# roysubhankar/dwt-domain-adaptation

Measured on NVIDIA H100. Metric: ResNet-50-DWT images/sec fwd+bwd, higher is better.
Workload: dtype f32

## Files before the change

dwt-domain-adaptation_b200/dwt_b200/_native.py:

```python
from __future__ import annotations

import ctypes
import os
import threading

import torch

_HERE = os.path.dirname(os.path.abspath(__file__))
LIB_PATH = os.environ.get("DWT_B200_LIB") or os.path.join(_HERE, "lib", "libdwt_b200.so")

ABI_VERSION = 10
MAX_DOMAINS = 4
MAX_GROUP_SIZE = 64
TC_MAX_GROUP_SIZE = 128
MODE_TRAIN, MODE_EVAL = 0, 1
EPI_NONE, EPI_AFFINE, EPI_RELU, EPI_RESIDUAL = 0, 1, 2, 4
LAYOUT_NHWC = 0x100
DTYPE_BF16 = 0x200
STATUS_NOT_PD, STATUS_BAD_LABEL = 1, 2
ZCA_MAX_ITERATIONS = 16
EIGH = "eigh"
KIND_WHITEN, KIND_BN = 0, 1

_c_float_p = ctypes.c_void_p
_PtrArray = ctypes.c_void_p * MAX_DOMAINS


class TailSite(ctypes.Structure):
    _fields_ = [("x", ctypes.c_void_p), ("eps", ctypes.c_float), ("momentum", ctypes.c_float),
                ("update_running", ctypes.c_int), ("running_mean", ctypes.POINTER(ctypes.c_void_p)),
                ("running_cov", ctypes.POINTER(ctypes.c_void_p)), ("gamma", ctypes.c_void_p), ("beta", ctypes.c_void_p),
                ("save_mean", ctypes.c_void_p), ("save_w", ctypes.c_void_p), ("dx", ctypes.c_void_p),
                ("dgamma", ctypes.c_void_p), ("dbeta", ctypes.c_void_p)]

_SIGNATURES = {
    "dwt_abi_version": (ctypes.c_int, []),
    "dwt_last_error": (ctypes.c_char_p, []),
    "dwt_workspace_bytes": (ctypes.c_size_t, [ctypes.c_int64, ctypes.c_int64, ctypes.c_int64, ctypes.c_int, ctypes.c_int]),
    "dwt_whiten_fwd": (ctypes.c_int, [_c_float_p, _c_float_p, ctypes.c_int64, ctypes.c_int64, ctypes.c_int64,
                                      ctypes.c_int, ctypes.c_int, ctypes.c_int, ctypes.c_float, ctypes.c_float,
                                      ctypes.c_int, ctypes.POINTER(ctypes.c_void_p), ctypes.POINTER(ctypes.c_void_p),
                                      _c_float_p, _c_float_p, _c_float_p, ctypes.c_void_p, ctypes.c_int, _c_float_p,
                                      _c_float_p, ctypes.c_void_p, ctypes.c_size_t, ctypes.c_void_p]),
    "dwt_whiten_bwd": (ctypes.c_int, [_c_float_p, _c_float_p, _c_float_p, _c_float_p, ctypes.c_int64, ctypes.c_int64,
                                      ctypes.c_int64, ctypes.c_int, ctypes.c_int, ctypes.c_int, ctypes.c_float,
                                      _c_float_p, _c_float_p, _c_float_p, _c_float_p, ctypes.c_void_p, _c_float_p,
                                      ctypes.c_int, _c_float_p, _c_float_p, ctypes.c_void_p, ctypes.c_size_t,
                                      ctypes.c_void_p]),
    "dwt_whiten_zca_fwd": (ctypes.c_int, [_c_float_p, _c_float_p, ctypes.c_int64, ctypes.c_int64, ctypes.c_int64,
                                          ctypes.c_int, ctypes.c_int, ctypes.c_int, ctypes.c_float, ctypes.c_float,
                                          ctypes.c_int, ctypes.POINTER(ctypes.c_void_p), ctypes.POINTER(ctypes.c_void_p),
                                          ctypes.c_int, _c_float_p, _c_float_p, _c_float_p, ctypes.c_void_p,
                                          ctypes.c_size_t, ctypes.c_void_p]),
    "dwt_whiten_zca_bwd": (ctypes.c_int, [_c_float_p, _c_float_p, _c_float_p, ctypes.c_int64, ctypes.c_int64,
                                          ctypes.c_int64, ctypes.c_int, ctypes.c_int, ctypes.c_int, ctypes.c_float,
                                          ctypes.c_int, _c_float_p, _c_float_p, _c_float_p, ctypes.c_void_p,
                                          ctypes.c_size_t, ctypes.c_void_p]),
    "dwt_whiten_eigh_fwd": (ctypes.c_int, [_c_float_p, _c_float_p, ctypes.c_int64, ctypes.c_int64, ctypes.c_int64,
                                           ctypes.c_int, ctypes.c_int, ctypes.c_int, ctypes.c_float, ctypes.c_float,
                                           ctypes.c_int, ctypes.POINTER(ctypes.c_void_p), ctypes.POINTER(ctypes.c_void_p),
                                           _c_float_p, _c_float_p, _c_float_p, ctypes.c_void_p, ctypes.c_size_t,
                                           ctypes.c_void_p]),
    "dwt_whiten_eigh_bwd": (ctypes.c_int, [_c_float_p, _c_float_p, _c_float_p, ctypes.c_int64, ctypes.c_int64,
                                           ctypes.c_int64, ctypes.c_int, ctypes.c_int, ctypes.c_int, ctypes.c_float,
                                           _c_float_p, _c_float_p, _c_float_p, ctypes.c_void_p, ctypes.c_size_t,
                                           ctypes.c_void_p]),
    "dwt_whiten_color_fwd": (ctypes.c_int, [_c_float_p, _c_float_p, ctypes.c_int64, ctypes.c_int64, ctypes.c_int64,
                                            ctypes.c_int, ctypes.c_int, ctypes.c_int, ctypes.c_float, ctypes.c_float,
                                            ctypes.c_int, ctypes.POINTER(ctypes.c_void_p), ctypes.POINTER(ctypes.c_void_p),
                                            _c_float_p, _c_float_p, _c_float_p, _c_float_p, ctypes.c_void_p, ctypes.c_size_t,
                                            ctypes.c_void_p]),
    "dwt_whiten_color_bwd": (ctypes.c_int, [_c_float_p, _c_float_p, _c_float_p, ctypes.c_int64, ctypes.c_int64,
                                            ctypes.c_int64, ctypes.c_int, ctypes.c_int, ctypes.c_int, ctypes.c_float,
                                            _c_float_p, _c_float_p, _c_float_p, _c_float_p, _c_float_p, ctypes.c_void_p,
                                            ctypes.c_size_t, ctypes.c_void_p]),
    "dwt_instance_workspace_bytes": (ctypes.c_size_t, [ctypes.c_int64, ctypes.c_int64, ctypes.c_int64, ctypes.c_int]),
    "dwt_whiten_instance_fwd": (ctypes.c_int, [_c_float_p, _c_float_p, ctypes.c_int64, ctypes.c_int64, ctypes.c_int64,
                                               ctypes.c_int, ctypes.c_int, ctypes.c_float, _c_float_p, _c_float_p,
                                               ctypes.c_void_p, ctypes.c_size_t, ctypes.c_void_p]),
    "dwt_whiten_instance_bwd": (ctypes.c_int, [_c_float_p, _c_float_p, _c_float_p, ctypes.c_int64, ctypes.c_int64,
                                               ctypes.c_int64, ctypes.c_int, ctypes.c_int, ctypes.c_float, _c_float_p,
                                               _c_float_p, ctypes.c_void_p, ctypes.c_size_t, ctypes.c_void_p]),
    "dwt_switch_workspace_bytes": (ctypes.c_size_t, [ctypes.c_int64, ctypes.c_int64, ctypes.c_int64, ctypes.c_int]),
    "dwt_whiten_switch_fwd": (ctypes.c_int, [_c_float_p, _c_float_p, ctypes.c_int64, ctypes.c_int64, ctypes.c_int64,
                                             ctypes.c_int, ctypes.c_int, ctypes.c_float, ctypes.c_float, ctypes.c_int,
                                             _c_float_p, _c_float_p, _c_float_p, _c_float_p, _c_float_p, _c_float_p,
                                             ctypes.c_void_p, ctypes.c_size_t, ctypes.c_void_p]),
    "dwt_whiten_switch_bwd": (ctypes.c_int, [_c_float_p, _c_float_p, _c_float_p, ctypes.c_int64, ctypes.c_int64,
                                             ctypes.c_int64, ctypes.c_int, ctypes.c_int, ctypes.c_float, _c_float_p,
                                             _c_float_p, _c_float_p, _c_float_p, _c_float_p, ctypes.c_void_p,
                                             ctypes.c_size_t, ctypes.c_void_p]),
    "dwt_bn_fwd": (ctypes.c_int, [_c_float_p, _c_float_p, ctypes.c_int64, ctypes.c_int64, ctypes.c_int64,
                                  ctypes.c_int, ctypes.c_int, ctypes.c_float, ctypes.c_float, ctypes.c_int,
                                  ctypes.POINTER(ctypes.c_void_p), ctypes.POINTER(ctypes.c_void_p), _c_float_p,
                                  _c_float_p, _c_float_p, ctypes.c_void_p, ctypes.c_int, _c_float_p, _c_float_p,
                                  ctypes.c_void_p, ctypes.c_size_t, ctypes.c_void_p]),
    "dwt_bn_bwd": (ctypes.c_int, [_c_float_p, _c_float_p, _c_float_p, _c_float_p, ctypes.c_int64, ctypes.c_int64, ctypes.c_int64,
                                  ctypes.c_int, ctypes.c_int, _c_float_p, _c_float_p, _c_float_p, _c_float_p,
                                  ctypes.c_void_p, _c_float_p, ctypes.c_int, _c_float_p, _c_float_p, ctypes.c_void_p,
                                  ctypes.c_size_t, ctypes.c_void_p]),
    "dwt_tail2_fwd": (ctypes.c_int, [ctypes.c_int, ctypes.POINTER(TailSite), _c_float_p, ctypes.c_void_p, ctypes.c_int64,
                                     ctypes.c_int64, ctypes.c_int64, ctypes.c_int, ctypes.c_int, ctypes.c_void_p,
                                     ctypes.c_size_t, ctypes.c_void_p]),
    "dwt_tail2_bwd": (ctypes.c_int, [ctypes.c_int, ctypes.POINTER(TailSite), _c_float_p, _c_float_p, ctypes.c_void_p,
                                     _c_float_p, ctypes.c_int64, ctypes.c_int64, ctypes.c_int64, ctypes.c_int, ctypes.c_int,
                                     ctypes.c_void_p, ctypes.c_size_t, ctypes.c_void_p]),
    "dwt_mec_fwd_bwd": (ctypes.c_int, [_c_float_p, _c_float_p, ctypes.c_int64, ctypes.c_int64, _c_float_p,
                                       _c_float_p, _c_float_p, ctypes.c_void_p]),
    "dwt_head_loss_fwd_bwd": (ctypes.c_int, [_c_float_p, ctypes.c_void_p, ctypes.c_int64, ctypes.c_int64, ctypes.c_float,
                                             _c_float_p, _c_float_p, ctypes.c_void_p, ctypes.c_void_p]),
    "dwt_augment_pair": (ctypes.c_int, [ctypes.c_void_p, ctypes.c_int64, ctypes.c_int, ctypes.c_int, ctypes.c_int,
                                        ctypes.c_void_p, ctypes.c_void_p, ctypes.c_void_p, _c_float_p,
                                        ctypes.POINTER(ctypes.c_float), ctypes.POINTER(ctypes.c_float), _c_float_p,
                                        _c_float_p, ctypes.c_int, ctypes.c_void_p]),
    "dwt_maxpool_fwd": (ctypes.c_int, [_c_float_p, _c_float_p, ctypes.c_void_p, ctypes.c_int64, ctypes.c_int64, ctypes.c_int64,
                                       ctypes.c_int64, ctypes.c_int, ctypes.c_int, ctypes.c_int, ctypes.c_int, ctypes.c_void_p]),
    "dwt_maxpool_bwd": (ctypes.c_int, [_c_float_p, ctypes.c_void_p, _c_float_p, ctypes.c_int64, ctypes.c_int64, ctypes.c_int64,
                                       ctypes.c_int64, ctypes.c_int, ctypes.c_int, ctypes.c_int, ctypes.c_int, ctypes.c_void_p]),
    "dwt_launch_count": (ctypes.c_int64, []),
    "dwt_profile_begin": (None, []),
    "dwt_profile_end": (ctypes.c_int, [ctypes.c_void_p, ctypes.c_int]),
}


class ProfileEntry(ctypes.Structure):
    _fields_ = [("name", ctypes.c_char * 48), ("launches", ctypes.c_int64), ("ms", ctypes.c_double),
                ("bytes", ctypes.c_double)]


def profile_begin():
    lib().dwt_profile_begin()


def profile_end():
    cap = 1024
    buf = (ProfileEntry * cap)()
    k = lib().dwt_profile_end(ctypes.cast(buf, ctypes.c_void_p), cap)
    return {buf[i].name.decode(): dict(launches=buf[i].launches, ms=buf[i].ms, bytes=buf[i].bytes) for i in range(k)}


def by_family(prof):
    out = {}
    for name, v in prof.items():
        f = out.setdefault(name.split("|")[0], dict(launches=0, ms=0.0, bytes=0.0))
        for k in f:
            f[k] += v[k]
    return out


def launch_count() -> int:
    return int(lib().dwt_launch_count())
EXPORTS = tuple(_SIGNATURES)

_lib = None
_lock = threading.Lock()


class NativeError(RuntimeError):
    pass


def lib() -> ctypes.CDLL:
    global _lib
    if _lib is None:
        with _lock:
            if _lib is None:
                if not os.path.exists(LIB_PATH):
                    raise NativeError(
                        f"{LIB_PATH} is missing: build it with `python {os.path.join(_HERE, 'build.py')}` "
                        "(dwt_b200 has no CPU or PyTorch fallback)")
                handle = ctypes.CDLL(LIB_PATH)
                for name, (res, args) in _SIGNATURES.items():
                    fn = getattr(handle, name)
                    fn.restype, fn.argtypes = res, args
                if handle.dwt_abi_version() != ABI_VERSION:
                    raise NativeError("libdwt_b200.so ABI version mismatch; rebuild it")
                _lib = handle
    return _lib


def channels_last_supported(channels: int, group_size: int) -> bool:
    if group_size not in (1, 2, 4) or channels % 4:
        return False
    return 0 < channels // 4 <= 16384


def small_bf16_supported(hw: int, group_size: int) -> bool:
    return group_size in (1, 2, 4) and hw % 4 == 0


def tensor_core_bf16_supported(n: int, channels: int, hw: int, group_size: int) -> bool:
    return (group_size in (8, 16, 32, 64) and channels % group_size == 0 and hw >= 32 and hw % 8 == 0
            and n * hw >= 4096)


def tensor_core_nhwc_supported(n: int, channels: int, hw: int, group_size: int) -> bool:
    return (group_size in (8, 16, 32, 64, TC_MAX_GROUP_SIZE) and channels % group_size == 0 and hw >= 32 and hw % 4 == 0
            and n * hw >= 4096)


def check(rc: int) -> None:
    if rc != 0:
        raise NativeError(f"libdwt_b200 error {rc}: {lib().dwt_last_error().decode()}")


def ptr(t):
    return None if t is None else ctypes.c_void_p(t.data_ptr())


def ptr_array(tensors):
    arr = _PtrArray()
    for i, t in enumerate(tensors):
        arr[i] = None if t is None else t.data_ptr()
    return ctypes.cast(arr, ctypes.POINTER(ctypes.c_void_p))


def require_cuda(*tensors, any_dtype=False, bf16=False) -> torch.device:
    dev = None
    for t in tensors:
        if t is None:
            continue
        if not t.is_cuda:
            raise NativeError("dwt_b200 runs on CUDA tensors only (no CPU fallback); got a tensor on " + str(t.device))
        if t.dtype != torch.float32 and not any_dtype and not (bf16 and t.dtype == torch.bfloat16):
            raise NativeError("dwt_b200 computes in float32 (activations may also be bfloat16); got " + str(t.dtype))
        if dev is None:
            dev = t.device
        elif t.device != dev:
            raise NativeError(f"tensors on different devices: {dev} vs {t.device}")
    return dev


def stream_ptr(device) -> ctypes.c_void_p:
    return ctypes.c_void_p(torch.cuda.current_stream(device).cuda_stream)


_workspaces: dict = {}


def workspace(device, n, c, hw, gs, nd):
    if gs == TC_MAX_GROUP_SIZE and c % gs == 0:
        c, gs = 2 * c, MAX_GROUP_SIZE
    need = lib().dwt_workspace_bytes(n, c, hw, gs, nd)
    if need == 0:
        raise NativeError(f"invalid geometry for workspace: C={c} group_size={gs} domains={nd}")
    key = (device.index, torch.cuda.current_stream(device).cuda_stream)
    buf = _workspaces.get(key)
    if buf is None or buf.numel() < need:
        buf = torch.zeros(max(need, 8 << 20), dtype=torch.uint8, device=device)
        _workspaces[key] = buf
    return buf


def instance_workspace(device, n, c, hw, gs):
    need = lib().dwt_instance_workspace_bytes(n, c, hw, gs)
    buf = workspace(device, 1, 4, 1, 1, 1)
    if buf.numel() < need:
        buf = torch.zeros(need, dtype=torch.uint8, device=device)
        _workspaces[(device.index, torch.cuda.current_stream(device).cuda_stream)] = buf
    return buf


def switch_workspace(device, n, c, hw, gs):
    need = lib().dwt_switch_workspace_bytes(n, c, hw, gs)
    buf = workspace(device, 1, 4, 1, 1, 1)
    if buf.numel() < need:
        buf = torch.zeros(need, dtype=torch.uint8, device=device)
        _workspaces[(device.index, torch.cuda.current_stream(device).cuda_stream)] = buf
    return buf


def status(device=None) -> int:
    device = torch.device("cuda", torch.cuda.current_device()) if device is None else device
    buf = _workspaces.get((device.index, torch.cuda.current_stream(device).cuda_stream))
    return 0 if buf is None else int(buf[:4].view(torch.int32).item())


def status_all(device=None) -> int:
    device = torch.device("cuda", torch.cuda.current_device()) if device is None else device
    torch.cuda.synchronize(device)
    st = 0
    for (idx, _), buf in _workspaces.items():
        if idx == device.index:
            st |= int(buf[:4].view(torch.int32).item())
    return st


def status_ptr(device):
    return ctypes.c_void_p(workspace(device, 1, 4, 1, 1, 1).data_ptr())


def clear_status(device=None) -> None:
    device = torch.device("cuda", torch.cuda.current_device()) if device is None else device
    buf = _workspaces.get((device.index, torch.cuda.current_stream(device).cuda_stream))
    if buf is not None:
        buf[:4].zero_()


class NotPositiveDefiniteError(torch.linalg.LinAlgError):
    """What the reference's torch.cholesky raises at utils/whitening.py:53, raised late: the kernels never sync the
    host, so the failure is seen at the next poll (raise_on_status) or explicit check_status() call."""


_poll = {"every": 0, "count": 0}


def raise_on_status(every: int = 1) -> None:
    _poll["every"], _poll["count"] = max(0, int(every)), 0


def check_status(device=None) -> None:
    st = status(device)
    if st == 0:
        return
    clear_status(device)
    if st & STATUS_NOT_PD:
        raise NotPositiveDefiniteError(
            "cholesky: a whitening covariance was not positive definite (status word bit 0; the reference raises "
            "from torch.cholesky, utils/whitening.py:53); the affected group's output is NaN and its running-"
            "statistics update was skipped")
    if st & STATUS_BAD_LABEL:
        raise IndexError("head loss: a label was outside [0, num_classes) and is not ignore_index=-100 "
                         "(F.nll_loss asserts here); the row was dropped")
    raise NativeError(f"unknown status bits {st:#x}")


def poll_status(device) -> None:
    if _poll["every"]:
        _poll["count"] += 1
        if _poll["count"] >= _poll["every"]:
            _poll["count"] = 0
            check_status(device)
```

dwt-domain-adaptation_b200/dwt_b200/build.py:

```python
from __future__ import annotations

import os
import shlex
import subprocess
import sys

HERE = os.path.dirname(os.path.abspath(__file__))
CSRC = os.path.join(HERE, "csrc")
LIB = os.path.join(HERE, "lib", "libdwt_b200.so")
SOURCES = ["api.cu", "norm_small.cu", "norm_tiled.cu", "norm_tc.cu", "norm_tc_apply.cu", "norm_dense.cu", "norm_cl.cu", "mec.cu", "augment.cu", "pool.cu"]
NVCC_FLAGS = ["-O3", "-std=c++17", "-gencode", "arch=compute_90a,code=sm_90a", "-lineinfo",
              "-Xcompiler", "-fPIC,-fvisibility=hidden", "--expt-relaxed-constexpr"]
NVCC_FLAGS += shlex.split(os.environ.get("DWT_NVCC_EXTRA", ""))


def _nvcc() -> str:
    for cand in (os.environ.get("NVCC"), "/usr/local/cuda/bin/nvcc", "nvcc"):
        if cand and (os.path.isabs(cand) and os.path.exists(cand) or not os.path.isabs(cand)):
            return cand
    raise RuntimeError("nvcc not found")


def _stale() -> bool:
    if not os.path.exists(LIB):
        return True
    t = os.path.getmtime(LIB)
    deps = [os.path.join(CSRC, f) for f in os.listdir(CSRC)]
    deps.append(os.path.join(HERE, "..", "..", "include", "dwt_b200.h"))
    deps.append(os.path.abspath(__file__))
    return any(os.path.getmtime(d) > t for d in deps)


def build(force: bool = False, verbose: bool = False) -> str:
    if not force and not _stale():
        return LIB
    os.makedirs(os.path.dirname(LIB), exist_ok=True)
    objs = []
    procs = []
    for src in SOURCES:
        obj = os.path.join(HERE, "lib", src.replace(".cu", ".o"))
        cmd = [_nvcc(), *NVCC_FLAGS, "-c", os.path.join(CSRC, src), "-o", obj]
        if verbose:
            cmd.insert(1, "-Xptxas=-v")
            print(" ".join(cmd), flush=True)
        procs.append((src, subprocess.Popen(cmd, stdout=subprocess.PIPE, stderr=subprocess.STDOUT, text=True)))
        objs.append(obj)
    for src, p in procs:
        out, _ = p.communicate()
        if verbose or p.returncode:
            sys.stdout.write(out)
        if p.returncode:
            raise RuntimeError(f"nvcc failed on {src}")
    link = [_nvcc(), "-shared", "-gencode", "arch=compute_90a,code=sm_90a", "-Xcompiler", "-fPIC", *objs, "-o", LIB]
    subprocess.check_call(link)
    return LIB


if __name__ == "__main__":
    print(build(force="--force" in sys.argv, verbose="--verbose" in sys.argv))
```

dwt-domain-adaptation_b200/dwt_b200/csrc/api.cu:

```cuda
#include <stdarg.h>
#include <stdio.h>
#include <stdlib.h>

#include <atomic>
#include <mutex>
#include <string>
#include <vector>
#include <string.h>

#include "norm_launch.h"

namespace {

thread_local char g_err[512] = "";

int fail(int code, const char* fmt, ...) {
  va_list ap;
  va_start(ap, fmt);
  vsnprintf(g_err, sizeof(g_err), fmt, ap);
  va_end(ap);
  return code;
}

int check_launch(const char* what) {
// ... 587 lines not shown
        case SMALL: dwt::small_bwd_reduce(x, dout, bf16, p.gm, p.vec, fin, beta, w.partial, w.counters, st); break;
        case TILED: dwt::tiled_bwd_reduce(x, dout, p.gm, p.vec, fin, w.partial, w.counters, st); break;
        case TC:
          if (int cr = dwt::tc_bwd_reduce(x, dout, bf16, nhwc, p.gm, rchunks, save_mean, w.partial, st, c.mode == DWT_MODE_TRAIN))
            return fail(DWT_E_LAUNCH, "cuTensorMapEncodeTiled failed (CUresult %d) x=%p dout=%p N=%d C=%d HW=%d D=%d", cr, (const void*)x, (const void*)dout, p.gm.N, p.gm.C, p.gm.HW, p.gm.D);
      }
    }
    if (c.r.fam == CL || c.r.fam == TC) {
      if (int rc = check_launch(c.r.fam == CL ? "channels-last backward reduction kernel" : "tensor-core backward reduction kernel")) return rc;
      Launch l(basis.own() ? basis_family(basis, true, bf16) : c.name(true, FINALIZE), &p.gm, 0.0, st);
      if (c.r.fam == CL) {
        dwt::cl_bwd_finalize(w.partial, cp.nred, p.gm, fin, st);
      } else {
        dwt::dense_partial_reduce(w.partial, rchunks, rproblems, w.gram, st);
        if (basis.own()) basis_bwd(w.gram, p.gm, fin, basis, w.shift, st);
        else dwt::dense_bwd_coef(w.gram, p.gm, fin, w.shift, st);
      }
    }
  } else if (basis.own()) {
    Launch l(basis_family(basis, true, bf16), &p.gm, 0.0, st);
    basis_bwd(nullptr, p.gm, fin, basis, w.shift, st);
  } else {
    Launch l(c.name(true, PREP), &p.gm, 0.0, st);
    if (c.r.fam == TC) dwt::dense_bwd_coef(nullptr, p.gm, fin, w.shift, st);
    else if (c.r.fam == TILED) dwt::tiled_bwd_prep(p.gm, fin, st);
    else dwt::small_bwd_prep(p.gm, fin, st);
  }
  if (int rc = check_launch(c.r.fam == CL ? "channels-last backward finalize kernel" : "whitening backward reduction kernel")) return rc;
  {
    Launch l(c.name(true, APPLY), &p.gm, (3.0 + (dout2 && !masked ? 1.0 : 0.0)) * E, st);
    switch (c.r.fam) {
      case CL:
        if (masked) dwt::cl_bwd_apply(x, dresidual, nullptr, dx, bf16, p.gm, cp.new_, cp.gz_ew, DWT_EPI_AFFINE, w.coef, save_mean, save_w, gamma, beta, st);
        else dwt::cl_bwd_apply(x, dout, dout2, dx, bf16, p.gm, cp.new_, cp.gz_ew, epi, w.coef, save_mean, save_w, gamma, beta, st);
        break;
      case SMALL: dwt::small_bwd_apply(x, dout, dx, bf16, p.gm_ew, p.vec, p.chunks_ew, epi, w.coef, save_mean, save_w, gamma, beta, st); break;
      case TILED: dwt::tiled_bwd_apply(x, dout, dx, p.gm_ew, p.vec, p.chunks_ew, w.coef, st); break;
      case TC:
        if (int cr = dwt::tc_bwd_apply(x, dout, dx, bf16, nhwc, p.gm, tc_apply_ctas(p.gm, 1, 64), w.coef, save_mean, w.shift, st))
          return fail(DWT_E_LAUNCH, "cuTensorMapEncodeTiled failed (CUresult %d)", cr);
    }
  }
  return check_launch(c.r.fam == CL ? "channels-last backward apply kernel" : "whitening backward apply kernel");
}

struct SiteConst { float a, b, unbias; };
SiteConst site_const(int kind, float eps, int64_t N, int64_t HW) {
  if (kind == DWT_KIND_BN) {
    const double M = (double)N * (double)HW;
    return {1.f, eps, M > 1.0 ? (float)(M / (M - 1.0)) : 1.f};
  }
  return {1.f - eps, eps, 1.f};
}

int tail2_plan(Plan& p, int kind, bool bf16, const dwt_tail_site* s, const void* out, int64_t N, int64_t C, int64_t HW, int GS, int D) {
  if (kind != DWT_KIND_WHITEN && kind != DWT_KIND_BN) return fail(DWT_E_INVALID, "bad kind %d", kind);
  if (kind == DWT_KIND_BN && GS != 1) return fail(DWT_E_INVALID, "batch norm has group_size 1 (got %d)", GS);
  if (!s) return fail(DWT_E_INVALID, "null pointer argument");
  if (int rc = make_plan(p, K_STATS, K_APPLY, s[0].x, s[1].x, out, N, C, HW, GS, D, 4)) return rc;
  Route r;
  if (route(p, true, bf16, nullptr, &r) != DWT_OK || r.fam != CL)
    return fail(DWT_E_UNSUPPORTED, "the two-site tail runs on the channels-last kernels: " DWT_CL_RULE " (C=%lld gs=%d)",
                (long long)C, GS);
  for (int k = 0; k < 2; ++k)
    if (!s[k].x || !s[k].gamma || !s[k].beta || !s[k].save_mean || !s[k].save_w || !out) return fail(DWT_E_INVALID, "null pointer argument");
  return check_align(bf16, (uintptr_t)s[0].x | (uintptr_t)s[1].x | (uintptr_t)out, "channels-last tensors");
}

int tail2_workspace(Workspace (&w)[2], void* ws, size_t ws_bytes, int64_t C, int GS, int D) {
  if (!ws) return fail(DWT_E_INVALID, "null pointer argument");
  w[0] = carve(ws, C, GS, D);
  w[1] = carve(ws, C, GS, D, w[0].bytes);
  if (w[1].bytes > ws_bytes) return fail(DWT_E_WORKSPACE, "workspace too small: need %zu bytes, got %zu", w[1].bytes, ws_bytes);
  if ((uintptr_t)ws % 256 != 0) return fail(DWT_E_WORKSPACE, "workspace must be 256-byte aligned");
  return DWT_OK;
}

int tail2_fwd(int kind, const dwt_tail_site* s, float* y, uint8_t* relu_mask, int64_t N, int64_t C, int64_t HW, int GS, int D,
              void* ws, size_t ws_bytes, cudaStream_t st) {
  const bool bf16 = (kind & DWT_DTYPE_BF16) != 0;
  kind &= ~DWT_DTYPE_BF16;
  Plan p;
  if (int rc = tail2_plan(p, kind, bf16, s, y, N, C, HW, GS, D)) return rc;
  if (!relu_mask) return fail(DWT_E_INVALID, "the two-site tail writes the ReLU byte map its backward reads");
  for (int k = 0; k < 2; ++k)
    if (int rc = check_running(s[k].update_running != 0, s[k].running_mean, s[k].running_cov, D)) return rc;
  Workspace w[2];
  if (int rc = tail2_workspace(w, ws, ws_bytes, C, GS, D)) return rc;
  dwt::FwdFin fin[2];
  for (int k = 0; k < 2; ++k) {
    const SiteConst sc = site_const(kind, s[k].eps, N, HW);
    fin[k] = make_fwd_fin(sc.a, sc.b, s[k].momentum, sc.unbias, s[k].update_running, s[k].update_running != 0, s[k].running_mean,
                          s[k].running_cov, s[k].save_mean, s[k].save_w, w[k], D);
  }
  const double n_el = (double)D * (double)N * (double)C * (double)HW;
  const double E = (bf16 ? 2.0 : 4.0) * n_el, Mb = 0.25 * n_el;
  const ClPlan cp = cl_plan(p.gm, 3, 3, 8, 4);
  for (int k = 0; k < 2; ++k) {
    Launch l(fam(bf16, "cl_stats", "cl_stats_bf16"), &p.gm, E, st);
    dwt::cl_stats(s[k].x, bf16, p.gm, cp.nred, cp.gz_red, w[k].partial, w[k].shift, st);
  }
  if (int rc = check_launch("channels-last statistics kernel")) return rc;
  {
    Launch l(fam(bf16, "cl_tail2_fwd_finalize", "cl_tail2_fwd_finalize_bf16"), &p.gm, 0.0, st);
    dwt::cl_fwd_finalize(w[0].partial, cp.nred, w[0].shift, p.gm, fin[0], st, &fin[1], (size_t)(w[1].partial - w[0].partial),
                         (size_t)(w[1].shift - w[0].shift));
  }
  if (int rc = check_launch("channels-last finalize kernel")) return rc;
  {
    Launch l(fam(bf16, "cl_tail2_apply", "cl_tail2_apply_bf16"), &p.gm, 3.0 * E + Mb, st);
    dwt::cl_tail2_apply(s[0].x, s[1].x, y, bf16, p.gm, cp.new_, cp.gz_ew, s[0].save_mean, s[0].save_w, s[0].gamma, s[0].beta,
                        s[1].save_mean, s[1].save_w, s[1].gamma, s[1].beta, relu_mask, st);
  }
  return check_launch("channels-last two-site apply kernel");
}

int tail2_bwd(int kind, const dwt_tail_site* s, const float* dout, const float* dout2, const uint8_t* relu_mask, float* dz,
              int64_t N, int64_t C, int64_t HW, int GS, int D, void* ws, size_t ws_bytes, cudaStream_t st) {
  const bool bf16 = (kind & DWT_DTYPE_BF16) != 0;
  kind &= ~DWT_DTYPE_BF16;
  Plan p;
  if (int rc = tail2_plan(p, kind, bf16, s, dz, N, C, HW, GS, D)) return rc;
  if (!dout || !relu_mask || !s[0].dx || !s[1].dx) return fail(DWT_E_INVALID, "null pointer argument");
  if (int rc = check_align(bf16, (uintptr_t)dout | (uintptr_t)dout2 | (uintptr_t)s[0].dx | (uintptr_t)s[1].dx, "channels-last tensors")) return rc;
  for (int k = 0; k < 2; ++k)
    if ((s[k].dgamma == nullptr) != (s[k].dbeta == nullptr)) return fail(DWT_E_INVALID, "dgamma and dbeta go together");
  Workspace w[2];
  if (int rc = tail2_workspace(w, ws, ws_bytes, C, GS, D)) return rc;
  dwt::BwdFin fin[2];
  for (int k = 0; k < 2; ++k)
    fin[k] = make_bwd_fin(site_const(kind, s[k].eps, N, HW).a, DWT_MODE_TRAIN, k ? DWT_EPI_AFFINE : (DWT_EPI_AFFINE | DWT_EPI_RELU | DWT_EPI_RESIDUAL),
                          s[k].save_mean, s[k].save_w, s[k].gamma, s[k].dgamma, s[k].dbeta, w[k]);
  const double n_el = (double)D * (double)N * (double)C * (double)HW;
  const double E = (bf16 ? 2.0 : 4.0) * n_el, Mb = 0.25 * n_el;
  const ClPlan cp = cl_plan(p.gm, 2, 2, 4, 4);
  {
    Launch l(fam(bf16, "cl_tail2_bwd_reduce", "cl_tail2_bwd_reduce_bf16"), &p.gm, (4.0 + (dout2 ? 1.0 : 0.0)) * E + Mb, st);
    dwt::cl_tail2_bwd_reduce(s[0].x, s[1].x, dout, dout2, bf16, p.gm, cp.nred, cp.gz_red, s[0].save_mean, s[1].save_mean, relu_mask, dz,
                             w[0].partial, (size_t)(w[1].partial - w[0].partial), st);
  }
  if (int rc = check_launch("channels-last two-site backward reduction kernel")) return rc;
  {
    Launch l(fam(bf16, "cl_tail2_bwd_finalize", "cl_tail2_bwd_finalize_bf16"), &p.gm, 0.0, st);
    dwt::cl_bwd_finalize(w[0].partial, cp.nred, p.gm, fin[0], st, &fin[1], (size_t)(w[1].partial - w[0].partial));
  }
  if (int rc = check_launch("channels-last backward finalize kernel")) return rc;
  {
    Launch l(fam(bf16, "cl_tail2_bwd_apply", "cl_tail2_bwd_apply_bf16"), &p.gm, 5.0 * E, st);
    dwt::cl_tail2_bwd_apply(s[0].x, s[1].x, dz, s[0].dx, s[1].dx, bf16, p.gm, cp.new_, cp.gz_ew, w[0].coef, w[1].coef, st);
  }
  return check_launch("channels-last two-site backward apply kernel");
}

int inst_refuse(int64_t N, int64_t C, int64_t HW, int GS, int flags, const char* what = "instance whitening") {
  return fail(DWT_E_UNSUPPORTED, "%s is built for the tensor-core kernels only: group_size 8, 16, 32, 64 "
              "dividing C, HW >= 256 and a multiple of 4 (NCHW bf16: of 8), N <= 65535 images, N*C*HW < 2^31 "
              "(C=%lld HW=%lld N=%lld gs=%d flags=%#x)", what, (long long)C, (long long)HW, (long long)N, GS, flags);
}

int inst_geom(dwt::Geom& gm, int64_t N, int64_t C, int64_t HW, int GS, int flags, const char* what = "instance whitening") {
  if (flags & ~(DWT_LAYOUT_NHWC | DWT_DTYPE_BF16)) return fail(DWT_E_INVALID, "bad flags %#x (DWT_LAYOUT_NHWC | DWT_DTYPE_BF16)", flags);
  if (N <= 0 || C <= 0 || HW <= 0) return fail(DWT_E_INVALID, "empty tensor (N=%lld C=%lld HW=%lld)", (long long)N,
                                               (long long)C, (long long)HW);
  const bool nchw_bf16 = (flags & DWT_DTYPE_BF16) && !(flags & DWT_LAYOUT_NHWC);
  if ((GS != 8 && GS != 16 && GS != 32 && GS != 64) || C % GS != 0 || HW < 256 || HW % (nchw_bf16 ? 8 : 4) != 0 ||
      N > 65535 || N * C * HW >= (int64_t)1 << 31)
    return inst_refuse(N, C, HW, GS, flags, what);
  gm = dwt::Geom{};
  gm.N = 1; gm.C = (int)C; gm.HW = (int)HW; gm.GS = GS; gm.G = (int)(C / GS); gm.D = (int)N; gm.ppc = 1;
  gm.M = (float)HW;
  gm.nchunks = tc_chunks(gm);
  return DWT_OK;
}

Workspace carve_instance(void* base, const dwt::Geom& gm) {
  const size_t P = (size_t)dwt::tc_superblocks(gm) * gm.D, nacc = 64 * 64 + 64;
  size_t off = kOffScratch;
  auto take = [&](size_t nbytes) { size_t o = off; off = align_up(off + nbytes, 256); return o; };
  char* b = static_cast<char*>(base);
  Workspace w{};
  w.status = reinterpret_cast<int*>(b);
  w.counters = reinterpret_cast<int*>(b + kOffCounters);
  w.dom_counter = reinterpret_cast<int*>(b + kOffDom1);
  w.dom_counter2 = reinterpret_cast<int*>(b + kOffDom2);
  w.partial = reinterpret_cast<float*>(b + take(sizeof(float) * P * gm.nchunks * nacc));
  w.gram = gm.nchunks > 1 ? reinterpret_cast<float*>(b + take(sizeof(float) * P * nacc)) : w.partial;
  w.shift = reinterpret_cast<float*>(b + take(sizeof(float) * P * 64));
  w.coef = reinterpret_cast<float*>(b + take(sizeof(float) * (size_t)gm.D * gm.G * dwt::coef_stride(gm.GS)));
  w.bytes = off;
  return w;
}

const char* const kIwName[6][4] = {
    {"iw_stats", "iw_stats_bf16", "iw_stats_nhwc", "iw_stats_nhwc_bf16"},
    {"iw_fwd_finalize", "iw_fwd_finalize_bf16", "iw_fwd_finalize", "iw_fwd_finalize_bf16"},
    {"iw_apply", "iw_apply_bf16", "iw_apply_nhwc", "iw_apply_nhwc_bf16"},
    {"iw_bwd_reduce", "iw_bwd_reduce_bf16", "iw_bwd_reduce_nhwc", "iw_bwd_reduce_nhwc_bf16"},
    {"iw_bwd_finalize", "iw_bwd_finalize_bf16", "iw_bwd_finalize", "iw_bwd_finalize_bf16"},
    {"iw_bwd_apply", "iw_bwd_apply_bf16", "iw_bwd_apply_nhwc", "iw_bwd_apply_nhwc_bf16"}};

int inst_validate(dwt::Geom& gm, Workspace& w, const void* in0, const void* in1, const void* out, int64_t N, int64_t C, int64_t HW,
                  int GS, int flags, const float* save_mean, const float* save_w, void* ws, size_t ws_bytes) {
  if (int rc = inst_geom(gm, N, C, HW, GS, flags)) return rc;
  if (!in0 || !in1 || !out || !save_mean || !save_w || !ws) return fail(DWT_E_INVALID, "null pointer argument");
  if (((uintptr_t)in0 | (uintptr_t)in1 | (uintptr_t)out | (uintptr_t)save_w) % 16 != 0)
    return fail(DWT_E_INVALID, "activation tensors and save_w must be 16-byte aligned (instance whitening: TMA and vector stores)");
  w = carve_instance(ws, gm);
  if (w.bytes > ws_bytes) return fail(DWT_E_WORKSPACE, "workspace too small: need %zu bytes, got %zu", w.bytes, ws_bytes);
  if ((uintptr_t)ws % 256 != 0) return fail(DWT_E_WORKSPACE, "workspace must be 256-byte aligned");
  if (ensure_tc() != 0) return inst_refuse(N, C, HW, GS, flags);
  return DWT_OK;
}

int instance_fwd(const void* x, void* y, int64_t N, int64_t C, int64_t HW, int GS, int flags, float eps, float* save_mean,
                 float* save_w, void* ws, size_t ws_bytes, cudaStream_t st) {
  dwt::Geom gm;
  Workspace w;
  if (int rc = inst_validate(gm, w, x, x, y, N, C, HW, GS, flags, save_mean, save_w, ws, ws_bytes)) return rc;
  const bool nhwc = (flags & DWT_LAYOUT_NHWC) != 0, bf16 = (flags & DWT_DTYPE_BF16) != 0;
  const int k = 2 * nhwc + bf16;
  const double E = (bf16 ? 2.0 : 4.0) * (double)N * (double)C * (double)HW;
  dwt::FwdFin fin{};
  fin.a = 1.f - eps; fin.b = eps; fin.save_mean = save_mean; fin.save_w = save_w; fin.status = w.status;
  {
    Launch l(kIwName[0][k], &gm, E, st);
    if (int cr = dwt::tc_stats(x, bf16, nhwc, gm, gm.nchunks, w.shift, w.partial, st))
      return fail(DWT_E_LAUNCH, "cuTensorMapEncodeTiled failed (CUresult %d) x=%p N=%lld C=%d HW=%d", cr, x, (long long)N, gm.C, gm.HW);
  }
  if (int rc = check_launch("instance whitening statistics kernel")) return rc;
  {
    Launch l(kIwName[1][k], &gm, 0.0, st);
    if (gm.nchunks > 1) dwt::dense_partial_reduce(w.partial, gm.nchunks, dwt::tc_superblocks(gm) * gm.D, w.gram, st);
    dwt::dense_fwd_instance(w.gram, w.shift, gm, fin, st);
  }
  if (int rc = check_launch("instance whitening finalize kernel")) return rc;
  {
    Launch l(kIwName[2][k], &gm, 2.0 * E, st);
    if (int cr = dwt::tc_apply(x, y, bf16, nhwc, gm, tc_apply_ctas(gm, 1, 64), save_mean, save_w, st))
      return fail(DWT_E_LAUNCH, "cuTensorMapEncodeTiled failed (CUresult %d)", cr);
  }
  return check_launch("instance whitening apply kernel");
}

int instance_bwd(const void* x, const void* dout, void* dx, int64_t N, int64_t C, int64_t HW, int GS, int flags, float eps,
                 const float* save_mean, const float* save_w, void* ws, size_t ws_bytes, cudaStream_t st) {
  dwt::Geom gm;
  Workspace w;
  if (int rc = inst_validate(gm, w, x, dout, dx, N, C, HW, GS, flags, save_mean, save_w, ws, ws_bytes)) return rc;
  const bool nhwc = (flags & DWT_LAYOUT_NHWC) != 0, bf16 = (flags & DWT_DTYPE_BF16) != 0;
  const int k = 2 * nhwc + bf16;
  const double E = (bf16 ? 2.0 : 4.0) * (double)N * (double)C * (double)HW;
  dwt::BwdFin fin{};
  fin.a = 1.f - eps; fin.mode = DWT_MODE_TRAIN; fin.save_mean = save_mean; fin.save_w = save_w; fin.coef = w.coef;
  {
    Launch l(kIwName[3][k], &gm, 2.0 * E, st);
    if (int cr = dwt::tc_bwd_reduce(x, dout, bf16, nhwc, gm, gm.nchunks, save_mean, w.partial, st))
      return fail(DWT_E_LAUNCH, "cuTensorMapEncodeTiled failed (CUresult %d) x=%p dout=%p N=%lld C=%d HW=%d", cr, x, dout,
                  (long long)N, gm.C, gm.HW);
  }
  if (int rc = check_launch("instance whitening backward reduction kernel")) return rc;
  {
    Launch l(kIwName[4][k], &gm, 0.0, st);
    if (gm.nchunks > 1) dwt::dense_partial_reduce(w.partial, gm.nchunks, dwt::tc_superblocks(gm) * gm.D, w.gram, st);
    dwt::dense_bwd_coef(w.gram, gm, fin, w.shift, st);
  }
  if (int rc = check_launch("instance whitening backward finalize kernel")) return rc;
  {
    Launch l(kIwName[5][k], &gm, 3.0 * E, st);
    if (int cr = dwt::tc_bwd_apply(x, dout, dx, bf16, nhwc, gm, tc_apply_ctas(gm, 1, 64), w.coef, save_mean, w.shift, st))
      return fail(DWT_E_LAUNCH, "cuTensorMapEncodeTiled failed (CUresult %d)", cr);
  }
  return check_launch("instance whitening backward apply kernel");
}

constexpr const char* kSw = "switchable whitening";

struct SwWork {
  Workspace w;
  float* pd;
  float* part;
  float* sums;
  float* mu;
};

SwWork carve_switch(void* base, const dwt::Geom& gm) {
  SwWork s{};
  s.w = carve_instance(base, gm);
  const size_t rec = (size_t)gm.GS * gm.GS + gm.GS, P = (size_t)gm.D * gm.G;
  size_t off = s.w.bytes;
  auto take = [&](size_t nbytes) { size_t o = off; off = align_up(off + nbytes, 256); return o; };
  char* b = static_cast<char*>(base);
  s.pd = reinterpret_cast<float*>(b + take(sizeof(float) * P * rec));
  s.part = reinterpret_cast<float*>(b + take(sizeof(float) * P * 8));
  s.sums = reinterpret_cast<float*>(b + take(sizeof(float) * gm.G * rec));
  s.mu = reinterpret_cast<float*>(b + take(sizeof(float) * (size_t)gm.D * gm.C));
  s.w.bytes = off;
  return s;
}

int sw_geom(dwt::Geom& gm, int64_t N, int64_t C, int64_t HW, int GS, int mode) {
  if (mode & ~(DWT_MODE_EVAL | DWT_LAYOUT_NHWC | DWT_DTYPE_BF16))
    return fail(DWT_E_INVALID, "bad mode %#x (DWT_MODE_TRAIN or DWT_MODE_EVAL | DWT_LAYOUT_NHWC | DWT_DTYPE_BF16)", mode);
  return inst_geom(gm, N, C, HW, GS, mode & ~DWT_MODE_EVAL, kSw);
}

const char* const kSwName[6][4] = {
// ... 110 lines not shown
}

int dwt_whiten_instance_fwd(const float* x, float* y, int64_t N, int64_t C, int64_t HW, int group_size, int flags, float eps,
                            float* save_mean, float* save_w, void* workspace, size_t workspace_bytes, dwt_stream_t stream) {
  return instance_fwd(x, y, N, C, HW, group_size, flags, eps, save_mean, save_w, workspace, workspace_bytes, (cudaStream_t)stream);
}

size_t dwt_switch_workspace_bytes(int64_t N, int64_t C, int64_t HW, int group_size) {
  dwt::Geom gm;
  char saved[sizeof(g_err)];
  memcpy(saved, g_err, sizeof(g_err));
  const int rc = sw_geom(gm, N, C, HW, group_size, 0);
  memcpy(g_err, saved, sizeof(g_err));
  return rc ? 0 : carve_switch(nullptr, gm).w.bytes;
}

int dwt_whiten_switch_fwd(const float* x, float* y, int64_t N, int64_t C, int64_t HW, int group_size, int mode, float eps,
                          float momentum, int update_running, float* running_mean, float* running_cov, const float* mix,
                          float* save_mean, float* save_w, float* save_stats, void* workspace, size_t workspace_bytes,
                          dwt_stream_t stream) {
  return switch_fwd(x, y, N, C, HW, group_size, mode, eps, momentum, update_running, running_mean, running_cov, mix, save_mean,
                    save_w, save_stats, workspace, workspace_bytes, (cudaStream_t)stream);
}

int dwt_whiten_switch_bwd(const float* x, const float* dout, float* dx, int64_t N, int64_t C, int64_t HW, int group_size,
                          int mode, float eps, const float* mix, const float* save_mean, const float* save_w,
                          const float* save_stats, float* dmix, void* workspace, size_t workspace_bytes, dwt_stream_t stream) {
  return switch_bwd(x, dout, dx, N, C, HW, group_size, mode, eps, mix, save_mean, save_w, save_stats, dmix, workspace,
                    workspace_bytes, (cudaStream_t)stream);
}

int dwt_whiten_instance_bwd(const float* x, const float* dout, float* dx, int64_t N, int64_t C, int64_t HW, int group_size,
                            int flags, float eps, const float* save_mean, const float* save_w, void* workspace,
                            size_t workspace_bytes, dwt_stream_t stream) {
  return instance_bwd(x, dout, dx, N, C, HW, group_size, flags, eps, save_mean, save_w, workspace, workspace_bytes,
                      (cudaStream_t)stream);
}

const char* dwt_last_error(void) { return g_err; }

size_t dwt_workspace_bytes(int64_t N, int64_t C, int64_t HW, int group_size, int n_domains) {
  (void)N; (void)HW;
  if (C <= 0 || group_size < 1 || group_size > DWT_MAX_GROUP_SIZE || C % group_size != 0 || n_domains < 1 ||
      n_domains > DWT_MAX_DOMAINS)
    return 0;
  return carve(nullptr, C, group_size, n_domains, carve(nullptr, C, group_size, n_domains).bytes).bytes;
}

int dwt_whiten_fwd(const float* x, float* y, int64_t N, int64_t C, int64_t HW, int group_size, int n_domains,
                   int mode, float eps, float momentum, int update_running, float* const* running_mean,
                   float* const* running_cov, const float* gamma, const float* beta, const float* residual,
                   uint8_t* relu_mask, int epilogue, float* save_mean, float* save_w, void* workspace,
                   size_t workspace_bytes, dwt_stream_t stream) {
  return whiten_like_fwd(x, y, N, C, HW, group_size, n_domains, mode, 1.f - eps, eps, momentum, 1.f, update_running,
                         running_mean, running_cov, gamma, beta, residual, relu_mask, epilogue, save_mean, save_w,
                         workspace, workspace_bytes, (cudaStream_t)stream);
}

int dwt_whiten_bwd(const float* x, const float* dout, const float* dout2, float* dx, int64_t N, int64_t C, int64_t HW, int group_size,
                   int n_domains, int mode, float eps, const float* save_mean, const float* save_w,
                   const float* gamma, const float* beta, const uint8_t* relu_mask, float* dresidual, int epilogue,
                   float* dgamma, float* dbeta, void* workspace, size_t workspace_bytes, dwt_stream_t stream) {
  return whiten_like_bwd(x, dout, dout2, dx, N, C, HW, group_size, n_domains, mode, 1.f - eps, save_mean, save_w, gamma,
                         beta, relu_mask, dresidual, epilogue, dgamma, dbeta, workspace, workspace_bytes,
                         (cudaStream_t)stream);
}

int dwt_whiten_zca_fwd(const float* x, float* y, int64_t N, int64_t C, int64_t HW, int group_size, int n_domains, int mode,
                       float eps, float momentum, int update_running, float* const* running_mean, float* const* running_cov,
                       int iterations, float* save_mean, float* save_w, float* save_p, void* workspace,
                       size_t workspace_bytes, dwt_stream_t stream) {
  return whiten_like_fwd(x, y, N, C, HW, group_size, n_domains, mode, 1.f - eps, eps, momentum, 1.f, update_running,
                         running_mean, running_cov, nullptr, nullptr, nullptr, nullptr, 0, save_mean, save_w, workspace,
                         workspace_bytes, (cudaStream_t)stream, Basis{Basis::NEWTON_SCHULZ, iterations, save_p});
}

int dwt_whiten_zca_bwd(const float* x, const float* dout, float* dx, int64_t N, int64_t C, int64_t HW, int group_size,
                       int n_domains, int mode, float eps, int iterations, const float* save_mean, const float* save_w,
                       const float* save_p, void* workspace, size_t workspace_bytes, dwt_stream_t stream) {
  return whiten_like_bwd(x, dout, nullptr, dx, N, C, HW, group_size, n_domains, mode, 1.f - eps, save_mean, save_w, nullptr,
                         nullptr, nullptr, nullptr, 0, nullptr, nullptr, workspace, workspace_bytes, (cudaStream_t)stream,
                         Basis{Basis::NEWTON_SCHULZ, iterations, save_p});
}

int dwt_whiten_eigh_fwd(const float* x, float* y, int64_t N, int64_t C, int64_t HW, int group_size, int n_domains, int mode,
                        float eps, float momentum, int update_running, float* const* running_mean, float* const* running_cov,
                        float* save_mean, float* save_w, float* save_e, void* workspace, size_t workspace_bytes,
                        dwt_stream_t stream) {
  return whiten_like_fwd(x, y, N, C, HW, group_size, n_domains, mode, 1.f - eps, eps, momentum, 1.f, update_running,
                         running_mean, running_cov, nullptr, nullptr, nullptr, nullptr, 0, save_mean, save_w, workspace,
                         workspace_bytes, (cudaStream_t)stream, Basis{Basis::EIGH, 0, save_e});
}

int dwt_whiten_eigh_bwd(const float* x, const float* dout, float* dx, int64_t N, int64_t C, int64_t HW, int group_size,
                        int n_domains, int mode, float eps, const float* save_mean, const float* save_w, const float* save_e,
                        void* workspace, size_t workspace_bytes, dwt_stream_t stream) {
  return whiten_like_bwd(x, dout, nullptr, dx, N, C, HW, group_size, n_domains, mode, 1.f - eps, save_mean, save_w, nullptr,
                         nullptr, nullptr, nullptr, 0, nullptr, nullptr, workspace, workspace_bytes, (cudaStream_t)stream,
                         Basis{Basis::EIGH, 0, save_e});
}

int dwt_whiten_color_fwd(const float* x, float* y, int64_t N, int64_t C, int64_t HW, int group_size, int n_domains, int mode,
                         float eps, float momentum, int update_running, float* const* running_mean, float* const* running_cov,
                         const float* color, const float* bias, float* save_mean, float* save_w, void* workspace,
                         size_t workspace_bytes, dwt_stream_t stream) {
  Basis b;
  b.kind = Basis::COLOR; b.color = color; b.bias = bias;
  return whiten_like_fwd(x, y, N, C, HW, group_size, n_domains, mode, 1.f - eps, eps, momentum, 1.f, update_running,
                         running_mean, running_cov, nullptr, nullptr, nullptr, nullptr, 0, save_mean, save_w, workspace,
                         workspace_bytes, (cudaStream_t)stream, b);
}

int dwt_whiten_color_bwd(const float* x, const float* dout, float* dx, int64_t N, int64_t C, int64_t HW, int group_size,
                         int n_domains, int mode, float eps, const float* save_mean, const float* save_w, const float* color,
                         float* dcolor, float* dbias, void* workspace, size_t workspace_bytes, dwt_stream_t stream) {
  Basis b;
  b.kind = Basis::COLOR; b.color = color; b.dcolor = dcolor; b.dbias = dbias;
  return whiten_like_bwd(x, dout, nullptr, dx, N, C, HW, group_size, n_domains, mode, 1.f - eps, save_mean, save_w, nullptr,
                         nullptr, nullptr, nullptr, 0, nullptr, nullptr, workspace, workspace_bytes, (cudaStream_t)stream, b);
}

int dwt_bn_fwd(const float* x, float* y, int64_t N, int64_t C, int64_t HW, int n_domains, int mode, float eps,
               float factor, int update_running, float* const* running_mean, float* const* running_var,
               const float* weight, const float* bias, const float* residual, uint8_t* relu_mask, int epilogue,
               float* save_mean, float* save_invstd, void* workspace, size_t workspace_bytes, dwt_stream_t stream) {
  const double M = (double)N * (double)HW;
  const float unbias = M > 1.0 ? (float)(M / (M - 1.0)) : 1.f;
  return whiten_like_fwd(x, y, N, C, HW, 1, n_domains, mode, 1.f, eps, factor, unbias, update_running, running_mean,
                         running_var, weight, bias, residual, relu_mask, epilogue, save_mean, save_invstd, workspace,
                         workspace_bytes, (cudaStream_t)stream);
}

int dwt_bn_bwd(const float* x, const float* dout, const float* dout2, float* dx, int64_t N, int64_t C, int64_t HW, int n_domains,
               int mode, const float* save_mean, const float* save_invstd, const float* weight, const float* bias,
               const uint8_t* relu_mask, float* dresidual, int epilogue, float* dweight, float* dbias, void* workspace,
               size_t workspace_bytes, dwt_stream_t stream) {
  return whiten_like_bwd(x, dout, dout2, dx, N, C, HW, 1, n_domains, mode, 1.f, save_mean, save_invstd, weight, bias,
                         relu_mask, dresidual, epilogue, dweight, dbias, workspace, workspace_bytes,
                         (cudaStream_t)stream);
}

int dwt_tail2_fwd(int kind, const dwt_tail_site* sites, float* y, uint8_t* relu_mask, int64_t N, int64_t C, int64_t HW,
                  int group_size, int n_domains, void* workspace, size_t workspace_bytes, dwt_stream_t stream) {
  return tail2_fwd(kind, sites, y, relu_mask, N, C, HW, group_size, n_domains, workspace, workspace_bytes, (cudaStream_t)stream);
}

int dwt_tail2_bwd(int kind, const dwt_tail_site* sites, const float* dout, const float* dout2, const uint8_t* relu_mask, float* dz,
                  int64_t N, int64_t C, int64_t HW, int group_size, int n_domains, void* workspace, size_t workspace_bytes,
                  dwt_stream_t stream) {
  return tail2_bwd(kind, sites, dout, dout2, relu_mask, dz, N, C, HW, group_size, n_domains, workspace, workspace_bytes,
                   (cudaStream_t)stream);
}

int dwt_mec_fwd_bwd(const float* x, const float* y, int64_t N, int64_t K, float* loss, float* gx, float* gy,
                    dwt_stream_t stream) {
  if (!x || !y || !loss || !gx || !gy) return fail(DWT_E_INVALID, "null pointer argument");
  if (N <= 0 || K <= 0 || N >= (1 << 24) || K >= (1 << 24)) return fail(DWT_E_INVALID, "bad logits shape [%lld,%lld]", (long long)N, (long long)K);
  {
    Launch l("mec", nullptr, 16.0 * (double)N * (double)K, (cudaStream_t)stream);
    dwt::mec_launch(x, y, (int)N, (int)K, loss, gx, gy, (cudaStream_t)stream);
  }
  return check_launch("MEC kernel");
}

int dwt_head_loss_fwd_bwd(const float* logits, const int64_t* labels, int64_t B, int64_t K, float lambda, float* losses,
                          float* grad, int* status, dwt_stream_t stream) {
  if (!logits || !labels || !losses || !grad) return fail(DWT_E_INVALID, "null pointer argument");
  if (B <= 0 || K <= 0 || B >= (1 << 22) || K >= (1 << 24)) return fail(DWT_E_INVALID, "bad logits shape [3*%lld,%lld]", (long long)B, (long long)K);
  {
    Launch l("head_loss", nullptr, 4.0 * 3 * (double)B * (double)K * 2, (cudaStream_t)stream);
    dwt::head_loss_launch(logits, reinterpret_cast<const long long*>(labels), (int)B, (int)K, lambda, losses, grad, status,
                          (cudaStream_t)stream);
  }
  return check_launch("head loss kernel");
}

int dwt_augment_pair(const uint8_t* images, int64_t B, int src_h, int src_w, int crop, const int32_t* crop_plain,
                     const int32_t* crop_aug, const uint8_t* flip, const float* affine, const float* mean,
                     const float* stdv, float* out_plain, float* out_aug, int layout, dwt_stream_t stream) {
  if (!images || !mean || !stdv) return fail(DWT_E_INVALID, "null pointer argument");
  if (!out_plain && !out_aug) return fail(DWT_E_INVALID, "at least one of out_plain / out_aug is needed");
  if (out_plain && !crop_plain) return fail(DWT_E_INVALID, "out_plain needs crop_plain");
  if (out_aug && (!crop_aug || !flip || !affine)) return fail(DWT_E_INVALID, "out_aug needs crop_aug, flip and affine");
  if (B <= 0 || B > 65535 || src_h <= 0 || src_w <= 0 || src_h > 16384 || src_w > 16384)
    return fail(DWT_E_INVALID, "bad image batch [%lld,%d,%d,3]", (long long)B, src_h, src_w);
  if (crop <= 0 || crop > src_h || crop > src_w) return fail(DWT_E_INVALID, "crop %d does not fit %dx%d", crop, src_h, src_w);
  if (layout != 0 && layout != DWT_LAYOUT_NHWC) return fail(DWT_E_INVALID, "layout must be 0 (NCHW) or DWT_LAYOUT_NHWC");
  for (int c = 0; c < 3; ++c)
    if (!(stdv[c] != 0.f)) return fail(DWT_E_INVALID, "std[%d] must be non-zero", c);
  {
    const double px = (double)B * crop * crop;
    Launch l("augment_pair", nullptr, px * 3 * ((out_plain ? 5.0 : 0.0) + (out_aug ? 5.0 : 0.0)), (cudaStream_t)stream);
    dwt::augment_pair_launch(images, (int)B, src_h, src_w, crop, crop_plain, crop_aug, flip, affine, mean, stdv, out_plain,
                             out_aug, layout != 0, (cudaStream_t)stream);
  }
  return check_launch("augmentation kernel");
}

namespace {
int pool_check(int64_t N, int64_t H, int64_t W, int64_t C, int k, int s, int p, int* OH, int* OW) {
  if (N <= 0 || H <= 0 || W <= 0 || C <= 0 || C % 4 != 0) return fail(DWT_E_INVALID, "bad pooling input [%lld,%lld,%lld,%lld] (C must be a multiple of 4)", (long long)N, (long long)H, (long long)W, (long long)C);
  if (k < 1 || k > 15 || s < 1 || p < 0 || 2 * p > k) return fail(DWT_E_INVALID, "bad pooling window k=%d s=%d p=%d (k <= 15, pad <= k/2)", k, s, p);
  if (H + 2 * p < k || W + 2 * p < k) return fail(DWT_E_INVALID, "pooling window larger than the padded image");
  *OH = (int)((H + 2 * p - k) / s + 1);
  *OW = (int)((W + 2 * p - k) / s + 1);
  if (N * H * W * C >= ((int64_t)1 << 40)) return fail(DWT_E_UNSUPPORTED, "tensor too large");
  return DWT_OK;
}
}

int dwt_maxpool_fwd(const float* x, float* y, uint8_t* argmax, int64_t N, int64_t H, int64_t W, int64_t C, int kernel,
                    int stride, int padding, int flags, dwt_stream_t stream) {
  int OH = 0, OW = 0;
  if (int rc = pool_check(N, H, W, C, kernel, stride, padding, &OH, &OW)) return rc;
  if (flags != 0 && flags != DWT_DTYPE_BF16) return fail(DWT_E_INVALID, "bad flags %#x (0 or DWT_DTYPE_BF16)", flags);
  const bool bf16 = flags == DWT_DTYPE_BF16;
  if (!x || !y || !argmax) return fail(DWT_E_INVALID, "null pointer argument");
  if ((uintptr_t)argmax % 4 != 0) return fail(DWT_E_INVALID, "pooling tensors must be 16-byte aligned");
  if (int rc = check_align(bf16, (uintptr_t)x | (uintptr_t)y, "pooling tensors")) return rc;
  {
    const double in = (double)N * H * W * C, out = (double)N * OH * OW * C;
    Launch l(fam(bf16, "maxpool_fwd", "maxpool_fwd_bf16"), nullptr, (bf16 ? 2.0 : 4.0) * (in + out) + out, (cudaStream_t)stream);
    dwt::maxpool_fwd_launch(x, y, bf16, argmax, (int)N, (int)H, (int)W, (int)C, OH, OW, kernel, stride, padding, (cudaStream_t)stream);
  }
  return check_launch("max-pool forward kernel");
}

int dwt_maxpool_bwd(const float* dy, const uint8_t* argmax, float* dx, int64_t N, int64_t H, int64_t W, int64_t C, int kernel,
                    int stride, int padding, int flags, dwt_stream_t stream) {
  int OH = 0, OW = 0;
  if (int rc = pool_check(N, H, W, C, kernel, stride, padding, &OH, &OW)) return rc;
  if (flags != 0 && flags != DWT_DTYPE_BF16) return fail(DWT_E_INVALID, "bad flags %#x (0 or DWT_DTYPE_BF16)", flags);
  const bool bf16 = flags == DWT_DTYPE_BF16;
  if (!dy || !dx || !argmax) return fail(DWT_E_INVALID, "null pointer argument");
  if ((uintptr_t)argmax % 4 != 0) return fail(DWT_E_INVALID, "pooling tensors must be 16-byte aligned");
  if (int rc = check_align(bf16, (uintptr_t)dy | (uintptr_t)dx, "pooling tensors")) return rc;
  {
    const double in = (double)N * H * W * C, out = (double)N * OH * OW * C;
    Launch l(fam(bf16, "maxpool_bwd", "maxpool_bwd_bf16"), nullptr, (bf16 ? 2.0 : 4.0) * (in + out) + out, (cudaStream_t)stream);
    dwt::maxpool_bwd_launch(dy, argmax, dx, bf16, (int)N, (int)H, (int)W, (int)C, OH, OW, kernel, stride, padding, (cudaStream_t)stream);
  }
  return check_launch("max-pool backward kernel");
}

int64_t dwt_launch_count(void) { return g_launches.load(); }

void dwt_profile_begin(void) {
  std::lock_guard<std::mutex> lk(g_prof_mu);
  for (auto& r : g_prof) { g_event_pool.push_back(r.a); g_event_pool.push_back(r.b); }
  g_prof.clear();
  g_prof_on = true;
}

int dwt_profile_end(dwt_profile_entry* out, int max_entries) {
  std::vector<ProfRec> recs;
  {
    std::lock_guard<std::mutex> lk(g_prof_mu);
    g_prof_on = false;
    recs.swap(g_prof);
  }
  int n = 0;
  for (auto& r : recs) {
    float ms = 0.f;
    if (cudaEventSynchronize(r.b) == cudaSuccess && cudaEventElapsedTime(&ms, r.a, r.b) == cudaSuccess) {
      int k = 0;
      for (; k < n; ++k)
        if (strcmp(out[k].name, r.name) == 0) break;
      if (k == n && n < max_entries) {
        memset(&out[n], 0, sizeof(out[n]));
        strncpy(out[n].name, r.name, sizeof(out[n].name) - 1);
        ++n;
      }
      if (k < n) { out[k].launches += 1; out[k].ms += ms; out[k].bytes += r.bytes; }
    }
    std::lock_guard<std::mutex> lk(g_prof_mu);
    g_event_pool.push_back(r.a); g_event_pool.push_back(r.b);
  }
  return n;
}

}
```

dwt-domain-adaptation_b200/dwt_b200/csrc/norm_cl.cu:

```cuda
#include <stdlib.h>

#include <type_traits>

#include <cuda_bf16.h>

#include "dwt_common.cuh"
#include "norm_launch.h"
#include "small_algebra.cuh"

namespace dwt {
namespace {

constexpr int kT = 256;

__device__ __forceinline__ void pdl_wait() { asm volatile("griddepcontrol.wait;" ::: "memory"); }
__device__ __forceinline__ void pdl_launch_dependents() { asm volatile("griddepcontrol.launch_dependents;" ::: "memory"); }

template <int GS> struct ClShape {
  static constexpr int NSUB = 4 / GS;
  static constexpr int NM = GS * (GS + 1) / 2;
  static constexpr int FWD1 = GS + NM;
  static constexpr int BWD1 = GS * GS + GS;
  static constexpr int FWD = NSUB * FWD1;
  static constexpr int BWD = NSUB * BWD1;
};

struct ClThread {
  int C4, CW, LS, rpi, col, rsub, q;
  bool active;
  __device__ __forceinline__ ClThread(const Geom& gm) {
    C4 = gm.C >> 2;
    CW = gm.cw;
    LS = gm.ls;
    rpi = kT / LS;
    col = threadIdx.x % LS;
    rsub = threadIdx.x / LS;
    q = blockIdx.y * CW + col;
    active = col < CW && rsub < rpi && q < C4;
  }
};

template <int UNROLL, bool DESC, class F>
__device__ __forceinline__ void sweep_rows(const ClThread& t, unsigned rows, F&& body) {
  const unsigned krows = (unsigned)t.rpi * UNROLL, nch = (rows + krows - 1) / krows;
  for (unsigned i = blockIdx.x; i < nch; i += gridDim.x) body((DESC ? nch - 1 - i : i) * krows + t.rsub);
}
#define CL_FOR_DOMAINS(d, gm, DESC) \
  for (int di_ = blockIdx.z, d = (DESC) ? (gm).D - 1 - di_ : di_; di_ < (gm).D; di_ += gridDim.z, d = (DESC) ? (gm).D - 1 - di_ : di_)

template <class T> constexpr bool kBf16 = !std::is_same<T, float>::value;
template <class T>
__device__ __forceinline__ float as_stored(float v) {
  if constexpr (kBf16<T>) return __bfloat162float(__float2bfloat16_rn(v));
  else return v;
}

template <int NACC>
__device__ __forceinline__ void column_reduce(const ClThread& t, float (&acc)[NACC], float* sRed) {
  if (t.rpi == 1) return;
  if (t.rsub < t.rpi) {
#pragma unroll
    for (int i = 0; i < NACC; ++i) sRed[i * kT + threadIdx.x] = acc[i];
  }
  __syncthreads();
  if (t.rsub == 0) {
#pragma unroll
    for (int i = 0; i < NACC; ++i) {
      float s = acc[i];
      for (int r = 1; r < t.rpi; ++r) s += sRed[i * kT + r * t.LS + t.col];
      acc[i] = s;
    }
  }
}

template <class T, int GS>
__global__ void __launch_bounds__(kT, 3) cl_stats_kernel(const T* __restrict__ x, const Geom gm,
                                                         float* __restrict__ partial, float* __restrict__ shift) {
  using S = ClShape<GS>;
  constexpr int UNROLL = 8;
  __shared__ float sRed[kT * S::FWD];
  const ClThread t(gm);
  const unsigned rows = (unsigned)gm.N * gm.HW;
  pdl_launch_dependents();
  CL_FOR_DOMAINS(d, gm, true) {
    const T* xd = x + (size_t)d * rows * gm.C + 4 * t.q;
    float K[4] = {0.f, 0.f, 0.f, 0.f};
    if (t.active) {
      const unsigned np = rows < 8 ? rows : 8;
      for (unsigned r = 0; r < np; ++r) {
        const float4 v = ld4(xd + (size_t)r * gm.C);
        K[0] += v.x; K[1] += v.y; K[2] += v.z; K[3] += v.w;
      }
#pragma unroll
      for (int c = 0; c < 4; ++c) K[c] /= (float)np;
      if (rows > 8) {
        float s1[4] = {0.f, 0.f, 0.f, 0.f}, s2[4] = {0.f, 0.f, 0.f, 0.f};
        const size_t mid = (size_t)gm.HW / 2 + (size_t)sqrtf((float)gm.HW) / 2;
        for (unsigned k = 0; k < 8; ++k) {
          const float4 v = ld4(xd + ((2 * (size_t)k + 1) * rows / 16 + mid) % rows * gm.C);
          const float e[4] = {v.x - K[0], v.y - K[1], v.z - K[2], v.w - K[3]};
#pragma unroll
          for (int c = 0; c < 4; ++c) { s1[c] += e[c]; s2[c] = fmaf(e[c], e[c], s2[c]); }
        }
#pragma unroll
        for (int c = 0; c < 4; ++c) {
          const float dk = s1[c] * 0.125f;
          if (401.f * dk * dk > 400.f * (s2[c] * 0.125f)) K[c] += dk;
        }
      }
      if (blockIdx.x == 0 && t.rsub == 0) *reinterpret_cast<float4*>(shift + (size_t)d * gm.C + 4 * t.q) = make_float4(K[0], K[1], K[2], K[3]);
    }
    float acc[S::FWD];
#pragma unroll
    for (int i = 0; i < S::FWD; ++i) acc[i] = 0.f;
    if (t.active) sweep_rows<UNROLL, true>(t, rows, [&](unsigned r) {
      float4 v[UNROLL];
#pragma unroll
      for (int u = 0; u < UNROLL; ++u) {
        const unsigned rr = r + u * t.rpi;
        v[u] = rr < rows ? ld4(xd + (size_t)rr * gm.C) : make_float4(K[0], K[1], K[2], K[3]);
      }
#pragma unroll
      for (int u = 0; u < UNROLL; ++u) {
        const float e[4] = {v[u].x - K[0], v[u].y - K[1], v[u].z - K[2], v[u].w - K[3]};
#pragma unroll
        for (int s = 0; s < S::NSUB; ++s) {
#pragma unroll
          for (int c = 0; c < GS; ++c) {
            acc[s * S::FWD1 + c] += e[s * GS + c];
#pragma unroll
            for (int j = 0; j <= c; ++j)
              acc[s * S::FWD1 + GS + c * (c + 1) / 2 + j] = fmaf(e[s * GS + c], e[s * GS + j], acc[s * S::FWD1 + GS + c * (c + 1) / 2 + j]);
          }
        }
      }
    });
    column_reduce<S::FWD>(t, acc, sRed);
    if (t.rsub == 0 && t.active) {
      float* dst = partial + (((size_t)d * gridDim.x + blockIdx.x) * t.C4 + t.q) * S::FWD;
#pragma unroll
      for (int i = 0; i < S::FWD; ++i) dst[i] = acc[i];
    }
    if (gridDim.z == 1) __syncthreads();
  }
}

template <int GS, int PER>
__device__ __forceinline__ int acc_index(int g, int a) {
  constexpr int NSUB = 4 / GS;
  return (g / NSUB) * (NSUB * PER) + (g % NSUB) * PER + a;
}

constexpr int kFinQ = 2;

template <int NACC>
__device__ __forceinline__ void column_row_sum(const float* __restrict__ col, int nrows, int W, float (&a)[NACC]) {
  static_assert(NACC % 2 == 0, "accumulators are read as float2");
#pragma unroll
  for (int i = 0; i < NACC; ++i) a[i] = 0.f;
#pragma unroll 4
  for (int r = threadIdx.x; r < nrows; r += 32) {
    const float2* p = reinterpret_cast<const float2*>(col + (size_t)r * W);
#pragma unroll
    for (int i = 0; i < NACC / 2; ++i) {
      const float2 v = __ldcg(p + i);
      a[2 * i] += v.x; a[2 * i + 1] += v.y;
    }
  }
#pragma unroll
  for (int o = 1; o < 32; o <<= 1)
#pragma unroll
    for (int i = 0; i < NACC; ++i) a[i] += __shfl_xor_sync(0xffffffffu, a[i], o);
}

template <int NSUB, int PER>
__device__ __forceinline__ void take_group(const float (&a)[NSUB * PER], int s, float (&v)[PER]) {
#pragma unroll
  for (int i = 0; i < PER; ++i) {
    v[i] = a[i];
#pragma unroll
    for (int k = 1; k < NSUB; ++k)
      if (s == k) v[i] = a[k * PER + i];
  }
}

template <int GS>
__device__ __forceinline__ void cl_fwd_finalize_site(const float* __restrict__ partial, int nrows, const float* __restrict__ shift,
                                                     const Geom& gm, const FwdFin& fin) {
  using SH = ClShape<GS>;
  constexpr int NST = GS + GS * GS;
  __shared__ float sStat[DWT_MAX_DOMAINS][kFinQ][SH::NSUB][NST + 1];
  __shared__ unsigned char sBad[DWT_MAX_DOMAINS][kFinQ][SH::NSUB];
  const int s = threadIdx.x, ql = threadIdx.y, d = threadIdx.z, q = blockIdx.x * blockDim.y + ql;
  const int W = (gm.C >> 2) * SH::FWD;
  const float invM = 1.f / gm.M;
  const bool colok = q < (gm.C >> 2);
  const bool lead = colok && s < SH::NSUB;
  const int g = q * SH::NSUB + (lead ? s : 0);
  const bool direct = gm.D == 1 || fin.aliased == 0;
  const int dbuf = direct ? d : 0;
  const bool upd = fin.update_running && lead && (direct || (fin.aliased == 1 && d == 0));
  float rc_old[GS * GS], rm_old[GS];
  if (upd) {
#pragma unroll
    for (int e = 0; e < GS * GS; ++e) rc_old[e] = fin.rcov[dbuf][(size_t)g * GS * GS + e];
#pragma unroll
    for (int e = 0; e < GS; ++e) rm_old[e] = fin.rmean[dbuf][g * GS + e];
  }
  pdl_launch_dependents();
  pdl_wait();
  float a[SH::FWD];
  if (colok) column_row_sum<SH::FWD>(partial + (size_t)d * nrows * W + (size_t)q * SH::FWD, nrows, W, a);
  if (lead) {
    float v[SH::FWD1];
    take_group<SH::NSUB, SH::FWD1>(a, s, v);
    float mean[GS], cov[GS][GS];
#pragma unroll
    for (int i = 0; i < GS; ++i) mean[i] = shift[(size_t)d * gm.C + g * GS + i] + v[i] * invM;
#pragma unroll
    for (int i = 0; i < GS; ++i)
#pragma unroll
      for (int j = 0; j <= i; ++j) {
        const float c = v[GS + i * (i + 1) / 2 + j] * invM - (v[i] * invM) * (v[j] * invM);
        cov[i][j] = c; cov[j][i] = c;
      }
    const bool bad = factor_thread<GS>(gm, fin, d, g, mean, cov, false);
    if (fin.update_running) {
      if (direct) {
        if (!bad) {
          const float m = fin.momentum, kk = 1.f - fin.momentum;
#pragma unroll
          for (int i = 0; i < GS; ++i) {
            fin.rmean[d][g * GS + i] = m * mean[i] + kk * rm_old[i];
#pragma unroll
            for (int j = 0; j < GS; ++j)
              fin.rcov[d][(size_t)g * GS * GS + i * GS + j] = m * (cov[i][j] * fin.unbias) + kk * rc_old[i * GS + j];
          }
        }
      } else {
        sBad[d][ql][s] = bad ? 1 : 0;
#pragma unroll
        for (int i = 0; i < GS; ++i) {
          sStat[d][ql][s][i] = mean[i];
#pragma unroll
          for (int j = 0; j < GS; ++j) sStat[d][ql][s][GS + i * GS + j] = cov[i][j];
        }
      }
    }
  }
  if (!fin.update_running || direct) return;
  __syncthreads();
  if (!(lead && d == 0)) return;
  if (fin.aliased == 1) {
    const float m = fin.momentum, kk = 1.f - fin.momentum;
    float* rc = fin.rcov[0] + (size_t)g * GS * GS;
    float* rm = fin.rmean[0] + g * GS;
    for (int dd = 0; dd < gm.D; ++dd) {
      if (sBad[dd][ql][s]) continue;
#pragma unroll
      for (int e = 0; e < GS * GS; ++e) rc_old[e] = m * (sStat[dd][ql][s][GS + e] * fin.unbias) + kk * rc_old[e];
#pragma unroll
      for (int e = 0; e < GS; ++e) rm_old[e] = m * sStat[dd][ql][s][e] + kk * rm_old[e];
    }
#pragma unroll
    for (int e = 0; e < GS * GS; ++e) rc[e] = rc_old[e];
#pragma unroll
    for (int e = 0; e < GS; ++e) rm[e] = rm_old[e];
  } else {
    for (int dd = 0; dd < gm.D; ++dd)
      if (!sBad[dd][ql][s]) ema_direct<GS>(gm, fin, dd, g, &sStat[dd][ql][s][0], &sStat[dd][ql][s][GS]);
  }
}

template <int GS>
__global__ void __launch_bounds__(32 * kFinQ * DWT_MAX_DOMAINS) cl_fwd_finalize_kernel(const float* __restrict__ partial, size_t pstride, int nrows,
                                                                                      const float* __restrict__ shift, size_t sstride, const Geom gm,
                                                                                      const __grid_constant__ FwdFin fin, const __grid_constant__ FwdFin fin2) {
  const bool second = blockIdx.y != 0;
  cl_fwd_finalize_site<GS>(partial + (second ? pstride : 0), nrows, shift + (second ? sstride : 0), gm, second ? fin2 : fin);
}

template <class T, int GS, int EPI, bool DS>
__global__ void __launch_bounds__(kT, 3) cl_apply_kernel(const T* __restrict__ x, T* __restrict__ y, const Geom gm,
                                                         const float* __restrict__ save_mean, const float* __restrict__ save_w,
                                                         const float* __restrict__ gamma, const float* __restrict__ beta,
                                                         const T* __restrict__ res, uint8_t* __restrict__ mask,
                                                         const float* __restrict__ save_mean_d, const float* __restrict__ save_w_d,
                                                         const float* __restrict__ gamma_d, const float* __restrict__ beta_d) {
  using S = ClShape<GS>;
  constexpr bool RES = (EPI & DWT_EPI_RESIDUAL) != 0;
  static_assert(!DS || RES, "the two-site tail is a residual epilogue");
  constexpr int UNROLL = DS ? 2 : (RES ? 4 : 8);
  const ClThread t(gm);
  if (!t.active) return;
  const unsigned rows = (unsigned)gm.N * gm.HW;
  pdl_wait();
  CL_FOR_DOMAINS(d, gm, false) {
    float Wp[S::NSUB][S::NM], bp[S::NSUB][GS], Wd[DS ? S::NSUB : 1][S::NM], bd[DS ? S::NSUB : 1][GS];
#pragma unroll
    for (int s = 0; s < S::NSUB; ++s) {
      const int g = t.q * S::NSUB + s;
      load_forward_map<GS, EPI>(save_w + ((size_t)d * gm.G + g) * GS * GS, save_mean + (size_t)d * gm.C + g * GS,
                                gamma + g * GS, beta + g * GS, Wp[s], bp[s]);
      if constexpr (DS)
        load_forward_map<GS, DWT_EPI_AFFINE>(save_w_d + ((size_t)d * gm.G + g) * GS * GS, save_mean_d + (size_t)d * gm.C + g * GS,
                                             gamma_d + g * GS, beta_d + g * GS, Wd[s], bd[s]);
    }
    const size_t base = (size_t)d * rows * gm.C + 4 * t.q;
    const T* xd = x + base;
    const T* rd = res + base;
    T* yd = y + base;
    uint8_t* md = mask + (size_t)d * rows * t.C4 + t.q;
    sweep_rows<UNROLL, false>(t, rows, [&](unsigned r) {
      float4 v[UNROLL], rs[UNROLL];
#pragma unroll
      for (int u = 0; u < UNROLL; ++u) {
        const unsigned rr = r + u * t.rpi;
        if (rr < rows) {
          v[u] = ld4(xd + rr * (unsigned)gm.C);
          if constexpr (RES) rs[u] = ld4(rd + rr * (unsigned)gm.C);
        }
      }
#pragma unroll
      for (int u = 0; u < UNROLL; ++u) {
        const unsigned rr = r + u * t.rpi;
        if (rr < rows) {
          const float e[4] = {v[u].x, v[u].y, v[u].z, v[u].w};
          float o[4], ra[4] = {0.f, 0.f, 0.f, 0.f};
          if constexpr (RES) { ra[0] = rs[u].x; ra[1] = rs[u].y; ra[2] = rs[u].z; ra[3] = rs[u].w; }
          unsigned bits = 0;
#pragma unroll
          for (int s = 0; s < S::NSUB; ++s) {
            float xi[GS], oi[GS];
            if constexpr (DS) {
              float xdi[GS], odi[GS];
#pragma unroll
              for (int c = 0; c < GS; ++c) xdi[c] = ra[s * GS + c];
              apply_group<GS>(Wd[s], bd[s], xdi, odi);
#pragma unroll
              for (int c = 0; c < GS; ++c) ra[s * GS + c] = as_stored<T>(odi[c]);
            }
#pragma unroll
            for (int c = 0; c < GS; ++c) xi[c] = e[s * GS + c];
            apply_group<GS>(Wp[s], bp[s], xi, oi);
#pragma unroll
            for (int c = 0; c < GS; ++c) {
              const float z = RES ? oi[c] + ra[s * GS + c] : oi[c];
              if constexpr (RES) bits |= (z > 0.f ? 1u : 0u) << (s * GS + c);
              o[s * GS + c] = (EPI & DWT_EPI_RELU) ? fmaxf(z, 0.f) : z;
            }
          }
          st4(yd + rr * (unsigned)gm.C, make_float4(o[0], o[1], o[2], o[3]));
          if constexpr (RES) { if (mask != nullptr) md[rr * (unsigned)t.C4] = (uint8_t)bits; }
        }
      }
    });
  }
}

template <int GS>
__device__ __forceinline__ void bwd_accumulate(float* acc, const float (&dz)[GS], const float (&xi)[GS], const float* mu) {
#pragma unroll
  for (int i = 0; i < GS; ++i) {
    acc[GS * GS + i] += dz[i];
#pragma unroll
    for (int j = 0; j < GS; ++j) acc[i * GS + j] = fmaf(dz[i], xi[j] - mu[j], acc[i * GS + j]);
  }
}

template <class T, int GS, int EPI, bool D2, bool DS>
__global__ void __launch_bounds__(kT, 2) cl_bwd_reduce_kernel(const T* __restrict__ x, const T* __restrict__ dout, const T* __restrict__ dout2,
                                                              const Geom gm, const float* __restrict__ save_mean,
                                                              const float* __restrict__ save_w, const float* __restrict__ gamma,
                                                              const float* __restrict__ beta, const uint8_t* __restrict__ mask,
                                                              T* __restrict__ dzout, float* __restrict__ partial,
                                                              const T* __restrict__ xds, const float* __restrict__ save_mean_d,
                                                              size_t pstride) {
  using S = ClShape<GS>;
  constexpr int UNROLL = 4;
  constexpr bool MASK = (EPI & DWT_EPI_RESIDUAL) != 0;
  constexpr bool RELU = (EPI & DWT_EPI_RELU) != 0 && !MASK;
  static_assert(!DS || MASK, "the two-site tail is a residual epilogue");
  constexpr int NS = DS ? 2 : 1;
  __shared__ float sRed[kT * S::BWD];
  const ClThread t(gm);
  const unsigned rows = (unsigned)gm.N * gm.HW;
  pdl_launch_dependents();
  CL_FOR_DOMAINS(d, gm, true) {
    float Wp[S::NSUB][S::NM], bp[S::NSUB][GS], mu[NS][4];
    if (t.active) {
#pragma unroll
      for (int s = 0; s < S::NSUB; ++s) {
        const int g = t.q * S::NSUB + s;
        if constexpr (RELU)
          load_forward_map<GS, EPI>(save_w + ((size_t)d * gm.G + g) * GS * GS, save_mean + (size_t)d * gm.C + g * GS,
                                    gamma + g * GS, beta + g * GS, Wp[s], bp[s]);
      }
#pragma unroll
      for (int k = 0; k < NS; ++k) {
        const float4 m4 = ldg4((k ? save_mean_d : save_mean) + (size_t)d * gm.C + 4 * t.q);
        mu[k][0] = m4.x; mu[k][1] = m4.y; mu[k][2] = m4.z; mu[k][3] = m4.w;
      }
    }
    float acc[NS][S::BWD];
#pragma unroll
    for (int k = 0; k < NS; ++k)
#pragma unroll
      for (int i = 0; i < S::BWD; ++i) acc[k][i] = 0.f;
    const size_t base = (size_t)d * rows * gm.C + 4 * t.q;
    const T* xp[NS];
    xp[0] = x + base;
    if constexpr (DS) xp[NS - 1] = xds + base;
    const T* gd = dout + base;
    const T* gd2 = D2 ? dout2 + base : nullptr;
    T* zd = MASK ? dzout + base : nullptr;
    const uint8_t* md = mask + (size_t)d * rows * t.C4 + t.q;
    constexpr int H = DS ? UNROLL / 2 : UNROLL;
    if (t.active) sweep_rows<UNROLL, true>(t, rows, [&](unsigned r0) {
#pragma unroll
     for (int h = 0; h < UNROLL; h += H) {
      const unsigned r = r0 + h * t.rpi;
      float4 v[NS][H], q[H], q2[D2 ? H : 1];
      unsigned mb[H];
#pragma unroll
      for (int u = 0; u < H; ++u) {
        const unsigned rr = r + u * t.rpi;
        if (rr < rows) {
#pragma unroll
          for (int k = 0; k < NS; ++k) v[k][u] = ld4(xp[k] + (size_t)rr * gm.C);
          q[u] = ld4(gd + (size_t)rr * gm.C);
          if constexpr (MASK) mb[u] = __ldg(md + (size_t)rr * t.C4);
          if constexpr (D2) q2[u] = ld4(gd2 + (size_t)rr * gm.C);
        } else {
#pragma unroll
          for (int k = 0; k < NS; ++k) v[k][u] = make_float4(mu[k][0], mu[k][1], mu[k][2], mu[k][3]);
          q[u] = make_float4(0.f, 0.f, 0.f, 0.f);
          if constexpr (MASK) mb[u] = 0u;
          if constexpr (D2) q2[u] = make_float4(0.f, 0.f, 0.f, 0.f);
        }
      }
      if constexpr (D2) {
#pragma unroll
        for (int u = 0; u < H; ++u) {
          q[u].x = as_stored<T>(q[u].x + q2[u].x); q[u].y = as_stored<T>(q[u].y + q2[u].y);
          q[u].z = as_stored<T>(q[u].z + q2[u].z); q[u].w = as_stored<T>(q[u].w + q2[u].w);
        }
      }
#pragma unroll
      for (int u = 0; u < H; ++u) {
        const float ge[4] = {q[u].x, q[u].y, q[u].z, q[u].w};
        const float e[4] = {v[0][u].x, v[0][u].y, v[0][u].z, v[0][u].w};
        const float ed[4] = {v[NS - 1][u].x, v[NS - 1][u].y, v[NS - 1][u].z, v[NS - 1][u].w};
        float zm[4];
#pragma unroll
        for (int s = 0; s < S::NSUB; ++s) {
          float xi[GS], dz[GS];
#pragma unroll
          for (int c = 0; c < GS; ++c) { xi[c] = e[s * GS + c]; dz[c] = ge[s * GS + c]; }
          if constexpr (RELU) {
            float oi[GS];
            apply_group<GS>(Wp[s], bp[s], xi, oi);
#pragma unroll
            for (int c = 0; c < GS; ++c) dz[c] = oi[c] > 0.f ? dz[c] : 0.f;
          }
          if constexpr (MASK) {
#pragma unroll
            for (int c = 0; c < GS; ++c) { dz[c] = ((mb[u] >> (s * GS + c)) & 1u) ? dz[c] : 0.f; zm[s * GS + c] = dz[c]; }
          }
          bwd_accumulate<GS>(acc[0] + s * S::BWD1, dz, xi, &mu[0][s * GS]);
          if constexpr (DS) {
#pragma unroll
            for (int c = 0; c < GS; ++c) xi[c] = ed[s * GS + c];
            bwd_accumulate<GS>(acc[NS - 1] + s * S::BWD1, dz, xi, &mu[NS - 1][s * GS]);
          }
        }
        if constexpr (MASK) {
          const unsigned rr = r + u * t.rpi;
          if (rr < rows) st4(zd + (size_t)rr * gm.C, make_float4(zm[0], zm[1], zm[2], zm[3]));
        }
      }
     }
    });
#pragma unroll
    for (int k = 0; k < NS; ++k) {
      if (k) __syncthreads();
      column_reduce<S::BWD>(t, acc[k], sRed);
      if (t.rsub == 0 && t.active) {
        float* dst = partial + k * pstride + (((size_t)d * gridDim.x + blockIdx.x) * t.C4 + t.q) * S::BWD;
#pragma unroll
        for (int i = 0; i < S::BWD; ++i) dst[i] = acc[k][i];
      }
    }
    if (gridDim.z == 1) __syncthreads();
  }
}

template <int GS>
__device__ __forceinline__ void cl_bwd_finalize_site(const float* __restrict__ partial, int nrows, const Geom& gm, const BwdFin& fin) {
  using SH = ClShape<GS>;
  const int s = threadIdx.x, d = threadIdx.z, q = blockIdx.x * blockDim.y + threadIdx.y;
  const int W = (gm.C >> 2) * SH::BWD;
  const bool colok = q < (gm.C >> 2);
  pdl_launch_dependents();
  pdl_wait();
  float a[SH::BWD];
  if (colok) column_row_sum<SH::BWD>(partial + (size_t)d * nrows * W + (size_t)q * SH::BWD, nrows, W, a);
  if (colok && s < SH::NSUB) {
    float v[SH::BWD1], R[GS][GS], sdz[GS];
    take_group<SH::NSUB, SH::BWD1>(a, s, v);
#pragma unroll
    for (int i = 0; i < SH::BWD1; ++i) {
      if (i < GS * GS) R[i / GS][i % GS] = v[i]; else sdz[i - GS * GS] = v[i];
    }
    bwd_finalize_thread<GS>(gm, fin, d, q * SH::NSUB + s, R, sdz, false);
  }
  if (!((fin.epi & DWT_EPI_AFFINE) && fin.dgamma != nullptr)) return;
  __syncthreads();
  if (colok && d == 0 && s < 4) {
    const int ch = 4 * q + s;
    float sg = 0.f, sb = 0.f;
    for (int dd = 0; dd < gm.D; ++dd) {
      sg += fin.dgb_part[((size_t)dd * 2 + 0) * gm.C + ch];
      sb += fin.dgb_part[((size_t)dd * 2 + 1) * gm.C + ch];
    }
    fin.dgamma[ch] = sg;
    fin.dbeta[ch] = sb;
  }
}

template <int GS>
__global__ void __launch_bounds__(32 * kFinQ * DWT_MAX_DOMAINS) cl_bwd_finalize_kernel(const float* __restrict__ partial, size_t pstride, int nrows,
                                                                                      const Geom gm, const __grid_constant__ BwdFin fin,
                                                                                      const __grid_constant__ BwdFin fin2) {
  const bool second = blockIdx.y != 0;
  cl_bwd_finalize_site<GS>(partial + (second ? pstride : 0), nrows, gm, second ? fin2 : fin);
}

template <int GS>
struct BwdCoef {
  float A1[GS * (GS + 1) / 2], Bm[GS * (GS + 1) / 2], cv[GS];
  __device__ __forceinline__ void load(const float* cf) {
#pragma unroll
    for (int i = 0; i < GS; ++i) {
      cv[i] = __ldg(cf + 2 * GS * GS + i);
#pragma unroll
      for (int j = 0; j <= i; ++j) {
        A1[i * (i + 1) / 2 + j] = __ldg(cf + j * GS + i);
        Bm[i * (i + 1) / 2 + j] = __ldg(cf + GS * GS + i * GS + j);
      }
    }
  }
  __device__ __forceinline__ void apply(const float (&dz)[GS], const float (&xi)[GS], float* o) const {
#pragma unroll
    for (int i = 0; i < GS; ++i) {
      float a = cv[i];
#pragma unroll
      for (int j = i; j < GS; ++j) a = fmaf(A1[j * (j + 1) / 2 + i], dz[j], a);
#pragma unroll
      for (int j = 0; j < GS; ++j) {
        const int hi = i > j ? i : j, lo = i > j ? j : i;
        a = fmaf(Bm[hi * (hi + 1) / 2 + lo], xi[j], a);
      }
      o[i] = a;
    }
  }
};

template <class T, int GS, int EPI, bool D2, bool DS>
__global__ void __launch_bounds__(kT, 2) cl_bwd_apply_kernel(const T* __restrict__ x, const T* __restrict__ dout, const T* __restrict__ dout2,
                                                             T* __restrict__ dx, const Geom gm, const float* __restrict__ coef,
                                                             const float* __restrict__ save_mean, const float* __restrict__ save_w,
                                                             const float* __restrict__ gamma, const float* __restrict__ beta,
                                                             const T* __restrict__ xds, T* __restrict__ dxds,
                                                             const float* __restrict__ coef_d) {
  using S = ClShape<GS>;
  constexpr int UNROLL = 4;
  constexpr bool RELU = (EPI & DWT_EPI_RELU) != 0;
  static_assert((EPI & DWT_EPI_RESIDUAL) == 0, "the residual tail's apply runs with EPI = AFFINE on dz");
  static_assert(!DS || (!D2 && !RELU), "the two-site tail's apply reads dz");
  constexpr int NS = DS ? 2 : 1;
  const ClThread t(gm);
  if (!t.active) return;
  const unsigned rows = (unsigned)gm.N * gm.HW;
  pdl_wait();
  CL_FOR_DOMAINS(d, gm, false) {
    float Wp[S::NSUB][S::NM], bp[S::NSUB][GS];
    BwdCoef<GS> cf[NS][S::NSUB];
#pragma unroll
    for (int s = 0; s < S::NSUB; ++s) {
      const int g = t.q * S::NSUB + s;
      if constexpr (RELU)
        load_forward_map<GS, EPI>(save_w + ((size_t)d * gm.G + g) * GS * GS, save_mean + (size_t)d * gm.C + g * GS,
                                  gamma + g * GS, beta + g * GS, Wp[s], bp[s]);
#pragma unroll
      for (int k = 0; k < NS; ++k) cf[k][s].load((k ? coef_d : coef) + ((size_t)d * gm.G + g) * coef_stride(GS));
    }
    const size_t base = (size_t)d * rows * gm.C + 4 * t.q;
    const T* xp[NS];
    T* op[NS];
    xp[0] = x + base; op[0] = dx + base;
    if constexpr (DS) { xp[NS - 1] = xds + base; op[NS - 1] = dxds + base; }
    const T* gd = dout + base;
    const T* gd2 = D2 ? dout2 + base : nullptr;
    sweep_rows<UNROLL, false>(t, rows, [&](unsigned r) {
      float4 v[NS][UNROLL], q[UNROLL], q2[D2 ? UNROLL : 1];
#pragma unroll
      for (int u = 0; u < UNROLL; ++u) {
        const unsigned rr = r + u * t.rpi;
        if (rr < rows) {
#pragma unroll
          for (int k = 0; k < NS; ++k) v[k][u] = ld4(xp[k] + (size_t)rr * gm.C);
          q[u] = ld4(gd + (size_t)rr * gm.C);
          if constexpr (D2) q2[u] = ld4(gd2 + (size_t)rr * gm.C);
        }
      }
      if constexpr (D2) {
#pragma unroll
        for (int u = 0; u < UNROLL; ++u)
          if (r + u * t.rpi < rows) {
            q[u].x = as_stored<T>(q[u].x + q2[u].x); q[u].y = as_stored<T>(q[u].y + q2[u].y);
            q[u].z = as_stored<T>(q[u].z + q2[u].z); q[u].w = as_stored<T>(q[u].w + q2[u].w);
          }
      }
#pragma unroll
      for (int u = 0; u < UNROLL; ++u) {
        const unsigned rr = r + u * t.rpi;
        if (rr < rows) {
          const float ge[4] = {q[u].x, q[u].y, q[u].z, q[u].w};
#pragma unroll
          for (int k = 0; k < NS; ++k) {
            const float e[4] = {v[k][u].x, v[k][u].y, v[k][u].z, v[k][u].w};
            float o[4];
#pragma unroll
            for (int s = 0; s < S::NSUB; ++s) {
              float xi[GS], dz[GS];
#pragma unroll
              for (int c = 0; c < GS; ++c) { xi[c] = e[s * GS + c]; dz[c] = ge[s * GS + c]; }
              if constexpr (RELU) {
                float oi[GS];
                apply_group<GS>(Wp[s], bp[s], xi, oi);
#pragma unroll
                for (int c = 0; c < GS; ++c) dz[c] = oi[c] > 0.f ? dz[c] : 0.f;
              }
              cf[k][s].apply(dz, xi, o + s * GS);
            }
            st4(op[k] + (size_t)rr * gm.C, make_float4(o[0], o[1], o[2], o[3]));
          }
        }
      }
    });
  }
}

#define CL_GS(GS_, ...)                                  \
  switch (GS_) {                                         \
    case 1: { constexpr int kGS = 1; __VA_ARGS__; break; } \
    case 2: { constexpr int kGS = 2; __VA_ARGS__; break; } \
    case 4: { constexpr int kGS = 4; __VA_ARGS__; break; } \
    default: break;                                      \
  }
#define CL_EPI(E_, ...)                                                   \
  if ((E_) == 3) { constexpr int kEPI = 3; __VA_ARGS__; }                 \
  else if ((E_) == 1) { constexpr int kEPI = 1; __VA_ARGS__; }            \
  else { constexpr int kEPI = 0; __VA_ARGS__; }
#define CL_EPI_BWD(E_, ...)                                               \
  if ((E_) == 7) { constexpr int kEPI = 7; __VA_ARGS__; }                 \
  else CL_EPI(E_, __VA_ARGS__)
#define CL_D2(P_, ...)                                                    \
  if (P_) { constexpr bool kD2 = true; __VA_ARGS__; }                     \
  else { constexpr bool kD2 = false; __VA_ARGS__; }

inline bool use_pdl() {
  static const bool on = [] { const char* v = getenv("DWT_PDL"); return v != nullptr && v[0] == '1'; }();
  return on;
}

template <class... KArgs, class... Args>
inline void launch_k(void (*kernel)(KArgs...), dim3 grid, dim3 block, cudaStream_t st, bool pdl, Args... args) {
  cudaLaunchConfig_t cfg = {};
  cfg.gridDim = grid; cfg.blockDim = block; cfg.dynamicSmemBytes = 0; cfg.stream = st;
  cudaLaunchAttribute attr[1];
  attr[0].id = cudaLaunchAttributeProgrammaticStreamSerialization;
  attr[0].val.programmaticStreamSerializationAllowed = 1;
  cfg.attrs = attr; cfg.numAttrs = pdl ? 1 : 0;
  cudaLaunchKernelEx(&cfg, kernel, KArgs(args)...);
}

}

bool cl_supports(int C, int GS) {
  if (!(GS == 1 || GS == 2 || GS == 4) || C % 4 != 0) return false;
  const int c4 = C / 4;
  return c4 >= 1 && c4 <= 16384;
}

int cl_lane(int C, int CW) {
  if (C / 4 < 8) return CW;
  if (CW <= 32) {
    int l = 8;
    while (l < CW) l <<= 1;
    return l;
  }
  return (CW + 31) / 32 * 32;
}

namespace {
double cl_busy(int C4, int n) {
  const int cw = (C4 + n - 1) / n, last = C4 - (n - 1) * cw;
  if (cw < 8 || last <= 0) return -1.0;
  const int ls = cl_lane(4 * C4, cw);
  for (int v : {cw, last})
    if (ls <= 32 ? v < 8 : (v % 32 != 0 && v % 32 < 8)) return -1.0;
  return (double)C4 * (kT / ls) / ((double)n * kT);
}
}

int cl_slabs(int C) {
  const int C4 = C / 4;
  if ((C4 & (C4 - 1)) == 0) return C4 <= kT ? 1 : C4 / kT;
  if (C4 < 8) return 1;
  thread_local int memo_c = 0, memo_s = 0;
  if (memo_c == C) return memo_s;
  const int lo = (C4 + kT - 1) / kT, hi = C4 / 8;
  double top = 0.0;
  for (int n = lo; n <= hi; ++n) top = fmax(top, cl_busy(C4, n));
  int best = lo;
  for (int n = lo; n <= hi; ++n)
    if (cl_busy(C4, n) >= 0.0 && 64.0 * cl_busy(C4, n) >= 64.0 * top - 1.0) { best = n; break; }
  memo_c = C;
  memo_s = best;
  return best;
}

namespace {
inline dim3 cl_grid(const Geom& gm, int nctas, int gz) { return dim3(nctas, cl_slabs(gm.C), gz); }
inline Geom cl_geom(const Geom& gm) {
  Geom g = gm;
  const int C4 = gm.C / 4, slabs = cl_slabs(gm.C);
  g.cw = (C4 + slabs - 1) / slabs;
  g.ls = cl_lane(gm.C, g.cw);
  return g;
}
}
int cl_fwd_width(int C, int GS) { return (C / 4) * (4 / GS) * (GS + GS * (GS + 1) / 2); }
int cl_bwd_width(int C, int GS) { return (C / 4) * (4 / GS) * (GS * GS + GS); }


#define CL_T(BF16_, ...)                                                  \
  if (BF16_) { using TT = __nv_bfloat16; __VA_ARGS__; }                   \
  else { using TT = float; __VA_ARGS__; }
#define CL_IN(P_) static_cast<const TT*>(P_)
#define CL_OUT(P_) static_cast<TT*>(P_)

void cl_stats(const void* x, bool bf16, const Geom& gm, int nctas, int gz, float* partial, float* shift, cudaStream_t st) {
  CL_T(bf16, CL_GS(gm.GS, (cl_stats_kernel<TT, kGS><<<cl_grid(gm, nctas, gz), kT, 0, st>>>(CL_IN(x), cl_geom(gm), partial, shift))));
}
inline dim3 fin_block(const Geom& gm) { const int c4 = gm.C / 4; return dim3(32, c4 < kFinQ ? c4 : kFinQ, gm.D); }
inline unsigned fin_blocks(const Geom& gm, const dim3& b) { return (unsigned)((gm.C / 4 + b.y - 1) / b.y); }
void cl_fwd_finalize(const float* partial, int nrows, const float* shift, const Geom& gm, const FwdFin& fin, cudaStream_t st,
                     const FwdFin* fin2, size_t pstride, size_t sstride) {
  const dim3 b = fin_block(gm), g(fin_blocks(gm, b), fin2 ? 2 : 1);
  CL_GS(gm.GS, (launch_k(cl_fwd_finalize_kernel<kGS>, g, b, st, use_pdl(), partial, pstride, nrows, shift, sstride, gm, fin, fin2 ? *fin2 : fin)));
}
void cl_apply(const void* x, void* y, bool bf16, const Geom& gm, int nctas, int gz, int epi, const float* mean, const float* w,
              const float* gamma, const float* beta, const void* residual, uint8_t* mask, cudaStream_t st) {
  const float* nul = nullptr;
  CL_T(bf16, {
    const TT* tnul = nullptr;
    if (epi == 7) {
      CL_GS(gm.GS, (launch_k(cl_apply_kernel<TT, kGS, 7, false>, cl_grid(gm, nctas, gz), dim3(kT), st, use_pdl(), CL_IN(x), CL_OUT(y), cl_geom(gm), mean, w,
                             gamma, beta, CL_IN(residual), mask, nul, nul, nul, nul)));
    } else {
      CL_GS(gm.GS, CL_EPI(epi, (launch_k(cl_apply_kernel<TT, kGS, kEPI, false>, cl_grid(gm, nctas, gz), dim3(kT), st, use_pdl(), CL_IN(x), CL_OUT(y),
                                         cl_geom(gm), mean, w, gamma, beta, tnul, (uint8_t*)nullptr, nul, nul, nul, nul))));
    }
  });
}
void cl_tail2_apply(const void* x, const void* xd, void* y, bool bf16, const Geom& gm, int nctas, int gz, const float* mean, const float* w,
                    const float* gamma, const float* beta, const float* mean_d, const float* w_d, const float* gamma_d,
                    const float* beta_d, uint8_t* mask, cudaStream_t st) {
  CL_T(bf16, CL_GS(gm.GS, (launch_k(cl_apply_kernel<TT, kGS, 7, true>, cl_grid(gm, nctas, gz), dim3(kT), st, use_pdl(), CL_IN(x), CL_OUT(y), cl_geom(gm), mean,
                                    w, gamma, beta, CL_IN(xd), mask, mean_d, w_d, gamma_d, beta_d))));
}
void cl_bwd_reduce(const void* x, const void* dout, const void* dout2, bool bf16, const Geom& gm, int nctas, int gz, int epi, const float* mean,
                   const float* w, const float* gamma, const float* beta, const uint8_t* mask, void* dz, float* partial, cudaStream_t st) {
  const float* nul = nullptr;
  CL_T(bf16, {
    const TT* tnul = nullptr;
    CL_GS(gm.GS, CL_D2(dout2, CL_EPI_BWD(epi, (cl_bwd_reduce_kernel<TT, kGS, kEPI, kD2, false><<<cl_grid(gm, nctas, gz), kT, 0, st>>>(
                                                  CL_IN(x), CL_IN(dout), CL_IN(dout2), cl_geom(gm), mean, w, gamma, beta, mask, CL_OUT(dz), partial, tnul,
                                                  nul, 0)))));
  });
}
void cl_tail2_bwd_reduce(const void* x, const void* xd, const void* dout, const void* dout2, bool bf16, const Geom& gm, int nctas, int gz,
                         const float* mean, const float* mean_d, const uint8_t* mask, void* dz, float* partial, size_t pstride,
                         cudaStream_t st) {
  const float* nul = nullptr;
  CL_T(bf16, CL_GS(gm.GS, CL_D2(dout2, (cl_bwd_reduce_kernel<TT, kGS, 7, kD2, true><<<cl_grid(gm, nctas, gz), kT, 0, st>>>(
                                           CL_IN(x), CL_IN(dout), CL_IN(dout2), cl_geom(gm), mean, nul, nul, nul, mask, CL_OUT(dz), partial, CL_IN(xd),
                                           mean_d, pstride)))));
}
void cl_bwd_finalize(const float* partial, int nrows, const Geom& gm, const BwdFin& fin, cudaStream_t st, const BwdFin* fin2, size_t pstride) {
  const dim3 b = fin_block(gm), g(fin_blocks(gm, b), fin2 ? 2 : 1);
  CL_GS(gm.GS, (launch_k(cl_bwd_finalize_kernel<kGS>, g, b, st, use_pdl(), partial, pstride, nrows, gm, fin, fin2 ? *fin2 : fin)));
}
void cl_bwd_apply(const void* x, const void* dout, const void* dout2, void* dx, bool bf16, const Geom& gm, int nctas, int gz, int epi,
                  const float* coef, const float* mean, const float* w, const float* gamma, const float* beta, cudaStream_t st) {
  const float* nul = nullptr;
  CL_T(bf16, {
    const TT* tnul = nullptr;
    CL_GS(gm.GS, CL_D2(dout2, CL_EPI(epi, (launch_k(cl_bwd_apply_kernel<TT, kGS, kEPI, kD2, false>, cl_grid(gm, nctas, gz), dim3(kT), st, use_pdl(),
                                                    CL_IN(x), CL_IN(dout), CL_IN(dout2), CL_OUT(dx), cl_geom(gm), coef, mean, w, gamma, beta, tnul,
                                                    (TT*)nullptr, nul)))));
  });
}
void cl_tail2_bwd_apply(const void* x, const void* xd, const void* dz, void* dx, void* dxd, bool bf16, const Geom& gm, int nctas, int gz,
                        const float* coef, const float* coef_d, cudaStream_t st) {
  const float* nul = nullptr;
  CL_T(bf16, {
    const TT* tnul = nullptr;
    CL_GS(gm.GS, (launch_k(cl_bwd_apply_kernel<TT, kGS, 1, false, true>, cl_grid(gm, nctas, gz), dim3(kT), st, use_pdl(), CL_IN(x), CL_IN(dz), tnul,
                           CL_OUT(dx), cl_geom(gm), coef, nul, nul, nul, nul, CL_IN(xd), CL_OUT(dxd), coef_d)));
  });
}

}
```

dwt-domain-adaptation_b200/dwt_b200/csrc/norm_launch.h:

```cpp
#pragma once
#include <stdint.h>

#include "dwt_common.cuh"

namespace dwt {

inline void bind_context() {
  thread_local bool bound = false;
  if (!bound) { cudaFree(nullptr); bound = true; }
}

bool small_supports(int GS);
void small_stats(const void* x, bool bf16, const Geom& gm, int vec, const FwdFin& fin, float* partial, int* counters,
                 cudaStream_t st);
void small_eval_prep(const Geom& gm, const FwdFin& fin, cudaStream_t st);
void small_apply(const void* x, void* y, bool bf16, const Geom& gm, int vec, int chunks, int epi, const float* mean,
                 const float* w, const float* gamma, const float* beta, const void* residual, cudaStream_t st);
void small_bwd_reduce(const void* x, const void* dout, bool bf16, const Geom& gm, int vec, const BwdFin& fin,
                      const float* beta, float* partial, int* counters, cudaStream_t st);
void small_bwd_prep(const Geom& gm, const BwdFin& fin, cudaStream_t st);
void small_bwd_apply(const void* x, const void* dout, void* dx, bool bf16, const Geom& gm, int vec, int chunks, int epi,
                     const float* coef, const float* mean, const float* w, const float* gamma, const float* beta,
                     cudaStream_t st);

int tiled_smem_bytes(int GS);
int tiled_init();
void tiled_stats(const float* x, const Geom& gm, int vec, const FwdFin& fin, float* partial, int* counters,
                 cudaStream_t st);
void tiled_eval_prep(const Geom& gm, const FwdFin& fin, cudaStream_t st);
void tiled_apply(const float* x, float* y, const Geom& gm, int vec, int chunks, const float* mean, const float* w,
                 cudaStream_t st);
void tiled_bwd_reduce(const float* x, const float* dout, const Geom& gm, int vec, const BwdFin& fin, float* partial,
                      int* counters, cudaStream_t st);
void tiled_bwd_prep(const Geom& gm, const BwdFin& fin, cudaStream_t st);
void tiled_bwd_apply(const float* x, const float* dout, float* dx, const Geom& gm, int vec, int chunks,
                     const float* coef, cudaStream_t st);

int tc_init();
bool tc_supports(const Geom& gm, int vec);
int tc_superblocks(const Geom& gm);
int tc_stats(const void* x, bool bf16, bool nhwc, const Geom& gm, int nchunks, float* shift, float* partial, cudaStream_t st);
int tc_gram_pair(const void* x, bool nhwc, const Geom& gm, int nchunks, const float* shift, float* partial, cudaStream_t st);
int tc_bwd_reduce(const void* x, const void* dout, bool bf16, bool nhwc, const Geom& gm, int nchunks, const float* save_mean,
                  float* partial, cudaStream_t st, bool pilot = true);

int dense_init();
void dense_partial_reduce(const float* partial, int nchunks, int problems, float* gram, cudaStream_t st);
void dense_fwd_factor(const float* gram, const float* shift, const Geom& gm, const FwdFin& fin, cudaStream_t st);
void dense_bwd_coef(const float* rgram, const Geom& gm, const BwdFin& fin, float* dybar, cudaStream_t st);
void dense_fwd_zca(const float* gram, const float* shift, const Geom& gm, const FwdFin& fin, int iters, float* save_p,
                   cudaStream_t st);
void dense_bwd_zca(const float* rgram, const Geom& gm, const BwdFin& fin, int iters, const float* save_p, float* dybar,
                   cudaStream_t st);
void dense_fwd_eigh(const float* gram, const float* shift, const Geom& gm, const FwdFin& fin, float* save_e, cudaStream_t st);
void dense_bwd_eigh(const float* rgram, const Geom& gm, const BwdFin& fin, const float* save_e, float* dybar, cudaStream_t st);
void dense_fwd_color(const float* gram, const float* shift, const Geom& gm, const FwdFin& fin, const float* color, float* gw,
                     cudaStream_t st);
void dense_bwd_color(const float* rgram, const Geom& gm, const BwdFin& fin, const float* color, float* dcolor, float* dbias,
                     float* dybar, cudaStream_t st);
void dense_fwd_instance(const float* gram, const float* shift, const Geom& gm, const FwdFin& fin, cudaStream_t st);
struct SwFin {
  float a, b;
  float momentum;
  int train, update_running;
  const float* mix;
  float* rmean;
  float* rcov;
  float* save_mean;
  float* save_w;
  float* save_stats;
  int* status;
};
void dense_sw_stats(const float* gram, const float* shift, const Geom& gm, const SwFin& fin, cudaStream_t st);
void dense_sw_fwd_factor(const Geom& gm, const SwFin& fin, cudaStream_t st);
void dense_sw_bwd(const float* rgram, const Geom& gm, const SwFin& fin, float* pd, float* part, float* sums, float* dmix,
                  float* coef, float* dybar, float* mu, cudaStream_t st);

int tc_apply_init();
int tc_apply(const void* x, void* y, bool bf16, bool nhwc, const Geom& gm, int nctas, const float* save_mean, const float* save_w,
             cudaStream_t st, const float* bias = nullptr);
int tc_bwd_apply(const void* x, const void* dout, void* dx, bool bf16, bool nhwc, const Geom& gm, int nctas, const float* coef,
                 const float* save_mean, const float* dybar, cudaStream_t st);

bool cl_supports(int C, int GS);
int cl_slabs(int C);
int cl_lane(int C, int CW);
int cl_fwd_width(int C, int GS);
int cl_bwd_width(int C, int GS);
void cl_stats(const void* x, bool bf16, const Geom& gm, int nctas, int gz, float* partial, float* shift, cudaStream_t st);
void cl_fwd_finalize(const float* partial, int nrows, const float* shift, const Geom& gm, const FwdFin& fin, cudaStream_t st,
                     const FwdFin* fin2 = nullptr, size_t pstride = 0, size_t sstride = 0);
void cl_apply(const void* x, void* y, bool bf16, const Geom& gm, int nctas, int gz, int epi, const float* mean, const float* w,
              const float* gamma, const float* beta, const void* residual, uint8_t* mask, cudaStream_t st);
void cl_bwd_reduce(const void* x, const void* dout, const void* dout2, bool bf16, const Geom& gm, int nctas, int gz, int epi, const float* mean,
                   const float* w, const float* gamma, const float* beta, const uint8_t* mask, void* dz, float* partial, cudaStream_t st);
void cl_bwd_finalize(const float* partial, int nrows, const Geom& gm, const BwdFin& fin, cudaStream_t st,
                     const BwdFin* fin2 = nullptr, size_t pstride = 0);
void cl_bwd_apply(const void* x, const void* dout, const void* dout2, void* dx, bool bf16, const Geom& gm, int nctas, int gz, int epi,
                  const float* coef, const float* mean, const float* w, const float* gamma, const float* beta, cudaStream_t st);
void cl_tail2_apply(const void* x, const void* xd, void* y, bool bf16, const Geom& gm, int nctas, int gz, const float* mean, const float* w,
                    const float* gamma, const float* beta, const float* mean_d, const float* w_d, const float* gamma_d,
                    const float* beta_d, uint8_t* mask, cudaStream_t st);
void cl_tail2_bwd_reduce(const void* x, const void* xd, const void* dout, const void* dout2, bool bf16, const Geom& gm, int nctas, int gz,
                         const float* mean, const float* mean_d, const uint8_t* mask, void* dz, float* partial, size_t pstride,
                         cudaStream_t st);
void cl_tail2_bwd_apply(const void* x, const void* xd, const void* dz, void* dx, void* dxd, bool bf16, const Geom& gm, int nctas, int gz,
                        const float* coef, const float* coef_d, cudaStream_t st);

void maxpool_fwd_launch(const void* x, void* y, bool bf16, uint8_t* idx, int N, int H, int W, int C, int OH, int OW, int k, int s, int p,
                        cudaStream_t st);
void maxpool_bwd_launch(const void* dy, const uint8_t* idx, void* dx, bool bf16, int N, int H, int W, int C, int OH, int OW, int k, int s,
                        int p, cudaStream_t st);

void augment_pair_launch(const uint8_t* images, int B, int SH, int SW, int CR, const int* crop_plain, const int* crop_aug,
                         const uint8_t* flip, const float* affine, const float* mean, const float* stdv,
                         float* out_plain, float* out_aug, int nhwc, cudaStream_t st);
void head_loss_launch(const float* logits, const long long* labels, int B, int K, float lambda, float* losses,
                      float* grad, int* status, cudaStream_t st);
void mec_launch(const float* x, const float* y, int N, int K, float* loss, float* gx, float* gy, cudaStream_t st);

}
```

dwt-domain-adaptation_b200/dwt_b200/functional.py:

```python
from __future__ import annotations

import math
from typing import NamedTuple

import torch

from . import _native as nv


def _channels_last(x):
    return x.dim() == 4 and not x.is_contiguous() and x.is_contiguous(memory_format=torch.channels_last)


def _channels_last_family(x, group_size):
    return _channels_last(x) and nv.channels_last_supported(x.shape[1], group_size)


def _nhwc_tensor_core(x, group_size, n_domains):
    return (x.dim() == 4 and x.shape[0] % n_domains == 0 and x.data_ptr() % 16 == 0
            and nv.tensor_core_nhwc_supported(x.shape[0] // n_domains, x.shape[1], x.shape[2] * x.shape[3], group_size))


class Route(NamedTuple):
    nhwc: bool
# ... 136 lines not shown
    def backward(ctx, dout):
        lib = nv.lib()
        mask = save_p = None
        if ctx.iterations:
            x, save_mean, save_w, gamma_c, beta_c, save_p = ctx.saved_tensors
        elif ctx.residual_mode == "mask":
            x, save_mean, save_w, gamma_c, beta_c, mask = ctx.saved_tensors
        elif ctx.residual_mode == "aten":
            x, save_mean, save_w, gamma_c, beta_c, out = ctx.saved_tensors
            extra = ctx.__dict__.pop("_dwt_extra_grad", None)
            if extra is not None:
                dout = dout + extra
            dout = torch.ops.aten.threshold_backward(dout, out, 0)
        else:
            x, save_mean, save_w, gamma_c, beta_c = ctx.saved_tensors
        kind, gs, n_domains, mode, eps, epi, n, c, hw, gshape = ctx.cfg
        r = ctx.route
        dout2 = ctx.__dict__.pop("_dwt_extra_grad", None)
        if dout.dtype != x.dtype:
            dout = dout.to(x.dtype)
        if dout2 is not None and not (r.cl and dout2.shape == dout.shape and dout2.dtype == dout.dtype
                                      and dout2.is_contiguous(memory_format=torch.channels_last)):
            dout, dout2 = dout + dout2, None
        dout = dout.contiguous(memory_format=torch.channels_last) if r.nhwc else dout.contiguous()
        if r.align and dout.data_ptr() % r.align:
            dout = dout.clone(memory_format=torch.channels_last if r.nhwc else torch.contiguous_format)
        dev = nv.require_cuda(dout, bf16=True)
        dx = torch.empty_like(x)
        want_affine = gamma_c is not None and (ctx.needs_input_grad[1] or ctx.needs_input_grad[2])
        d_res = None
        if ctx.residual_mode == "mask":
            d_res = torch.empty_like(x)
        elif ctx.residual_mode == "aten" and ctx.needs_input_grad[3]:
            d_res = dout
        dgamma = torch.empty(c, dtype=torch.float32, device=dev) if want_affine else None
        dbeta = torch.empty(c, dtype=torch.float32, device=dev) if want_affine else None
        ws = nv.workspace(dev, n, c, hw, gs, n_domains)
        with torch.cuda.device(dev):
            if ctx.iterations == nv.EIGH:
                rc = lib.dwt_whiten_eigh_bwd(nv.ptr(x), nv.ptr(dout), nv.ptr(dx), n, c, hw, gs, n_domains, mode, eps,
                                             nv.ptr(save_mean), nv.ptr(save_w), nv.ptr(save_p), nv.ptr(ws), ws.numel(),
                                             nv.stream_ptr(dev))
            elif ctx.iterations:
                rc = lib.dwt_whiten_zca_bwd(nv.ptr(x), nv.ptr(dout), nv.ptr(dx), n, c, hw, gs, n_domains, mode, eps,
                                            int(ctx.iterations), nv.ptr(save_mean), nv.ptr(save_w), nv.ptr(save_p),
                                            nv.ptr(ws), ws.numel(), nv.stream_ptr(dev))
            elif kind == "whiten":
                rc = lib.dwt_whiten_bwd(nv.ptr(x), nv.ptr(dout), nv.ptr(dout2), nv.ptr(dx), n, c, hw, gs, n_domains, mode, eps,
                                        nv.ptr(save_mean), nv.ptr(save_w), nv.ptr(gamma_c), nv.ptr(beta_c), nv.ptr(mask),
                                        nv.ptr(d_res) if mask is not None else None, epi,
                                        nv.ptr(dgamma), nv.ptr(dbeta), nv.ptr(ws), ws.numel(), nv.stream_ptr(dev))
            else:
                rc = lib.dwt_bn_bwd(nv.ptr(x), nv.ptr(dout), nv.ptr(dout2), nv.ptr(dx), n, c, hw, n_domains, mode,
                                    nv.ptr(save_mean), nv.ptr(save_w), nv.ptr(gamma_c), nv.ptr(beta_c), nv.ptr(mask),
                                    nv.ptr(d_res) if mask is not None else None, epi,
                                    nv.ptr(dgamma), nv.ptr(dbeta), nv.ptr(ws), ws.numel(), nv.stream_ptr(dev))
        nv.check(rc)
        if want_affine:
            dgamma, dbeta = dgamma.view(gshape), dbeta.view(gshape)
        return (dx, dgamma, dbeta, d_res if ctx.needs_input_grad[3] else None) + (None,) * 11


class _TailPairFunction(torch.autograd.Function):

    @staticmethod
    def forward(ctx, x, xd, gamma, beta, gamma_d, beta_d, kind, group_size, n_domains, sites):
        lib = nv.lib()
        gs = group_size if kind == "whiten" else 1
        if not (x.shape == xd.shape and _channels_last_family(x, gs) and _channels_last_family(xd, gs)):
            raise ValueError("the two-site tail takes two channels-last tensors of one shape with a channels-last build")
        if x.shape[0] % n_domains != 0:
            raise ValueError(f"batch of {x.shape[0]} does not split into {n_domains} domains")
        n_all, c = x.shape[0], x.shape[1]
        hw = x.shape[2] * x.shape[3]
        n = n_all // n_domains
        if xd.dtype != x.dtype:
            raise ValueError("the two-site tail takes two tensors of one dtype")
        bf16 = x.dtype == torch.bfloat16
        stats = [gamma, beta, gamma_d, beta_d, *[t for run, *_ in sites for pair in run for t in pair]]
        dev = nv.require_cuda(x, xd, *stats, bf16=True)
        nv.require_cuda(*stats)
        params = [(gamma, beta), (gamma_d, beta_d)]
        c_sites = (nv.TailSite * 2)()
        keep = []
        saved = []
        for k, (inp, (g, b), (running, eps, momentum, update)) in enumerate(zip((x, xd), params, sites)):
            for d, (rm_t, rv_t) in enumerate(running):
                _check_param(f"running mean of domain {d}", rm_t, c)
                _check_param(f"running second moment of domain {d}", rv_t, c * gs)
            _check_param("gamma / weight", g, c)
            _check_param("beta / bias", b, c)
            g_c, b_c = g.detach().reshape(-1).contiguous(), b.detach().reshape(-1).contiguous()
            save_mean = torch.empty(n_domains, c, dtype=torch.float32, device=dev)
            save_w = torch.empty(n_domains, c // gs, gs, gs, dtype=torch.float32, device=dev)
            rm = nv.ptr_array([pr[0] for pr in running]) if update else None
            rv = nv.ptr_array([pr[1] for pr in running]) if update else None
            c_sites[k] = nv.TailSite(inp.data_ptr(), eps, momentum, int(update), rm, rv, g_c.data_ptr(), b_c.data_ptr(),
                                     save_mean.data_ptr(), save_w.data_ptr(), None, None, None)
            keep += [g_c, b_c, rm, rv]
            saved += [save_mean, save_w, g_c]
        y = torch.empty_like(x)
        mask = torch.empty(x.numel() // 4, dtype=torch.uint8, device=dev)
        ws = nv.workspace(dev, n, c, hw, gs, n_domains)
        nv_kind = (nv.KIND_WHITEN if kind == "whiten" else nv.KIND_BN) | (nv.DTYPE_BF16 if bf16 else 0)
        with torch.cuda.device(dev):
            rc = lib.dwt_tail2_fwd(nv_kind, c_sites, nv.ptr(y), nv.ptr(mask), n, c, hw, gs, n_domains, nv.ptr(ws), ws.numel(),
                                   nv.stream_ptr(dev))
        nv.check(rc)
        nv.poll_status(dev)
        seen = set()
        for running, _, _, update in sites:
            for buf in (t for pair in running for t in pair) if update else ():
                if id(buf) not in seen:
                    seen.add(id(buf))
                    torch.autograd.graph.increment_version(buf)
        ctx.save_for_backward(x, xd, mask, *saved)
        ctx.cfg = (nv_kind, gs, n_domains, n, c, hw, [s[1] for s in sites], gamma.shape, gamma_d.shape)
        return y

    @staticmethod
    def backward(ctx, dout):
        lib = nv.lib()
        x, xd, mask, mean0, w0, g0, mean1, w1, g1 = ctx.saved_tensors
        nv_kind, gs, n_domains, n, c, hw, eps, gshape, gshape_d = ctx.cfg
        dout2 = ctx.__dict__.pop("_dwt_extra_grad", None)
        if dout.dtype != x.dtype:
            dout = dout.to(x.dtype)
        if dout2 is not None and not (dout2.shape == dout.shape and dout2.dtype == dout.dtype
                                      and dout2.is_contiguous(memory_format=torch.channels_last)):
            dout, dout2 = dout + dout2, None
        dout = dout.contiguous(memory_format=torch.channels_last)
        dev = nv.require_cuda(dout, bf16=True)
        dz = torch.empty_like(x)
        dx, dxd = torch.empty_like(x), torch.empty_like(xd)
        grads = [torch.empty(2, c, dtype=torch.float32, device=dev) for _ in range(2)]
        c_sites = (nv.TailSite * 2)()
        for k, (inp, mean, w, g, d_in, gr) in enumerate(zip((x, xd), (mean0, mean1), (w0, w1), (g0, g1), (dx, dxd), grads)):
            c_sites[k] = nv.TailSite(inp.data_ptr(), eps[k], 0.0, 0, None, None, g.data_ptr(), g.data_ptr(), mean.data_ptr(),
                                     w.data_ptr(), d_in.data_ptr(), gr[0].data_ptr(), gr[1].data_ptr())
        ws = nv.workspace(dev, n, c, hw, gs, n_domains)
        with torch.cuda.device(dev):
            rc = lib.dwt_tail2_bwd(nv_kind, c_sites, nv.ptr(dout), nv.ptr(dout2), nv.ptr(mask), nv.ptr(dz), n, c, hw, gs, n_domains,
                                   nv.ptr(ws), ws.numel(), nv.stream_ptr(dev))
        nv.check(rc)
        return (dx, dxd, grads[0][0].view(gshape), grads[0][1].view(gshape), grads[1][0].view(gshape_d),
                grads[1][1].view(gshape_d)) + (None,) * 4


def tail_pair(x, xd, gamma, beta, gamma_d, beta_d, *, kind, group_size, n_domains, sites):
    return _TailPairFunction.apply(x, xd, gamma, beta, gamma_d, beta_d, kind, group_size, n_domains,
                                   [(r, float(e), float(m), bool(u)) for r, e, m, u in sites])


class _ForkForSum(torch.autograd.Function):

    @staticmethod
    def forward(ctx, y):
        ctx.producer = y.grad_fn
        return y.view_as(y), y.view_as(y)

    @staticmethod
    def backward(ctx, ga, gb):
        producer, ctx.producer = ctx.producer, None
        if ga is None or gb is None:
            return ga if gb is None else gb
        if producer is None or "_dwt_extra_grad" in producer.__dict__:
            return ga + gb
        producer.__dict__["_dwt_extra_grad"] = gb
        return ga


def fork_for_sum(y):
    fn = getattr(y, "grad_fn", None)
    if not torch.is_grad_enabled() or fn is None or not isinstance(fn, (_NormFunction._backward_cls, _TailPairFunction._backward_cls)):
        return y, y
    return _ForkForSum.apply(y)


_ACT_DTYPES = (torch.float32, torch.bfloat16)


def norm(x, gamma, beta, *, kind, group_size, n_domains, training_stats, eps, momentum, update_running,
         running, relu=False, residual=None, iterations=0):
    if iterations != nv.EIGH and iterations and not 1 <= iterations <= nv.ZCA_MAX_ITERATIONS:
        raise ValueError(f"iterations must be in [1, {nv.ZCA_MAX_ITERATIONS}] (got {iterations})")
    mode = nv.MODE_TRAIN if training_stats else nv.MODE_EVAL
    args = (kind, group_size, n_domains, mode, float(eps), float(momentum), bool(update_running), running, bool(relu))
    r = route(x, residual, kind, group_size, n_domains)
    if r is None:
        xf, rf = x.float(), None if residual is None else residual.float()
        y = _NormFunction.apply(xf, gamma, beta, rf, *args, route(xf, rf, kind, group_size, n_domains), iterations)
        return y.to(x.dtype)
    return _NormFunction.apply(x, gamma, beta, residual, *args, r, iterations)


def _aligned(t):
    t = t.detach().contiguous()
    return t if t.data_ptr() % 16 == 0 else t.clone()


class _ColorFunction(torch.autograd.Function):

    @staticmethod
    def forward(ctx, x, color, bias, group_size, n_domains, mode, eps, momentum, update_running, running, r):
        lib = nv.lib()
        gs = group_size
        if not r.nhwc and not x.is_contiguous():
            x = x.contiguous()
        n_all, c, hw = x.shape[0], x.shape[1], math.prod(x.shape[2:])
        layout = (nv.LAYOUT_NHWC if r.nhwc else 0) | (nv.DTYPE_BF16 if r.bf16 else 0)
        if n_all % n_domains != 0:
            raise ValueError(f"batch of {n_all} does not split into {n_domains} domains")
        n = n_all // n_domains
        stats = [color, bias, *[t for pair in running for t in pair]]
        dev = nv.require_cuda(x, *stats, bf16=True)
        nv.require_cuda(*stats)
        for d, (rm_t, rv_t) in enumerate(running):
            _check_param(f"running mean of domain {d}", rm_t, c)
            _check_param(f"running second moment of domain {d}", rv_t, c * gs)
        color_c, bias_c = _aligned(color), _aligned(bias)
        _check_param("color / weight", color_c, c * gs)
        _check_param("bias", bias_c, c)
        y = torch.empty_like(x)
        save_mean = torch.empty(n_domains, c, dtype=torch.float32, device=dev)
        save_w = torch.empty(n_domains, c // gs, gs, gs, dtype=torch.float32, device=dev)
        ws = nv.workspace(dev, n, c, hw, gs, n_domains)
        need_running = (mode == nv.MODE_EVAL) or update_running
        rm = nv.ptr_array([p[0] for p in running]) if need_running else None
        rv = nv.ptr_array([p[1] for p in running]) if need_running else None
        with torch.cuda.device(dev):
            rc = lib.dwt_whiten_color_fwd(nv.ptr(x), nv.ptr(y), n, c, hw, gs, n_domains, mode | layout, eps, momentum,
                                          int(update_running), rm, rv, nv.ptr(color_c), nv.ptr(bias_c), nv.ptr(save_mean),
                                          nv.ptr(save_w), nv.ptr(ws), ws.numel(), nv.stream_ptr(dev))
        nv.check(rc)
        nv.poll_status(dev)
        if update_running and mode == nv.MODE_TRAIN:
            seen = set()
            for pair in running:
                for buf in pair:
                    if buf is not None and id(buf) not in seen:
                        seen.add(id(buf))
                        torch.autograd.graph.increment_version(buf)
        ctx.save_for_backward(x, save_mean, save_w, color_c)
        ctx.cfg = (gs, n_domains, mode | layout, eps, n, c, hw, color.shape, bias.shape)
        ctx.route = r
        return y

    @staticmethod
    def backward(ctx, dout):
        lib = nv.lib()
        x, save_mean, save_w, color_c = ctx.saved_tensors
        gs, n_domains, mode, eps, n, c, hw, cshape, bshape = ctx.cfg
        r = ctx.route
        if dout.dtype != x.dtype:
            dout = dout.to(x.dtype)
        dout = dout.contiguous(memory_format=torch.channels_last) if r.nhwc else dout.contiguous()
        if r.align and dout.data_ptr() % r.align:
            dout = dout.clone(memory_format=torch.channels_last if r.nhwc else torch.contiguous_format)
        dev = nv.require_cuda(dout, bf16=True)
        dx = torch.empty_like(x)
        want = ctx.needs_input_grad[1] or ctx.needs_input_grad[2]
        dcolor = torch.empty(c // gs, gs, gs, dtype=torch.float32, device=dev) if want else None
        dbias = torch.empty(c, dtype=torch.float32, device=dev) if want else None
        ws = nv.workspace(dev, n, c, hw, gs, n_domains)
        with torch.cuda.device(dev):
            rc = lib.dwt_whiten_color_bwd(nv.ptr(x), nv.ptr(dout), nv.ptr(dx), n, c, hw, gs, n_domains, mode, eps,
                                          nv.ptr(save_mean), nv.ptr(save_w), nv.ptr(color_c), nv.ptr(dcolor), nv.ptr(dbias),
                                          nv.ptr(ws), ws.numel(), nv.stream_ptr(dev))
        nv.check(rc)
        if want:
            dcolor, dbias = dcolor.view(cshape), dbias.view(bshape)
        return (dx, dcolor, dbias) + (None,) * 8


def color(x, weight, bias, *, group_size, n_domains, training_stats, eps, momentum, update_running, running):
    mode = nv.MODE_TRAIN if training_stats else nv.MODE_EVAL
    args = (group_size, n_domains, mode, float(eps), float(momentum), bool(update_running), running)
    r = route(x, None, "whiten", group_size, n_domains)
    if r is None:
        xf = x.float()
        y = _ColorFunction.apply(xf, weight, bias, *args, route(xf, None, "whiten", group_size, n_domains))
        return y.to(x.dtype)
    return _ColorFunction.apply(x, weight, bias, *args, r)


class _InstanceFunction(torch.autograd.Function):

    @staticmethod
    def forward(ctx, x, group_size, eps):
        dev = nv.require_cuda(x, bf16=True)
        lib = nv.lib()
        gs = group_size
        nhwc = _channels_last(x)
        fmt = torch.channels_last if nhwc else torch.contiguous_format
        x = x.contiguous(memory_format=fmt)
        if x.data_ptr() % 16:
            x = x.clone(memory_format=fmt)
        n, c, hw = x.shape[0], x.shape[1], math.prod(x.shape[2:])
        flags = (nv.LAYOUT_NHWC if nhwc else 0) | (nv.DTYPE_BF16 if x.dtype == torch.bfloat16 else 0)
        y = torch.empty_like(x)
        save_mean = torch.empty(n, c, dtype=torch.float32, device=dev)
        save_w = torch.empty(n, max(c // gs, 1), gs, gs, dtype=torch.float32, device=dev)
        ws = nv.instance_workspace(dev, n, c, hw, gs)
        with torch.cuda.device(dev):
            rc = lib.dwt_whiten_instance_fwd(nv.ptr(x), nv.ptr(y), n, c, hw, gs, flags, eps, nv.ptr(save_mean),
                                             nv.ptr(save_w), nv.ptr(ws), ws.numel(), nv.stream_ptr(dev))
        nv.check(rc)
        nv.poll_status(dev)
        ctx.save_for_backward(x, save_mean, save_w)
        ctx.cfg = (gs, flags, eps, n, c, hw, fmt)
        return y

    @staticmethod
    def backward(ctx, dout):
        lib = nv.lib()
        x, save_mean, save_w = ctx.saved_tensors
        gs, flags, eps, n, c, hw, fmt = ctx.cfg
        dout = dout.to(x.dtype).contiguous(memory_format=fmt)
        if dout.data_ptr() % 16:
            dout = dout.clone(memory_format=fmt)
        dev = nv.require_cuda(dout, bf16=True)
        dx = torch.empty_like(x)
        ws = nv.instance_workspace(dev, n, c, hw, gs)
        with torch.cuda.device(dev):
            rc = lib.dwt_whiten_instance_bwd(nv.ptr(x), nv.ptr(dout), nv.ptr(dx), n, c, hw, gs, flags, eps, nv.ptr(save_mean),
                                             nv.ptr(save_w), nv.ptr(ws), ws.numel(), nv.stream_ptr(dev))
        nv.check(rc)
        return dx, None, None


def instance_whiten(x, *, group_size, eps):
    if x.dim() < 3:
        raise ValueError(f"instance whitening expects [N, C, *] input (got {x.dim()}D input)")
    nv.require_cuda(x, bf16=True)
    if x.dtype == torch.bfloat16 and not _channels_last(x) and math.prod(x.shape[2:]) % 8:
        return _InstanceFunction.apply(x.float(), int(group_size), float(eps)).to(x.dtype)
# ... 139 lines not shown
```

dwt-domain-adaptation_b200/dwt_b200/fused.py:

```python
from __future__ import annotations

import torch
import torch.nn as nn

from . import _native as nv
from . import functional as F
from .whitening import _Whitening


class DomainTripleNorm(nn.Module):
    def __init__(self, kind, num_features, group_size=4, n_domains=3):
        super().__init__()
        if kind not in ("whiten", "bn"):
            raise ValueError("kind must be 'whiten' or 'bn'")
        self.kind, self.num_features, self.n_domains = kind, num_features, n_domains
        self.group_size = min(num_features, group_size) if kind == "whiten" else 1
        self.kernel_epilogue = self.group_size in (1, 2, 4)

    def forward(self, x, domain_modules, gamma, beta, relu=False, residual=None, replicated=False, count_batches=True):
        mods = list(domain_modules)
        if len(mods) != self.n_domains:
            raise ValueError(f"expected {self.n_domains} domain modules")
        if x.dim() != 4:
            raise ValueError('expected 4D input (got {}D input)'.format(x.dim()))
        if gamma is not None and gamma.dim() == 3 and tuple(gamma.shape[1:]) != (1, 1):
            return self._forward_color(x, mods, gamma, beta, relu, residual, replicated, count_batches)
        if not self.kernel_epilogue and torch.bfloat16 in (x.dtype, getattr(residual, "dtype", None)):
            out = self.forward(x.float(), mods, gamma, beta, relu, None if residual is None else residual.float(), replicated,
                               count_batches)
            return out.to(x.dtype)
        if replicated:
            return self._forward_replicated(x, mods, gamma, beta, relu, residual, count_batches)
        iterations = self._iterations(mods)
        running, eps, momentum, update = self._running_args(mods, count_batches)
        batch_stats = mods[0].training or not mods[0].track_running_stats
        if not self.kernel_epilogue:
            y = F.norm(x, None, None, kind=self.kind, group_size=self.group_size, n_domains=self.n_domains,
                       training_stats=batch_stats, eps=eps, momentum=momentum, update_running=update, running=running,
                       iterations=iterations)
            return self._tensor_epilogue(y, gamma, beta, relu, residual)
        return F.norm(x, gamma, beta, kind=self.kind, group_size=self.group_size, n_domains=self.n_domains,
                      training_stats=batch_stats, eps=eps, momentum=momentum, update_running=update,
                      running=running, relu=relu, residual=residual)

    def _forward_color(self, x, mods, gamma, beta, relu, residual, replicated, count_batches):
        gs = self.group_size
        if self.kind != "whiten" or self.kernel_epilogue:
            raise nv.NativeError("a matrix gamma (colouring) is built for whitening at group_size 8, 16, 32, 64 on the "
                                 f"tensor-core kernels (got {self.kind}, group_size {gs})")
        if self._iterations(mods):
            raise nv.NativeError("a matrix gamma (colouring) whitens in the Cholesky basis: the domain modules must be "
                                 "WTransform2d")
        if tuple(gamma.shape) != (self.num_features // gs, gs, gs):
            raise ValueError(f"a matrix gamma has shape [C/gs, gs, gs] = {[self.num_features // gs, gs, gs]}, "
                             f"got {list(gamma.shape)}")
        if residual is not None and not relu:
            raise ValueError("a fused residual needs relu=True")
        bias = beta.reshape(-1)
        if replicated:
            y = self._forward_replicated(x, mods, gamma, bias, False, None, count_batches, color=True)
        else:
            running, eps, momentum, update = self._running_args(mods, count_batches)
            y = F.color(x, gamma, bias, group_size=gs, n_domains=self.n_domains,
                        training_stats=mods[0].training or not mods[0].track_running_stats, eps=eps, momentum=momentum,
                        update_running=update, running=running)
        return self._tensor_epilogue(y, None, None, relu, residual)

    def _iterations(self, mods):
        if self.kind != "whiten":
            return 0
        basis = {m._iterations() if isinstance(m, _Whitening) else 0 for m in mods}
        if len(basis) != 1:
            raise ValueError("the domain modules of a whitening site must share one basis (WTransform2d, "
                             "ExactZCAWTransform2d, or ZCAWTransform2d with one number of iterations); got iterations "
                             f"{sorted(basis, key=str)}")
        iterations = basis.pop()
        if iterations and self.kernel_epilogue:
            raise nv.NativeError("the ZCA basis runs on the tensor-core kernels: group_size 8, 16, 32, 64 "
                                 f"(got {self.group_size})")
        return iterations

    def _running_args(self, mods, count_batches):
        m0 = mods[0]
        update = m0.training and m0.track_running_stats
        if self.kind == "whiten":
            running = [(m.running_mean, m.running_variance) for m in mods]
            eps, momentum = m0.eps, m0.momentum
        else:
            if count_batches:
                counters = [m.num_batches_tracked for m in mods if m.training and m.track_running_stats]
                if counters:
                    torch._foreach_add_(counters, 1)
            running = [(m.running_mean, m.running_var) for m in mods]
            eps = m0.eps
            momentum = m0.momentum if m0.momentum is not None or not update else 1.0 / m0.num_batches_tracked.item()
        return running, eps, momentum or 0.0, update

    def forward_with_downsample(self, x, domain_modules, gamma, beta, xd, down, down_modules, down_gamma, down_beta,
                                count_batches=True):
        mods, down_mods = list(domain_modules), list(down_modules)
        self._iterations(mods)
        down._iterations(down_mods)
        pair =(self.kernel_epilogue and down.kernel_epilogue and self.kind == down.kind
                and self.group_size == down.group_size and self.n_domains == down.n_domains
                and len(mods) == len(down_mods) == self.n_domains and x.dim() == 4 and x.shape == xd.shape
                and mods[0].training and down_mods[0].training
                and x.dtype == xd.dtype
                and all(F._channels_last_family(t, self.group_size) for t in (x, xd)))
        if not pair:
            identity = down(xd, down_mods, down_gamma, down_beta, relu=False, count_batches=count_batches)
            return self(x, mods, gamma, beta, True, residual=identity, count_batches=count_batches)
        down_args = down._running_args(down_mods, count_batches)
        site_args = self._running_args(mods, count_batches)
        return F.tail_pair(x, xd, gamma, beta, down_gamma, down_beta, kind=self.kind, group_size=self.group_size,
                           n_domains=self.n_domains, sites=(site_args, down_args))

    @staticmethod
    def _tensor_epilogue(y, gamma, beta, relu, residual):
        if residual is not None and not relu:
            raise ValueError("a fused residual needs relu=True")
        if gamma is not None:
            y = y * gamma + beta
        if residual is not None:
            y = y + residual
        return torch.relu(y) if relu else y

    def _forward_replicated(self, x, mods, gamma, beta, relu, residual, count_batches=True, color=False):
        second = "running_variance" if self.kind == "whiten" else "running_var"
        keep = {}
        for m in mods:
            if not (m.training and m.track_running_stats):
                continue
            if self.kind == "bn":
                if count_batches:
                    m.num_batches_tracked += 1
                f = m.momentum if m.momentum is not None else 1.0 / m.num_batches_tracked.item()
            else:
                f = m.momentum
            rm, rv = m.running_mean, getattr(m, second)
            key = (rm.data_ptr(), rv.data_ptr())
            prod, _ = keep.get(key, (1.0, None))
            keep[key] = (prod * (1.0 - f), (rm, rv))
        means = {k[0] for k in keep}
        seconds = {k[1] for k in keep}
        if len(means) != len(keep) or len(seconds) != len(keep):
            raise ValueError("replicated statistics need each running_mean paired with one second-moment buffer")
        m0 = mods[0]
        iterations = self._iterations(mods)
        common = dict(kind=self.kind, group_size=self.group_size, n_domains=1, training_stats=True, eps=m0.eps,
                      iterations=iterations)
        if self.kernel_epilogue:
            common.update(relu=relu, residual=residual)
            g_arg, b_arg = gamma, beta
        else:
            g_arg = b_arg = None

        def site(training_stats, momentum, update_running, running):
            if color:
                return F.color(x, gamma, beta, group_size=self.group_size, n_domains=1, training_stats=training_stats,
                               eps=m0.eps, momentum=momentum, update_running=update_running, running=running)
            return F.norm(x, g_arg, b_arg, momentum=momentum, update_running=update_running, running=running,
                          **dict(common, training_stats=training_stats))
        out = None
        if not m0.training and m0.track_running_stats:
            out = site(False, 0.0, False, [(m0.running_mean, getattr(m0, second))])
        for prod, pair in keep.values():
            y = site(True, 1.0 - prod, True, [pair])
            out = y if out is None else out
        if out is None:
            out = site(True, 0.0, False, [(m0.running_mean, getattr(m0, second))])
        return out if self.kernel_epilogue or color else self._tensor_epilogue(out, gamma, beta, relu, residual)
```

harness/resnet50_dwt.py:

```python
from __future__ import annotations

import torch
import torch.nn as nn

_STAGES = ((64, 3, 1), (128, 4, 2), (256, 6, 2), (512, 3, 2))
_DOMAINS = ("s", "t", "t_aug")
EXPANSION = 4


_REPLICATED = [False]
_BATCHED_COUNTERS = [False]


class WhitenScaleShift(nn.Module):

    def __init__(self, layers, planes, group_size, running_mean, running_variance,
                 track_running_stats=True, affine=True):
        super().__init__()
        self.planes, self.group_size, self.affine = planes, group_size, affine
        self.wh = layers.WTransform2d(planes, group_size, running_m=running_mean,
                                      running_var=running_variance,
                                      track_running_stats=track_running_stats)
        if affine:
            self.gamma = nn.Parameter(torch.ones(planes, 1, 1))
# ... 21 lines not shown
        for n, m in zip(names, mods):
            setattr(self, n, m)
        gname = f"{pre}gamma{post}" if pre == "" else "downsample_gamma"
        bname = f"{pre}beta{post}" if pre == "" else "downsample_beta"
        setattr(self, gname, nn.Parameter(gamma))
        setattr(self, bname, nn.Parameter(beta))
        if not hasattr(self, "_sites"):
            self._sites = {}
        self._sites[tag] = (names, gname, bname, whiten)
        if site_mode == "fused":
            object.__setattr__(self, f"_fused_{tag}", layers.DomainTripleNorm(
                kind="whiten" if whiten else "bn", num_features=planes,
                group_size=group_size if whiten else 1))

    def _site(self, tag, x, relu, residual=None):
        names, gname, bname, whiten = self._sites[tag]
        gamma, beta = getattr(self, gname), getattr(self, bname)
        if residual is not None:
            fused = getattr(self, f"_fused_{tag}", None) if self.training else None
            if fused is not None:
                mods = [getattr(self, n) for n in names]
                return fused(x, [m.wh if whiten else m for m in mods], gamma, beta, True, residual=residual,
                             replicated=_REPLICATED[0], count_batches=not _BATCHED_COUNTERS[0])
            return torch.relu_(self._site(tag, x, relu=False) + residual)
        if self.training:
            fused = getattr(self, f"_fused_{tag}", None)
            mods = [getattr(self, n) for n in names]
            if fused is not None:
                return fused(x, [m.wh if whiten else m for m in mods], gamma, beta, relu, replicated=_REPLICATED[0],
                             count_batches=not _BATCHED_COUNTERS[0])
            if _REPLICATED[0]:
                raise RuntimeError("replicated statistics collection needs site_mode='fused'")
            parts = torch.split(x, x.shape[0] // 3, dim=0)
            s, t, a = (m(p) for m, p in zip(mods, parts))
            out = torch.cat((s, torch.cat((t, a), dim=0)), dim=0) * gamma + beta
        else:
            out = getattr(self, names[1])(x) * gamma + beta
        return torch.relu_(out) if relu else out


class Bottleneck(_SiteOwner):
    def __init__(self, layers, inplanes, planes, layer, sub_layer, stats, group_size, stride,
                 downsample, site_mode):
        super().__init__()
        whiten = layer == 1
        key = f"layer{layer}.{sub_layer}"
        self.conv1 = nn.Conv2d(inplanes, planes, 1, bias=False)
        self._add_site(layers, "1", key + ".bn1", planes, whiten, group_size, stats, site_mode)
        self.conv2 = nn.Conv2d(planes, planes, 3, stride=stride, padding=1, bias=False)
        self._add_site(layers, "2", key + ".bn2", planes, whiten, group_size, stats, site_mode)
        self.conv3 = nn.Conv2d(planes, planes * EXPANSION, 1, bias=False)
        self._add_site(layers, "3", key + ".bn3", planes * EXPANSION, whiten, group_size, stats, site_mode)
        self.downsample = downsample
        if downsample is not None:
            self._add_site(layers, "downsample", f"layer{layer}.0.downsample_bn", planes * EXPANSION,
                           whiten, group_size, stats, site_mode)
        object.__setattr__(self, "_fork", getattr(layers, "fork_for_sum", None) if site_mode == "fused" else None)

    def forward(self, x):
        xa, xb = self._fork(x) if (self._fork is not None and self.training) else (x, x)
        out = self._site("1", self.conv1(xa), relu=True)
        out = self._site("2", self.conv2(out), relu=True)
        if self.downsample is None:
            return self._site("3", self.conv3(out), relu=True, residual=xb)
        tail = getattr(self, "_fused_3", None) if (self.training and not _REPLICATED[0]) else None
        if tail is None:
            identity = self._site("downsample", self.downsample(xb), relu=False)
            return self._site("3", self.conv3(out), relu=True, residual=identity)
        xd = self.downsample(xb)
        names, gname, bname, whiten = self._sites["3"]
        dnames, dgname, dbname, _ = self._sites["downsample"]
        unwrap = (lambda m: m.wh) if whiten else (lambda m: m)
        return tail.forward_with_downsample(
            self.conv3(out), [unwrap(getattr(self, n)) for n in names], getattr(self, gname), getattr(self, bname),
            xd, self._fused_downsample, [unwrap(getattr(self, n)) for n in dnames], getattr(self, dgname),
            getattr(self, dbname), count_batches=not _BATCHED_COUNTERS[0])


class ResNet50DWT(_SiteOwner):
    def __init__(self, layers, state_dict, num_classes=65, group_size=4, site_mode="modules", stem_pad=0, stem_nchw=False,
                 stem_s2d=False):
        super().__init__()
        self.stem_s2d = stem_s2d
        self.stem_nchw = stem_nchw
        self.stem_pad = stem_pad
        if site_mode not in ("modules", "fused"):
            raise ValueError("site_mode must be 'modules' or 'fused'")
        stats = {k: v for k, v in state_dict.items() if "bn" in k or "downsample" in k}
        self.site_mode = site_mode
        self.conv1 = nn.Conv2d(3, 64, 7, stride=2, padding=3, bias=False)
        self._add_site(layers, "1", "bn1", 64, True, group_size, stats, site_mode)
        self.maxpool = nn.MaxPool2d(3, stride=2, padding=1)
        inplanes = 64
        for li, (planes, blocks, stride) in enumerate(_STAGES, start=1):
            seq = []
            for b in range(blocks):
                down = None
                if b == 0 and (stride != 1 or inplanes != planes * EXPANSION):
                    down = nn.Sequential(nn.Conv2d(inplanes, planes * EXPANSION, 1, stride=stride, bias=False))
                seq.append(Bottleneck(layers, inplanes, planes, li, b, stats, 4, stride if b == 0 else 1,
                                      down, site_mode))
                inplanes = planes * EXPANSION
            setattr(self, f"layer{li}", nn.Sequential(*seq))
        self.avgpool = nn.AdaptiveAvgPool2d((1, 1))
        self.fc_out = nn.Linear(512 * EXPANSION, num_classes)
        for m in self.modules():
            if isinstance(m, nn.Conv2d):
                nn.init.kaiming_normal_(m.weight, mode="fan_out", nonlinearity="relu")

    def _stem_s2d(self, x):
        n, c, h, w = x.shape
        if h % 2 or w % 2:
            return self.conv1(x)
        cl = x.is_contiguous(memory_format=torch.channels_last) and not x.is_contiguous()
        xp = torch.nn.functional.pad(x, (3, 3, 3, 3))
        hp, wp = (h + 6) // 2, (w + 6) // 2
        wt = torch.nn.functional.pad(self.conv1.weight, (0, 1, 0, 1))
        o = wt.shape[0]
        if cl:
            xs = xp.view(n, c, hp, 2, wp, 2).permute(0, 2, 4, 1, 3, 5).reshape(n, hp, wp, 4 * c).permute(0, 3, 1, 2)
            w4 = wt.view(o, c, 4, 2, 4, 2).permute(0, 2, 4, 1, 3, 5).reshape(o, 4, 4, 4 * c).permute(0, 3, 1, 2)
        else:
            xs = xp.view(n, c, hp, 2, wp, 2).permute(0, 1, 3, 5, 2, 4).reshape(n, 4 * c, hp, wp)
            w4 = wt.view(o, c, 4, 2, 4, 2).permute(0, 1, 3, 5, 2, 4).reshape(o, 4 * c, 4, 4)
        return torch.nn.functional.conv2d(xs, w4)

    def _stem(self, x):
        if self.stem_s2d:
            return self._stem_s2d(x)
        if self.stem_nchw:
            return self.conv1(x.contiguous()).contiguous(memory_format=torch.channels_last)
        if not self.stem_pad or x.shape[1] >= self.stem_pad:
            return self.conv1(x)
        extra = self.stem_pad - x.shape[1]
        fmt = torch.channels_last if (x.is_contiguous(memory_format=torch.channels_last) and not x.is_contiguous()) \
            else torch.contiguous_format
        xp = torch.zeros((x.shape[0], self.stem_pad) + tuple(x.shape[2:]), dtype=x.dtype, device=x.device).contiguous(memory_format=fmt)
        xp[:, :x.shape[1]] = x
        w = torch.nn.functional.pad(self.conv1.weight, (0, 0, 0, 0, 0, extra))
        if fmt == torch.channels_last:
            w = w.contiguous(memory_format=torch.channels_last)
        c = self.conv1
        return torch.nn.functional.conv2d(xp, w, None, c.stride, c.padding, c.dilation, c.groups)

    def _bump_counters(self):
        cs = getattr(self, "_bn_counters", None)
        if cs is None:
            cs = [m.num_batches_tracked for m in self.modules()
                  if hasattr(m, "num_batches_tracked") and m.num_batches_tracked is not None and getattr(m, "track_running_stats", False)]
            object.__setattr__(self, "_bn_counters", cs)
        if cs:
            torch._foreach_add_(cs, 1)

    def forward(self, x):
        batched = self.training and self.site_mode == "fused"
        if batched:
            self._bump_counters()
        _BATCHED_COUNTERS[0] = batched
        try:
            x = self.maxpool(self._site("1", self._stem(x), relu=True))
            x = self.layer4(self.layer3(self.layer2(self.layer1(x))))
        finally:
            _BATCHED_COUNTERS[0] = False
        return self.fc_out(torch.flatten(self.avgpool(x), 1))


def build_resnet50_dwt(state_dict, layers, site_mode="modules", num_classes=65, channels_last=False, stem_pad=0,
                       stem_nchw=False, stem_s2d=False, group_size=4):
    model = ResNet50DWT(layers, state_dict, num_classes=num_classes, group_size=group_size, site_mode=site_mode,
                        stem_pad=stem_pad, stem_nchw=stem_nchw and channels_last, stem_s2d=stem_s2d)
    model.load_state_dict(state_dict, strict=False)
    if channels_last and hasattr(layers, "MaxPool2d"):
        model.maxpool = layers.MaxPool2d(3, stride=2, padding=1)
    if channels_last:
        for m in model.modules():
            if isinstance(m, nn.Conv2d) and not (model.stem_nchw and m is model.conv1):
                m.weight.data = m.weight.data.contiguous(memory_format=torch.channels_last)
    return model


def collect_stats(model, batches, passes=1, replicated=True):
    was_training = model.training
    model.train(True)
    out = None
    try:
        with torch.no_grad():
            for _ in range(passes):
                for data in batches:
                    if replicated:
                        _REPLICATED[0] = True
                        out = model(data)
                    else:
                        out = model(torch.cat((data, data, data), dim=0))
    finally:
        _REPLICATED[0] = False
        model.train(was_training)
    return out
```

include/dwt_b200.h:

```cpp
#ifndef DWT_B200_H_
#define DWT_B200_H_

#include <stddef.h>
#include <stdint.h>

#ifdef __cplusplus
extern "C" {
#endif

#define DWT_B200_ABI_VERSION 10
#define DWT_MAX_DOMAINS 4
#define DWT_MAX_GROUP_SIZE 64
#define DWT_TC_MAX_GROUP_SIZE 128

#define DWT_OK 0
#define DWT_E_INVALID (-1)
#define DWT_E_WORKSPACE (-2)
#define DWT_E_LAUNCH (-3)
#define DWT_E_UNSUPPORTED (-4)

#define DWT_MODE_TRAIN 0
#define DWT_MODE_EVAL 1

#define DWT_LAYOUT_NHWC 0x100

#define DWT_DTYPE_BF16 0x200

#define DWT_EPI_NONE 0
#define DWT_EPI_AFFINE 1
#define DWT_EPI_RELU 2
#define DWT_EPI_RESIDUAL 4

typedef struct CUstream_st *dwt_stream_t;

#if defined(__GNUC__)
#define DWT_API __attribute__((visibility("default")))
#else
#define DWT_API
#endif

DWT_API int dwt_abi_version(void);
DWT_API const char *dwt_last_error(void);

DWT_API size_t dwt_workspace_bytes(int64_t N, int64_t C, int64_t HW, int group_size, int n_domains);

#define DWT_STATUS_NOT_PD 1
#define DWT_STATUS_BAD_LABEL 2

DWT_API int dwt_whiten_fwd(const float *x, float *y, int64_t N, int64_t C, int64_t HW, int group_size,
                   int n_domains, int mode, float eps, float momentum, int update_running,
                   float *const *running_mean, float *const *running_cov, const float *gamma,
                   const float *beta, const float *residual, uint8_t *relu_mask, int epilogue, float *save_mean,
                   float *save_w, void *workspace, size_t workspace_bytes, dwt_stream_t stream);

DWT_API int dwt_whiten_bwd(const float *x, const float *dout, const float *dout2, float *dx, int64_t N, int64_t C, int64_t HW,
                   int group_size, int n_domains, int mode, float eps, const float *save_mean,
                   const float *save_w, const float *gamma, const float *beta, const uint8_t *relu_mask,
                   float *dresidual, int epilogue, float *dgamma, float *dbeta, void *workspace,
                   size_t workspace_bytes, dwt_stream_t stream);

#define DWT_ZCA_MAX_ITERATIONS 16
DWT_API int dwt_whiten_zca_fwd(const float *x, float *y, int64_t N, int64_t C, int64_t HW, int group_size, int n_domains,
                       int mode, float eps, float momentum, int update_running, float *const *running_mean,
                       float *const *running_cov, int iterations, float *save_mean, float *save_w, float *save_p,
                       void *workspace, size_t workspace_bytes, dwt_stream_t stream);
DWT_API int dwt_whiten_zca_bwd(const float *x, const float *dout, float *dx, int64_t N, int64_t C, int64_t HW, int group_size,
                       int n_domains, int mode, float eps, int iterations, const float *save_mean, const float *save_w,
                       const float *save_p, void *workspace, size_t workspace_bytes, dwt_stream_t stream);

DWT_API int dwt_whiten_eigh_fwd(const float *x, float *y, int64_t N, int64_t C, int64_t HW, int group_size, int n_domains,
                       int mode, float eps, float momentum, int update_running, float *const *running_mean,
                       float *const *running_cov, float *save_mean, float *save_w, float *save_e,
                       void *workspace, size_t workspace_bytes, dwt_stream_t stream);
DWT_API int dwt_whiten_eigh_bwd(const float *x, const float *dout, float *dx, int64_t N, int64_t C, int64_t HW, int group_size,
                       int n_domains, int mode, float eps, const float *save_mean, const float *save_w,
                       const float *save_e, void *workspace, size_t workspace_bytes, dwt_stream_t stream);

DWT_API int dwt_whiten_color_fwd(const float *x, float *y, int64_t N, int64_t C, int64_t HW, int group_size, int n_domains,
                       int mode, float eps, float momentum, int update_running, float *const *running_mean,
                       float *const *running_cov, const float *color, const float *bias, float *save_mean, float *save_w,
                       void *workspace, size_t workspace_bytes, dwt_stream_t stream);
DWT_API int dwt_whiten_color_bwd(const float *x, const float *dout, float *dx, int64_t N, int64_t C, int64_t HW, int group_size,
                       int n_domains, int mode, float eps, const float *save_mean, const float *save_w, const float *color,
                       float *dcolor, float *dbias, void *workspace, size_t workspace_bytes, dwt_stream_t stream);

DWT_API size_t dwt_instance_workspace_bytes(int64_t N, int64_t C, int64_t HW, int group_size);
DWT_API int dwt_whiten_instance_fwd(const float *x, float *y, int64_t N, int64_t C, int64_t HW, int group_size, int flags,
                       float eps, float *save_mean, float *save_w, void *workspace, size_t workspace_bytes,
                       dwt_stream_t stream);
DWT_API int dwt_whiten_instance_bwd(const float *x, const float *dout, float *dx, int64_t N, int64_t C, int64_t HW,
                       int group_size, int flags, float eps, const float *save_mean, const float *save_w, void *workspace,
                       size_t workspace_bytes, dwt_stream_t stream);

DWT_API size_t dwt_switch_workspace_bytes(int64_t N, int64_t C, int64_t HW, int group_size);
DWT_API int dwt_whiten_switch_fwd(const float *x, float *y, int64_t N, int64_t C, int64_t HW, int group_size, int mode,
                   float eps, float momentum, int update_running, float *running_mean, float *running_cov,
                   const float *mix, float *save_mean, float *save_w, float *save_stats,
                   void *workspace, size_t workspace_bytes, dwt_stream_t stream);
DWT_API int dwt_whiten_switch_bwd(const float *x, const float *dout, float *dx, int64_t N, int64_t C, int64_t HW,
                   int group_size, int mode, float eps, const float *mix, const float *save_mean, const float *save_w,
                   const float *save_stats, float *dmix, void *workspace, size_t workspace_bytes, dwt_stream_t stream);

DWT_API int dwt_bn_fwd(const float *x, float *y, int64_t N, int64_t C, int64_t HW, int n_domains, int mode,
               float eps, float factor, int update_running, float *const *running_mean,
               float *const *running_var, const float *weight, const float *bias, const float *residual,
               uint8_t *relu_mask, int epilogue, float *save_mean, float *save_invstd, void *workspace,
               size_t workspace_bytes, dwt_stream_t stream);

DWT_API int dwt_bn_bwd(const float *x, const float *dout, const float *dout2, float *dx, int64_t N, int64_t C, int64_t HW,
               int n_domains, int mode, const float *save_mean, const float *save_invstd,
               const float *weight, const float *bias, const uint8_t *relu_mask, float *dresidual, int epilogue,
               float *dweight, float *dbias, void *workspace, size_t workspace_bytes, dwt_stream_t stream);

#define DWT_KIND_WHITEN 0
#define DWT_KIND_BN 1
typedef struct {
  const float *x;
  float eps, momentum;
  int update_running;
  float *const *running_mean;
  float *const *running_cov;
  const float *gamma, *beta;
  float *save_mean, *save_w;
  float *dx;
  float *dgamma, *dbeta;
} dwt_tail_site;

DWT_API int dwt_tail2_fwd(int kind, const dwt_tail_site *sites, float *y, uint8_t *relu_mask, int64_t N, int64_t C,
                  int64_t HW, int group_size, int n_domains, void *workspace, size_t workspace_bytes,
                  dwt_stream_t stream);
DWT_API int dwt_tail2_bwd(int kind, const dwt_tail_site *sites, const float *dout, const float *dout2,
                  const uint8_t *relu_mask, float *dz, int64_t N, int64_t C, int64_t HW, int group_size,
                  int n_domains, void *workspace, size_t workspace_bytes, dwt_stream_t stream);

DWT_API int dwt_mec_fwd_bwd(const float *x, const float *y, int64_t N, int64_t K, float *loss, float *gx,
                    float *gy, dwt_stream_t stream);

DWT_API int dwt_head_loss_fwd_bwd(const float *logits, const int64_t *labels, int64_t B, int64_t K, float lambda,
                          float *losses, float *grad, int *status, dwt_stream_t stream);

DWT_API int dwt_augment_pair(const uint8_t *images, int64_t B, int src_h, int src_w, int crop, const int32_t *crop_plain,
                     const int32_t *crop_aug, const uint8_t *flip, const float *affine, const float *mean,
                     const float *stdv, float *out_plain, float *out_aug, int layout, dwt_stream_t stream);

DWT_API int dwt_maxpool_fwd(const float *x, float *y, uint8_t *argmax, int64_t N, int64_t H, int64_t W, int64_t C,
                    int kernel, int stride, int padding, int flags, dwt_stream_t stream);
DWT_API int dwt_maxpool_bwd(const float *dy, const uint8_t *argmax, float *dx, int64_t N, int64_t H, int64_t W, int64_t C,
                    int kernel, int stride, int padding, int flags, dwt_stream_t stream);

typedef struct {
  char name[48];
  int64_t launches;
  double ms;
  double bytes;
} dwt_profile_entry;

DWT_API int64_t dwt_launch_count(void);
DWT_API void dwt_profile_begin(void);
DWT_API int dwt_profile_end(dwt_profile_entry *out, int max_entries);

#ifdef __cplusplus
}
#endif
#endif
```

Before: 3377.

## Fuse stem whitening site with ReLU and 3x3 max-pool in forward and backward

```diff
diff --git a/dwt-domain-adaptation_b200/dwt_b200/_native.py b/dwt-domain-adaptation_b200/dwt_b200/_native.py
--- a/dwt-domain-adaptation_b200/dwt_b200/_native.py
+++ b/dwt-domain-adaptation_b200/dwt_b200/_native.py
@@ -105,6 +105,14 @@
     "dwt_tail2_bwd": (ctypes.c_int, [ctypes.c_int, ctypes.POINTER(TailSite), _c_float_p, _c_float_p, ctypes.c_void_p,
                                      _c_float_p, ctypes.c_int64, ctypes.c_int64, ctypes.c_int64, ctypes.c_int, ctypes.c_int,
                                      ctypes.c_void_p, ctypes.c_size_t, ctypes.c_void_p]),
+    "dwt_site_pool_fwd": (ctypes.c_int, [ctypes.c_int, _c_float_p, _c_float_p, ctypes.c_void_p, ctypes.c_int64, ctypes.c_int64,
+                                         ctypes.c_int64, ctypes.c_int64, ctypes.c_int, ctypes.c_int, ctypes.c_float, ctypes.c_float,
+                                         ctypes.c_int, ctypes.POINTER(ctypes.c_void_p), ctypes.POINTER(ctypes.c_void_p), _c_float_p,
+                                         _c_float_p, _c_float_p, _c_float_p, ctypes.c_void_p, ctypes.c_size_t, ctypes.c_void_p]),
+    "dwt_site_pool_bwd": (ctypes.c_int, [ctypes.c_int, _c_float_p, _c_float_p, ctypes.c_void_p, _c_float_p, ctypes.c_int64,
+                                         ctypes.c_int64, ctypes.c_int64, ctypes.c_int64, ctypes.c_int, ctypes.c_int, ctypes.c_float,
+                                         _c_float_p, _c_float_p, _c_float_p, _c_float_p, _c_float_p, _c_float_p, ctypes.c_void_p,
+                                         ctypes.c_size_t, ctypes.c_void_p]),
     "dwt_mec_fwd_bwd": (ctypes.c_int, [_c_float_p, _c_float_p, ctypes.c_int64, ctypes.c_int64, _c_float_p,
                                        _c_float_p, _c_float_p, ctypes.c_void_p]),
     "dwt_head_loss_fwd_bwd": (ctypes.c_int, [_c_float_p, ctypes.c_void_p, ctypes.c_int64, ctypes.c_int64, ctypes.c_float,
@@ -185,6 +193,12 @@
     return 0 < channels // 4 <= 16384
 
 
+def stem_pool_supported(channels: int, h: int, w: int, group_size: int) -> bool:
+    c4 = channels // 4
+    return (group_size in (1, 4) and channels % 4 == 0 and 1 <= c4 <= 256 and c4 & (c4 - 1) == 0
+            and h >= 4 and w >= 4 and h % 4 == 0 and w % 4 == 0)
+
+
 def small_bf16_supported(hw: int, group_size: int) -> bool:
     return group_size in (1, 2, 4) and hw % 4 == 0
 
diff --git a/dwt-domain-adaptation_b200/dwt_b200/build.py b/dwt-domain-adaptation_b200/dwt_b200/build.py
--- a/dwt-domain-adaptation_b200/dwt_b200/build.py
+++ b/dwt-domain-adaptation_b200/dwt_b200/build.py
@@ -8,7 +8,7 @@
 HERE = os.path.dirname(os.path.abspath(__file__))
 CSRC = os.path.join(HERE, "csrc")
 LIB = os.path.join(HERE, "lib", "libdwt_b200.so")
-SOURCES = ["api.cu", "norm_small.cu", "norm_tiled.cu", "norm_tc.cu", "norm_tc_apply.cu", "norm_dense.cu", "norm_cl.cu", "mec.cu", "augment.cu", "pool.cu"]
+SOURCES = ["api.cu", "norm_small.cu", "norm_tiled.cu", "norm_tc.cu", "norm_tc_apply.cu", "norm_dense.cu", "norm_cl.cu", "mec.cu", "augment.cu", "pool.cu", "stem_pool.cu"]
 NVCC_FLAGS = ["-O3", "-std=c++17", "-gencode", "arch=compute_90a,code=sm_90a", "-lineinfo",
               "-Xcompiler", "-fPIC,-fvisibility=hidden", "--expt-relaxed-constexpr"]
 NVCC_FLAGS += shlex.split(os.environ.get("DWT_NVCC_EXTRA", ""))
diff --git a/dwt-domain-adaptation_b200/dwt_b200/csrc/api.cu b/dwt-domain-adaptation_b200/dwt_b200/csrc/api.cu
--- a/dwt-domain-adaptation_b200/dwt_b200/csrc/api.cu
+++ b/dwt-domain-adaptation_b200/dwt_b200/csrc/api.cu
@@ -763,6 +763,91 @@
   return check_launch("channels-last two-site backward apply kernel");
 }
 
+int site_pool_check(int kind, int64_t C, int64_t H, int64_t W, int GS, const uint8_t* argmax) {
+  if (kind != DWT_KIND_WHITEN && kind != DWT_KIND_BN) return fail(DWT_E_INVALID, "bad kind %d", kind);
+  if (kind == DWT_KIND_BN && GS != 1) return fail(DWT_E_INVALID, "batch norm has group_size 1 (got %d)", GS);
+  if (H <= 0 || W <= 0 || H > 65536 || W > 65536 || C <= 0 || C > 65536 || !dwt::stem_pool_supports((int)C, (int)H, (int)W, GS))
+    return fail(DWT_E_UNSUPPORTED, "the site + max-pool kernels are built for H and W multiples of 4, C/4 a power of two <= 256, "
+                "group_size 4 (whitening) or 1 (C=%lld H=%lld W=%lld gs=%d)", (long long)C, (long long)H, (long long)W, GS);
+  if (!argmax) return fail(DWT_E_INVALID, "null pointer argument");
+  if ((uintptr_t)argmax % 4 != 0) return fail(DWT_E_INVALID, "argmax must be 4-byte aligned");
+  return DWT_OK;
+}
+
+int site_pool_fwd(int kind, const void* x, void* y, uint8_t* argmax, int64_t N, int64_t C, int64_t H, int64_t W, int GS, int D,
+                  float eps, float momentum, int update_running, float* const* rmean, float* const* rcov, const float* gamma,
+                  const float* beta, float* save_mean, float* save_w, void* ws, size_t ws_bytes, cudaStream_t st) {
+  const bool bf16 = (kind & DWT_DTYPE_BF16) != 0;
+  kind &= ~DWT_DTYPE_BF16;
+  if (int rc = site_pool_check(kind, C, H, W, GS, argmax)) return rc;
+  const int64_t HW = H * W;
+  const int epi = DWT_EPI_AFFINE | DWT_EPI_RELU;
+  Call c;
+  const int mode = DWT_MODE_TRAIN | DWT_LAYOUT_NHWC | (bf16 ? DWT_DTYPE_BF16 : 0);
+  if (int rc = validate(c, false, x, x, y, nullptr, N, C, HW, GS, D, mode, epi, gamma, beta, save_mean, save_w, ws, ws_bytes,
+                        [&] { return check_running(update_running != 0, rmean, rcov, D); }))
+    return rc;
+  const Plan& p = c.p; const Workspace& w = c.w;
+  const SiteConst sc = site_const(kind, eps, N, HW);
+  const dwt::FwdFin fin = make_fwd_fin(sc.a, sc.b, momentum, sc.unbias, update_running, update_running != 0, rmean, rcov, save_mean,
+                                       save_w, w, D);
+  const double n_el = (double)D * (double)N * (double)C * (double)HW;
+  const double E = (bf16 ? 2.0 : 4.0) * n_el;
+  const ClPlan cp = cl_plan(p.gm, 3, 3, 8, 8);
+  {
+    Launch l(fam(bf16, "cl_stats", "cl_stats_bf16"), &p.gm, E, st);
+    dwt::cl_stats(x, bf16, p.gm, cp.nred, cp.gz_red, w.partial, w.shift, st);
+  }
+  if (int rc = check_launch("channels-last statistics kernel")) return rc;
+  {
+    Launch l(fam(bf16, "cl_fwd_finalize", "cl_fwd_finalize_bf16"), &p.gm, 0.0, st);
+    dwt::cl_fwd_finalize(w.partial, cp.nred, w.shift, p.gm, fin, st);
+  }
+  if (int rc = check_launch("channels-last finalize kernel")) return rc;
+  {
+    Launch l(fam(bf16, "maxpool_fwd_site", "maxpool_fwd_site_bf16"), &p.gm, 1.25 * E + n_el / 4, st);
+    dwt::stem_pool_apply(x, y, argmax, bf16, p.gm, (int)H, (int)W, sm_count(), save_mean, save_w, gamma, beta, st);
+  }
+  return check_launch("site + max-pool apply kernel");
+}
+
+int site_pool_bwd(int kind, const void* x, const void* dy, const uint8_t* argmax, void* dx, int64_t N, int64_t C, int64_t H, int64_t W,
+                  int GS, int D, float eps, const float* save_mean, const float* save_w, const float* gamma, const float* beta,
+                  float* dgamma, float* dbeta, void* ws, size_t ws_bytes, cudaStream_t st) {
+  const bool bf16 = (kind & DWT_DTYPE_BF16) != 0;
+  kind &= ~DWT_DTYPE_BF16;
+  if (int rc = site_pool_check(kind, C, H, W, GS, argmax)) return rc;
+  const int64_t HW = H * W;
+  const int epi = DWT_EPI_AFFINE | DWT_EPI_RELU;
+  Call c;
+  const int mode = DWT_MODE_TRAIN | DWT_LAYOUT_NHWC | (bf16 ? DWT_DTYPE_BF16 : 0);
+  if (int rc = validate(c, true, x, dy, dx, nullptr, N, C, HW, GS, D, mode, epi, gamma, beta, save_mean, save_w, ws, ws_bytes, [&] {
+        return (dgamma == nullptr) != (dbeta == nullptr) ? fail(DWT_E_INVALID, "dgamma and dbeta go together") : DWT_OK;
+      }))
+    return rc;
+  const Plan& p = c.p; const Workspace& w = c.w;
+  const dwt::BwdFin fin = make_bwd_fin(site_const(kind, eps, N, HW).a, DWT_MODE_TRAIN, epi, save_mean, save_w, gamma, dgamma, dbeta, w);
+  const double n_el = (double)D * (double)N * (double)C * (double)HW;
+  const double E = (bf16 ? 2.0 : 4.0) * n_el;
+  const ClPlan cp = cl_plan(p.gm, 2, 2, 4, 4);
+  const int nred = cp.nred;
+  {
+    Launch l(fam(bf16, "maxpool_bwd_site_reduce", "maxpool_bwd_site_reduce_bf16"), &p.gm, 1.25 * E + n_el / 4, st);
+    dwt::cl_pool_bwd_reduce(x, dy, argmax, bf16, p.gm, (int)W, nred, cp.gz_red, save_mean, save_w, gamma, beta, w.partial, st);
+  }
+  if (int rc = check_launch("site + max-pool backward reduction kernel")) return rc;
+  {
+    Launch l(fam(bf16, "cl_bwd_finalize", "cl_bwd_finalize_bf16"), &p.gm, 0.0, st);
+    dwt::cl_bwd_finalize(w.partial, nred, p.gm, fin, st);
+  }
+  if (int rc = check_launch("channels-last backward finalize kernel")) return rc;
+  {
+    Launch l(fam(bf16, "maxpool_bwd_site_apply", "maxpool_bwd_site_apply_bf16"), &p.gm, 2.25 * E + n_el / 4, st);
+    dwt::stem_pool_bwd_apply(x, dy, argmax, dx, bf16, p.gm, (int)H, (int)W, sm_count(), w.coef, save_mean, save_w, gamma, beta, st);
+  }
+  return check_launch("site + max-pool backward apply kernel");
+}
+
 int inst_refuse(int64_t N, int64_t C, int64_t HW, int GS, int flags, const char* what = "instance whitening") {
   return fail(DWT_E_UNSUPPORTED, "%s is built for the tensor-core kernels only: group_size 8, 16, 32, 64 "
               "dividing C, HW >= 256 and a multiple of 4 (NCHW bf16: of 8), N <= 65535 images, N*C*HW < 2^31 "
@@ -1179,6 +1264,22 @@
                    (cudaStream_t)stream);
 }
 
+int dwt_site_pool_fwd(int kind, const float* x, float* y, uint8_t* argmax, int64_t N, int64_t C, int64_t H, int64_t W, int group_size,
+                      int n_domains, float eps, float momentum, int update_running, float* const* running_mean,
+                      float* const* running_cov, const float* gamma, const float* beta, float* save_mean, float* save_w,
+                      void* workspace, size_t workspace_bytes, dwt_stream_t stream) {
+  return site_pool_fwd(kind, x, y, argmax, N, C, H, W, group_size, n_domains, eps, momentum, update_running, running_mean, running_cov,
+                       gamma, beta, save_mean, save_w, workspace, workspace_bytes, (cudaStream_t)stream);
+}
+
+int dwt_site_pool_bwd(int kind, const float* x, const float* dy, const uint8_t* argmax, float* dx, int64_t N, int64_t C, int64_t H,
+                      int64_t W, int group_size, int n_domains, float eps, const float* save_mean, const float* save_w,
+                      const float* gamma, const float* beta, float* dgamma, float* dbeta, void* workspace, size_t workspace_bytes,
+                      dwt_stream_t stream) {
+  return site_pool_bwd(kind, x, dy, argmax, dx, N, C, H, W, group_size, n_domains, eps, save_mean, save_w, gamma, beta, dgamma, dbeta,
+                       workspace, workspace_bytes, (cudaStream_t)stream);
+}
+
 int dwt_mec_fwd_bwd(const float* x, const float* y, int64_t N, int64_t K, float* loss, float* gx, float* gy,
                     dwt_stream_t stream) {
   if (!x || !y || !loss || !gx || !gy) return fail(DWT_E_INVALID, "null pointer argument");
diff --git a/dwt-domain-adaptation_b200/dwt_b200/csrc/norm_cl.cu b/dwt-domain-adaptation_b200/dwt_b200/csrc/norm_cl.cu
--- a/dwt-domain-adaptation_b200/dwt_b200/csrc/norm_cl.cu
+++ b/dwt-domain-adaptation_b200/dwt_b200/csrc/norm_cl.cu
@@ -1,10 +1,9 @@
 #include <stdlib.h>
 
-#include <type_traits>
-
 #include <cuda_bf16.h>
 
 #include "dwt_common.cuh"
+#include "norm_cl.cuh"
 #include "norm_launch.h"
 #include "small_algebra.cuh"
 
@@ -15,15 +14,6 @@
 
 __device__ __forceinline__ void pdl_wait() { asm volatile("griddepcontrol.wait;" ::: "memory"); }
 __device__ __forceinline__ void pdl_launch_dependents() { asm volatile("griddepcontrol.launch_dependents;" ::: "memory"); }
-
-template <int GS> struct ClShape {
-  static constexpr int NSUB = 4 / GS;
-  static constexpr int NM = GS * (GS + 1) / 2;
-  static constexpr int FWD1 = GS + NM;
-  static constexpr int BWD1 = GS * GS + GS;
-  static constexpr int FWD = NSUB * FWD1;
-  static constexpr int BWD = NSUB * BWD1;
-};
 
 struct ClThread {
   int C4, CW, LS, rpi, col, rsub, q;
@@ -47,13 +37,6 @@
 }
 #define CL_FOR_DOMAINS(d, gm, DESC) \
   for (int di_ = blockIdx.z, d = (DESC) ? (gm).D - 1 - di_ : di_; di_ < (gm).D; di_ += gridDim.z, d = (DESC) ? (gm).D - 1 - di_ : di_)
-
-template <class T> constexpr bool kBf16 = !std::is_same<T, float>::value;
-template <class T>
-__device__ __forceinline__ float as_stored(float v) {
-  if constexpr (kBf16<T>) return __bfloat162float(__float2bfloat16_rn(v));
-  else return v;
-}
 
 template <int NACC>
 __device__ __forceinline__ void column_reduce(const ClThread& t, float (&acc)[NACC], float* sRed) {
@@ -355,16 +338,6 @@
         }
       }
     });
-  }
-}
-
-template <int GS>
-__device__ __forceinline__ void bwd_accumulate(float* acc, const float (&dz)[GS], const float (&xi)[GS], const float* mu) {
-#pragma unroll
-  for (int i = 0; i < GS; ++i) {
-    acc[GS * GS + i] += dz[i];
-#pragma unroll
-    for (int j = 0; j < GS; ++j) acc[i * GS + j] = fmaf(dz[i], xi[j] - mu[j], acc[i * GS + j]);
   }
 }
 
@@ -495,6 +468,116 @@
   }
 }
 
+template <class T>
+__device__ __forceinline__ float4 pool_gather(const uint32_t* __restrict__ ixd, const T* __restrict__ gd, unsigned n, unsigned h,
+                                              unsigned w, int OH, int OW, int C4) {
+  const int oh0 = (int)(h >> 1), ow0 = (int)(w >> 1);
+  const bool h2 = (h & 1u) && oh0 + 1 < OH, w2 = (w & 1u) && ow0 + 1 < OW;
+  uint32_t m[2][2];
+  float4 g[2][2];
+#pragma unroll
+  for (int a = 0; a < 2; ++a)
+#pragma unroll
+    for (int b = 0; b < 2; ++b) {
+      const bool ok = (a == 0 || h2) && (b == 0 || w2);
+      const size_t o = ((size_t)n * OH + oh0 + a) * OW + ow0 + b;
+      m[a][b] = ok ? __ldg(ixd + o * C4) : 0xFFFFFFFFu;
+      g[a][b] = ok ? ld4(gd + o * 4 * C4) : make_float4(0.f, 0.f, 0.f, 0.f);
+    }
+  float4 acc = make_float4(0.f, 0.f, 0.f, 0.f);
+#pragma unroll
+  for (int a = 0; a < 2; ++a)
+#pragma unroll
+    for (int b = 0; b < 2; ++b) {
+      const unsigned code = (h + 1u - 2u * (unsigned)(oh0 + a)) * 3u + (w + 1u - 2u * (unsigned)(ow0 + b));
+      if ((m[a][b] & 0xFFu) == code) acc.x += g[a][b].x;
+      if (((m[a][b] >> 8) & 0xFFu) == code) acc.y += g[a][b].y;
+      if (((m[a][b] >> 16) & 0xFFu) == code) acc.z += g[a][b].z;
+      if ((m[a][b] >> 24) == code) acc.w += g[a][b].w;
+    }
+  return make_float4(as_stored<T>(acc.x), as_stored<T>(acc.y), as_stored<T>(acc.z), as_stored<T>(acc.w));
+}
+
+template <class T, int GS>
+__global__ void __launch_bounds__(kT, 2) cl_pool_bwd_reduce_kernel(const T* __restrict__ x, const T* __restrict__ dy,
+                                                                   const uint8_t* __restrict__ idx, const Geom gm, const int W,
+                                                                   const float* __restrict__ save_mean, const float* __restrict__ save_w,
+                                                                   const float* __restrict__ gamma, const float* __restrict__ beta,
+                                                                   float* __restrict__ partial) {
+  using S = ClShape<GS>;
+  constexpr int UNROLL = 4;
+  constexpr int EPI = DWT_EPI_AFFINE | DWT_EPI_RELU;
+  __shared__ float sRed[kT * S::BWD];
+  const ClThread t(gm);
+  const unsigned rows = (unsigned)gm.N * gm.HW;
+  const int H = gm.HW / W, OW = W >> 1, OH = H >> 1;
+  CL_FOR_DOMAINS(d, gm, true) {
+    float Wp[S::NSUB][S::NM], bp[S::NSUB][GS], mu[4];
+    if (t.active) {
+#pragma unroll
+      for (int s = 0; s < S::NSUB; ++s) {
+        const int g = t.q * S::NSUB + s;
+        load_forward_map<GS, EPI>(save_w + ((size_t)d * gm.G + g) * GS * GS, save_mean + (size_t)d * gm.C + g * GS,
+                                  gamma + g * GS, beta + g * GS, Wp[s], bp[s]);
+      }
+      const float4 m4 = ldg4(save_mean + (size_t)d * gm.C + 4 * t.q);
+      mu[0] = m4.x; mu[1] = m4.y; mu[2] = m4.z; mu[3] = m4.w;
+    }
+    float acc[S::BWD];
+#pragma unroll
+    for (int i = 0; i < S::BWD; ++i) acc[i] = 0.f;
+    const T* xd = x + (size_t)d * rows * gm.C + 4 * t.q;
+    const size_t pd = (size_t)d * gm.N * OH * OW;
+    const uint32_t* ixd = reinterpret_cast<const uint32_t*>(idx) + pd * t.C4 + t.q;
+    const T* gd = dy + pd * gm.C + 4 * t.q;
+    if (t.active) sweep_rows<UNROLL, true>(t, rows, [&](unsigned r) {
+      float4 v[UNROLL], q[UNROLL];
+      unsigned n = r / (unsigned)gm.HW, h = r - n * (unsigned)gm.HW, w = h % (unsigned)W;
+      h /= (unsigned)W;
+#pragma unroll
+      for (int u = 0; u < UNROLL; ++u) {
+        const unsigned rr = r + u * t.rpi;
+        if (u > 0) {
+          w += (unsigned)t.rpi;
+          while (w >= (unsigned)W) {
+            w -= (unsigned)W;
+            if (++h == (unsigned)H) { h = 0; ++n; }
+          }
+        }
+        if (rr < rows) {
+          v[u] = ld4(xd + (size_t)rr * gm.C);
+          q[u] = pool_gather<T>(ixd, gd, n, h, w, OH, OW, t.C4);
+        } else {
+          v[u] = make_float4(mu[0], mu[1], mu[2], mu[3]);
+          q[u] = make_float4(0.f, 0.f, 0.f, 0.f);
+        }
+      }
+#pragma unroll
+      for (int u = 0; u < UNROLL; ++u) {
+        const float ge[4] = {q[u].x, q[u].y, q[u].z, q[u].w};
+        const float e[4] = {v[u].x, v[u].y, v[u].z, v[u].w};
+#pragma unroll
+        for (int s = 0; s < S::NSUB; ++s) {
+          float xi[GS], dz[GS], oi[GS];
+#pragma unroll
+          for (int c = 0; c < GS; ++c) { xi[c] = e[s * GS + c]; dz[c] = ge[s * GS + c]; }
+          apply_group<GS>(Wp[s], bp[s], xi, oi);
+#pragma unroll
+          for (int c = 0; c < GS; ++c) dz[c] = oi[c] > 0.f ? dz[c] : 0.f;
+          bwd_accumulate<GS>(acc + s * S::BWD1, dz, xi, &mu[s * GS]);
+        }
+      }
+    });
+    column_reduce<S::BWD>(t, acc, sRed);
+    if (t.rsub == 0 && t.active) {
+      float* dst = partial + (((size_t)d * gridDim.x + blockIdx.x) * t.C4 + t.q) * S::BWD;
+#pragma unroll
+      for (int i = 0; i < S::BWD; ++i) dst[i] = acc[i];
+    }
+    if (gridDim.z == 1) __syncthreads();
+  }
+}
+
 template <int GS>
 __device__ __forceinline__ void cl_bwd_finalize_site(const float* __restrict__ partial, int nrows, const Geom& gm, const BwdFin& fin) {
   using SH = ClShape<GS>;
@@ -535,36 +618,6 @@
   const bool second = blockIdx.y != 0;
   cl_bwd_finalize_site<GS>(partial + (second ? pstride : 0), nrows, gm, second ? fin2 : fin);
 }
-
-template <int GS>
-struct BwdCoef {
-  float A1[GS * (GS + 1) / 2], Bm[GS * (GS + 1) / 2], cv[GS];
-  __device__ __forceinline__ void load(const float* cf) {
-#pragma unroll
-    for (int i = 0; i < GS; ++i) {
-      cv[i] = __ldg(cf + 2 * GS * GS + i);
-#pragma unroll
-      for (int j = 0; j <= i; ++j) {
-        A1[i * (i + 1) / 2 + j] = __ldg(cf + j * GS + i);
-        Bm[i * (i + 1) / 2 + j] = __ldg(cf + GS * GS + i * GS + j);
-      }
-    }
-  }
-  __device__ __forceinline__ void apply(const float (&dz)[GS], const float (&xi)[GS], float* o) const {
-#pragma unroll
-    for (int i = 0; i < GS; ++i) {
-      float a = cv[i];
-#pragma unroll
-      for (int j = i; j < GS; ++j) a = fmaf(A1[j * (j + 1) / 2 + i], dz[j], a);
-#pragma unroll
-      for (int j = 0; j < GS; ++j) {
-        const int hi = i > j ? i : j, lo = i > j ? j : i;
-        a = fmaf(Bm[hi * (hi + 1) / 2 + lo], xi[j], a);
-      }
-      o[i] = a;
-    }
-  }
-};
 
 template <class T, int GS, int EPI, bool D2, bool DS>
 __global__ void __launch_bounds__(kT, 2) cl_bwd_apply_kernel(const T* __restrict__ x, const T* __restrict__ dout, const T* __restrict__ dout2,
@@ -800,6 +853,11 @@
                                            CL_IN(x), CL_IN(dout), CL_IN(dout2), cl_geom(gm), mean, nul, nul, nul, mask, CL_OUT(dz), partial, CL_IN(xd),
                                            mean_d, pstride)))));
 }
+void cl_pool_bwd_reduce(const void* x, const void* dy, const uint8_t* idx, bool bf16, const Geom& gm, int W, int nctas, int gz,
+                        const float* mean, const float* w, const float* gamma, const float* beta, float* partial, cudaStream_t st) {
+  CL_T(bf16, CL_GS(gm.GS, (cl_pool_bwd_reduce_kernel<TT, kGS><<<cl_grid(gm, nctas, gz), kT, 0, st>>>(
+                              CL_IN(x), CL_IN(dy), idx, cl_geom(gm), W, mean, w, gamma, beta, partial))));
+}
 void cl_bwd_finalize(const float* partial, int nrows, const Geom& gm, const BwdFin& fin, cudaStream_t st, const BwdFin* fin2, size_t pstride) {
   const dim3 b = fin_block(gm), g(fin_blocks(gm, b), fin2 ? 2 : 1);
   CL_GS(gm.GS, (launch_k(cl_bwd_finalize_kernel<kGS>, g, b, st, use_pdl(), partial, pstride, nrows, gm, fin, fin2 ? *fin2 : fin)));
diff --git a/dwt-domain-adaptation_b200/dwt_b200/csrc/norm_cl.cuh b/dwt-domain-adaptation_b200/dwt_b200/csrc/norm_cl.cuh
--- /dev/null
+++ b/dwt-domain-adaptation_b200/dwt_b200/csrc/norm_cl.cuh
@@ -0,0 +1,67 @@
+#pragma once
+
+#include <type_traits>
+
+#include <cuda_bf16.h>
+
+#include "dwt_common.cuh"
+
+namespace dwt {
+
+template <int GS> struct ClShape {
+  static constexpr int NSUB = 4 / GS;
+  static constexpr int NM = GS * (GS + 1) / 2;
+  static constexpr int FWD1 = GS + NM;
+  static constexpr int BWD1 = GS * GS + GS;
+  static constexpr int FWD = NSUB * FWD1;
+  static constexpr int BWD = NSUB * BWD1;
+};
+
+template <class T> constexpr bool kBf16 = !std::is_same<T, float>::value;
+template <class T>
+__device__ __forceinline__ float as_stored(float v) {
+  if constexpr (kBf16<T>) return __bfloat162float(__float2bfloat16_rn(v));
+  else return v;
+}
+
+template <int GS>
+__device__ __forceinline__ void bwd_accumulate(float* acc, const float (&dz)[GS], const float (&xi)[GS], const float* mu) {
+#pragma unroll
+  for (int i = 0; i < GS; ++i) {
+    acc[GS * GS + i] += dz[i];
+#pragma unroll
+    for (int j = 0; j < GS; ++j) acc[i * GS + j] = fmaf(dz[i], xi[j] - mu[j], acc[i * GS + j]);
+  }
+}
+
+template <int GS>
+struct BwdCoef {
+  float A1[GS * (GS + 1) / 2], Bm[GS * (GS + 1) / 2], cv[GS];
+  __device__ __forceinline__ void load(const float* cf) {
+#pragma unroll
+    for (int i = 0; i < GS; ++i) {
+      cv[i] = __ldg(cf + 2 * GS * GS + i);
+#pragma unroll
+      for (int j = 0; j <= i; ++j) {
+        A1[i * (i + 1) / 2 + j] = __ldg(cf + j * GS + i);
+        Bm[i * (i + 1) / 2 + j] = __ldg(cf + GS * GS + i * GS + j);
+      }
+    }
+  }
+  __device__ __forceinline__ void apply(const float (&dz)[GS], const float (&xi)[GS], float* o) const {
+#pragma unroll
+    for (int i = 0; i < GS; ++i) {
+      float a = cv[i];
+#pragma unroll
+      for (int j = i; j < GS; ++j) a = fmaf(A1[j * (j + 1) / 2 + i], dz[j], a);
+#pragma unroll
+      for (int j = 0; j < GS; ++j) {
+        const int hi = i > j ? i : j, lo = i > j ? j : i;
+        a = fmaf(Bm[hi * (hi + 1) / 2 + lo], xi[j], a);
+      }
+      o[i] = a;
+    }
+  }
+};
+
+}
diff --git a/dwt-domain-adaptation_b200/dwt_b200/csrc/norm_launch.h b/dwt-domain-adaptation_b200/dwt_b200/csrc/norm_launch.h
--- a/dwt-domain-adaptation_b200/dwt_b200/csrc/norm_launch.h
+++ b/dwt-domain-adaptation_b200/dwt_b200/csrc/norm_launch.h
@@ -107,6 +107,14 @@
 void cl_tail2_bwd_apply(const void* x, const void* xd, const void* dz, void* dx, void* dxd, bool bf16, const Geom& gm, int nctas, int gz,
                         const float* coef, const float* coef_d, cudaStream_t st);
 
+bool stem_pool_supports(int C, int H, int W, int GS);
+void stem_pool_apply(const void* x, void* y, uint8_t* idx, bool bf16, const Geom& gm, int H, int W, int sms, const float* mean,
+                     const float* w, const float* gamma, const float* beta, cudaStream_t st);
+void cl_pool_bwd_reduce(const void* x, const void* dy, const uint8_t* idx, bool bf16, const Geom& gm, int W, int nctas, int gz,
+                        const float* mean, const float* w, const float* gamma, const float* beta, float* partial, cudaStream_t st);
+void stem_pool_bwd_apply(const void* x, const void* dy, const uint8_t* idx, void* dx, bool bf16, const Geom& gm, int H, int W, int sms,
+                         const float* coef, const float* mean, const float* w, const float* gamma, const float* beta, cudaStream_t st);
+
 void maxpool_fwd_launch(const void* x, void* y, bool bf16, uint8_t* idx, int N, int H, int W, int C, int OH, int OW, int k, int s, int p,
                         cudaStream_t st);
 void maxpool_bwd_launch(const void* dy, const uint8_t* idx, void* dx, bool bf16, int N, int H, int W, int C, int OH, int OW, int k, int s,
diff --git a/dwt-domain-adaptation_b200/dwt_b200/csrc/stem_pool.cu b/dwt-domain-adaptation_b200/dwt_b200/csrc/stem_pool.cu
--- /dev/null
+++ b/dwt-domain-adaptation_b200/dwt_b200/csrc/stem_pool.cu
@@ -0,0 +1,278 @@
+#include <cuda_bf16.h>
+
+#include "dwt_common.cuh"
+#include "norm_cl.cuh"
+#include "norm_launch.h"
+#include "small_algebra.cuh"
+
+namespace dwt {
+namespace {
+
+constexpr int kT = 256;
+constexpr int kEpi = DWT_EPI_AFFINE | DWT_EPI_RELU;
+
+struct SpGeom {
+  int N;
+  int H, W;
+  int C4;
+  int c4shift;
+  int G;
+};
+
+template <class T>
+__device__ __forceinline__ float4 stored(const float4& v) {
+  if constexpr (kBf16<T>) {
+    const __nv_bfloat162 a = __floats2bfloat162_rn(v.x, v.y), b = __floats2bfloat162_rn(v.z, v.w);
+    return make_float4(__low2float(a), __high2float(a), __low2float(b), __high2float(b));
+  } else {
+    return v;
+  }
+}
+
+struct SpThread {
+  int q, lane, lanes;
+  __device__ __forceinline__ explicit SpThread(const SpGeom& g)
+      : q(threadIdx.x & (g.C4 - 1)), lane(threadIdx.x >> g.c4shift), lanes(kT >> g.c4shift) {}
+};
+
+template <int GS>
+struct FwdMap {
+  static constexpr int NSUB = 4 / GS;
+  float Wp[NSUB][GS * (GS + 1) / 2], bp[NSUB][GS];
+  __device__ __forceinline__ void load(const float* save_w, const float* save_mean, const float* gamma, const float* beta, int d,
+                                       const SpGeom& g, int q) {
+#pragma unroll
+    for (int s = 0; s < NSUB; ++s) {
+      const int gi = q * NSUB + s;
+      load_forward_map<GS, kEpi>(save_w + ((size_t)d * g.G + gi) * GS * GS, save_mean + (size_t)d * 4 * g.C4 + gi * GS,
+                                 gamma + gi * GS, beta + gi * GS, Wp[s], bp[s]);
+    }
+  }
+  __device__ __forceinline__ void pre(const float4& v, float (&o)[4]) const {
+    const float e[4] = {v.x, v.y, v.z, v.w};
+#pragma unroll
+    for (int s = 0; s < NSUB; ++s) {
+      float xi[GS], oi[GS];
+#pragma unroll
+      for (int c = 0; c < GS; ++c) xi[c] = e[s * GS + c];
+      apply_group<GS>(Wp[s], bp[s], xi, oi);
+#pragma unroll
+      for (int c = 0; c < GS; ++c) o[s * GS + c] = oi[c];
+    }
+  }
+};
+
+__device__ __forceinline__ bool takes(float v, float best) { return (v > best) || (v != v); }
+
+template <class T, int GS>
+__global__ void __launch_bounds__(kT, 2) stem_pool_apply_kernel(const T* __restrict__ x, T* __restrict__ y, uint8_t* __restrict__ idx,
+                                                             const SpGeom g, const float* __restrict__ save_mean,
+                                                             const float* __restrict__ save_w, const float* __restrict__ gamma,
+                                                             const float* __restrict__ beta) {
+  const SpThread t(g);
+  const int d = blockIdx.z, C = 4 * g.C4, OH = g.H >> 1, OW = g.W >> 1, OW2 = OW >> 1;
+  FwdMap<GS> fm;
+  fm.load(save_w, save_mean, gamma, beta, d, g, t.q);
+  const unsigned per_img = (unsigned)(OH >> 1) * OW2, total = (unsigned)g.N * per_img;
+  for (unsigned i = blockIdx.x * t.lanes + t.lane; i < total; i += gridDim.x * t.lanes) {
+    const unsigned nl = i / per_img, rem = i - nl * per_img;
+    const int a = (int)(rem / OW2), b = (int)(rem - (unsigned)a * OW2);
+    const size_t n = (size_t)d * g.N + nl;
+    const T* xn = x + n * g.H * g.W * C + 4 * t.q;
+    float best[2][2][4];
+    unsigned bi[2][2][4];
+    const int h0 = 4 * a - 1, w0 = 4 * b - 1;
+#pragma unroll
+    for (int oa = 0; oa < 2; ++oa)
+#pragma unroll
+      for (int ob = 0; ob < 2; ++ob) {
+        const unsigned first = (unsigned)(max(0, -(h0 + 2 * oa)) * 3 + max(0, -(w0 + 2 * ob)));
+#pragma unroll
+        for (int c = 0; c < 4; ++c) { best[oa][ob][c] = -INFINITY; bi[oa][ob][c] = first; }
+      }
+#pragma unroll
+    for (int r = 0; r < 5; ++r) {
+      const int h = h0 + r;
+      if (h < 0 || h >= g.H) continue;
+      float4 row[5];
+      bool in[5];
+#pragma unroll
+      for (int cc = 0; cc < 5; ++cc) {
+        const int w = w0 + cc;
+        in[cc] = w >= 0 && w < g.W;
+        row[cc] = in[cc] ? ld4(xn + ((size_t)h * g.W + w) * C) : make_float4(0.f, 0.f, 0.f, 0.f);
+      }
+#pragma unroll
+      for (int cc = 0; cc < 5; ++cc) {
+        float o[4];
+        fm.pre(row[cc], o);
+        row[cc] = stored<T>(make_float4(fmaxf(o[0], 0.f), fmaxf(o[1], 0.f), fmaxf(o[2], 0.f), fmaxf(o[3], 0.f)));
+      }
+#pragma unroll
+      for (int oa = 0; oa < 2; ++oa) {
+        const int kh = r - 2 * oa;
+        if (kh < 0 || kh > 2) continue;
+#pragma unroll
+        for (int ob = 0; ob < 2; ++ob)
+#pragma unroll
+          for (int kw = 0; kw < 3; ++kw) {
+            const int cc = 2 * ob + kw;
+            if (!in[cc]) continue;
+            const float e[4] = {row[cc].x, row[cc].y, row[cc].z, row[cc].w};
+            const unsigned code = (unsigned)(kh * 3 + kw);
+#pragma unroll
+            for (int c = 0; c < 4; ++c)
+              if (takes(e[c], best[oa][ob][c])) { best[oa][ob][c] = e[c]; bi[oa][ob][c] = code; }
+          }
+      }
+    }
+#pragma unroll
+    for (int oa = 0; oa < 2; ++oa)
+#pragma unroll
+      for (int ob = 0; ob < 2; ++ob) {
+        const size_t o = ((n * OH + 2 * a + oa) * OW + 2 * b + ob) * g.C4 + t.q;
+        st4(y + 4 * o, make_float4(best[oa][ob][0], best[oa][ob][1], best[oa][ob][2], best[oa][ob][3]));
+        reinterpret_cast<uint32_t*>(idx)[o] = bi[oa][ob][0] | (bi[oa][ob][1] << 8) | (bi[oa][ob][2] << 16) | (bi[oa][ob][3] << 24);
+      }
+  }
+}
+
+__device__ __forceinline__ void take(float4& acc, const float4& gq, uint32_t m, unsigned code) {
+  if ((m & 0xFFu) == code) acc.x += gq.x;
+  if (((m >> 8) & 0xFFu) == code) acc.y += gq.y;
+  if (((m >> 16) & 0xFFu) == code) acc.z += gq.z;
+  if ((m >> 24) == code) acc.w += gq.w;
+}
+
+template <class T>
+struct Patch {
+  float4 x[4], dy[4];
+  __device__ __forceinline__ void load(const T* __restrict__ x_, const T* __restrict__ dy_, const uint8_t* __restrict__ idx, const SpGeom& g,
+                                       size_t n, int k, int j, int q) {
+    const int C = 4 * g.C4, OH = g.H >> 1, OW = g.W >> 1;
+    const size_t p0 = ((n * g.H + 2 * k) * g.W + 2 * j) * C + 4 * q;
+    x[0] = ld4(x_ + p0);
+    x[1] = ld4(x_ + p0 + C);
+    x[2] = ld4(x_ + p0 + (size_t)g.W * C);
+    x[3] = ld4(x_ + p0 + (size_t)g.W * C + C);
+    uint32_t m[2][2];
+    float4 gq[2][2];
+#pragma unroll
+    for (int a = 0; a < 2; ++a)
+#pragma unroll
+      for (int b = 0; b < 2; ++b) {
+        const bool ok = (k + a < OH) && (j + b < OW);
+        const size_t o = ((n * OH + k + a) * OW + (j + b)) * g.C4 + q;
+        m[a][b] = ok ? __ldg(reinterpret_cast<const uint32_t*>(idx) + o) : 0xFFFFFFFFu;
+        gq[a][b] = ok ? ld4(dy_ + 4 * o) : make_float4(0.f, 0.f, 0.f, 0.f);
+      }
+    float4 o00 = make_float4(0.f, 0.f, 0.f, 0.f), o01 = o00, o10 = o00, o11 = o00;
+    take(o00, gq[0][0], m[0][0], 4u);
+    take(o01, gq[0][0], m[0][0], 5u); take(o01, gq[0][1], m[0][1], 3u);
+    take(o10, gq[0][0], m[0][0], 7u); take(o10, gq[1][0], m[1][0], 1u);
+    take(o11, gq[0][0], m[0][0], 8u); take(o11, gq[0][1], m[0][1], 6u); take(o11, gq[1][0], m[1][0], 2u); take(o11, gq[1][1], m[1][1], 0u);
+    dy[0] = stored<T>(o00); dy[1] = stored<T>(o01); dy[2] = stored<T>(o10); dy[3] = stored<T>(o11);
+  }
+  template <int GS>
+  __device__ __forceinline__ void dz(const FwdMap<GS>& fm, int p, int s, float (&xi)[GS], float (&dzi)[GS]) const {
+    const float e[4] = {x[p].x, x[p].y, x[p].z, x[p].w}, ge[4] = {dy[p].x, dy[p].y, dy[p].z, dy[p].w};
+    float oi[GS];
+#pragma unroll
+    for (int c = 0; c < GS; ++c) xi[c] = e[s * GS + c];
+    apply_group<GS>(fm.Wp[s], fm.bp[s], xi, oi);
+#pragma unroll
+    for (int c = 0; c < GS; ++c) dzi[c] = oi[c] > 0.f ? ge[s * GS + c] : 0.f;
+  }
+};
+
+__device__ __forceinline__ void patch_of(unsigned i, unsigned per_img, int W2, int d, const SpGeom& g, size_t& n, int& k, int& j) {
+  const unsigned nl = i / per_img, rem = i - nl * per_img;
+  k = (int)(rem / (unsigned)W2);
+  j = (int)(rem - (unsigned)k * W2);
+  n = (size_t)d * g.N + nl;
+}
+
+template <class T, int GS>
+__global__ void __launch_bounds__(kT, 3) stem_pool_bwd_apply_kernel(const T* __restrict__ x, const T* __restrict__ dy,
+                                                                 const uint8_t* __restrict__ idx, T* __restrict__ dx, const SpGeom g,
+                                                                 const float* __restrict__ coef, const float* __restrict__ save_mean,
+                                                                 const float* __restrict__ save_w, const float* __restrict__ gamma,
+                                                                 const float* __restrict__ beta) {
+  using S = ClShape<GS>;
+  const SpThread t(g);
+  const int d = blockIdx.z, C = 4 * g.C4, W2 = g.W >> 1;
+  FwdMap<GS> fm;
+  fm.load(save_w, save_mean, gamma, beta, d, g, t.q);
+  BwdCoef<GS> cf[S::NSUB];
+#pragma unroll
+  for (int s = 0; s < S::NSUB; ++s) cf[s].load(coef + ((size_t)d * g.G + t.q * S::NSUB + s) * coef_stride(GS));
+  const unsigned per_img = (unsigned)(g.H >> 1) * W2, total = (unsigned)g.N * per_img;
+  for (unsigned i = blockIdx.x * t.lanes + t.lane; i < total; i += gridDim.x * t.lanes) {
+    size_t n;
+    int k, j;
+    patch_of(i, per_img, W2, d, g, n, k, j);
+    Patch<T> pt;
+    pt.load(x, dy, idx, g, n, k, j, t.q);
+    T* d0 = dx + ((n * g.H + 2 * k) * g.W + 2 * j) * C + 4 * t.q;
+#pragma unroll
+    for (int p = 0; p < 4; ++p) {
+      float o[4];
+#pragma unroll
+      for (int s = 0; s < S::NSUB; ++s) {
+        float xi[GS], dzi[GS];
+        pt.template dz<GS>(fm, p, s, xi, dzi);
+        cf[s].apply(dzi, xi, o + s * GS);
+      }
+      st4(d0 + ((p >> 1) * (size_t)g.W + (p & 1)) * C, make_float4(o[0], o[1], o[2], o[3]));
+    }
+  }
+}
+
+SpGeom sp_geom(const Geom& gm, int H, int W) {
+  const int C4 = gm.C / 4;
+  int sh = 0;
+  while ((1 << sh) < C4) ++sh;
+  return SpGeom{gm.N, H, W, C4, sh, gm.G};
+}
+
+int sp_ctas(const Geom& gm, int H, int W, int sms, int per_sm) {
+  const long long lanes = kT / (gm.C / 4), patches = (long long)gm.N * (H / 2) * (W / 2);
+  long long n = (long long)per_sm * sms / gm.D;
+  const long long steps = (patches + lanes - 1) / lanes;
+  if (n > steps) n = steps;
+  return n < 1 ? 1 : (int)n;
+}
+
+#define SP_GS(GS_, ...)                                         \
+  if ((GS_) == 4) { constexpr int kGS = 4; __VA_ARGS__; }       \
+  else { constexpr int kGS = 1; __VA_ARGS__; }
+#define SP_T(BF16_, ...)                                        \
+  if (BF16_) { using TT = __nv_bfloat16; __VA_ARGS__; }         \
+  else { using TT = float; __VA_ARGS__; }
+
+}
+
+bool stem_pool_supports(int C, int H, int W, int GS) {
+  const int C4 = C / 4;
+  return (GS == 1 || GS == 4) && C % 4 == 0 && C4 >= 1 && C4 <= kT && (C4 & (C4 - 1)) == 0 && H >= 4 && W >= 4 && H % 4 == 0 &&
+         W % 4 == 0;
+}
+
+void stem_pool_apply(const void* x, void* y, uint8_t* idx, bool bf16, const Geom& gm, int H, int W, int sms, const float* mean,
+                     const float* w, const float* gamma, const float* beta, cudaStream_t st) {
+  const SpGeom g = sp_geom(gm, H, W);
+  const dim3 grid(sp_ctas(gm, H, W, sms, 8), 1, gm.D);
+  SP_T(bf16, SP_GS(gm.GS, (stem_pool_apply_kernel<TT, kGS><<<grid, kT, 0, st>>>(static_cast<const TT*>(x), static_cast<TT*>(y), idx, g,
+                                                                                 mean, w, gamma, beta))));
+}
+
+void stem_pool_bwd_apply(const void* x, const void* dy, const uint8_t* idx, void* dx, bool bf16, const Geom& gm, int H, int W, int sms,
+                         const float* coef, const float* mean, const float* w, const float* gamma, const float* beta, cudaStream_t st) {
+  const SpGeom g = sp_geom(gm, H, W);
+  const dim3 grid(sp_ctas(gm, H, W, sms, 8), 1, gm.D);
+  SP_T(bf16, SP_GS(gm.GS, (stem_pool_bwd_apply_kernel<TT, kGS><<<grid, kT, 0, st>>>(static_cast<const TT*>(x), static_cast<const TT*>(dy),
+                                                                                     idx, static_cast<TT*>(dx), g, coef, mean, w, gamma,
+                                                                                     beta))));
+}
+
+}
diff --git a/dwt-domain-adaptation_b200/dwt_b200/functional.py b/dwt-domain-adaptation_b200/dwt_b200/functional.py
--- a/dwt-domain-adaptation_b200/dwt_b200/functional.py
+++ b/dwt-domain-adaptation_b200/dwt_b200/functional.py
@@ -312,6 +312,82 @@
                                    [(r, float(e), float(m), bool(u)) for r, e, m, u in sites])
 
 
+class _SitePoolFunction(torch.autograd.Function):
+
+    @staticmethod
+    def forward(ctx, x, gamma, beta, kind, group_size, n_domains, eps, momentum, update_running, running):
+        lib = nv.lib()
+        gs = group_size if kind == "whiten" else 1
+        n_all, c, h, w = x.shape
+        n = n_all // n_domains
+        stats = [gamma, beta, *[t for pair in running for t in pair]]
+        dev = nv.require_cuda(x, *stats, bf16=True)
+        nv.require_cuda(*stats)
+        for d, (rm_t, rv_t) in enumerate(running):
+            _check_param(f"running mean of domain {d}", rm_t, c)
+            _check_param(f"running second moment of domain {d}", rv_t, c * gs)
+        _check_param("gamma / weight", gamma, c)
+        _check_param("beta / bias", beta, c)
+        gamma_c, beta_c = gamma.detach().reshape(-1).contiguous(), beta.detach().reshape(-1).contiguous()
+        y = torch.empty((n_all, c, h // 2, w // 2), dtype=x.dtype, device=dev, memory_format=torch.channels_last)
+        idx = torch.empty(y.numel(), dtype=torch.uint8, device=dev)
+        save_mean = torch.empty(n_domains, c, dtype=torch.float32, device=dev)
+        save_w = torch.empty(n_domains, c // gs, gs, gs, dtype=torch.float32, device=dev)
+        ws = nv.workspace(dev, n, c, h * w, gs, n_domains)
+        rm = nv.ptr_array([p[0] for p in running]) if update_running else None
+        rv = nv.ptr_array([p[1] for p in running]) if update_running else None
+        nv_kind = (nv.KIND_WHITEN if kind == "whiten" else nv.KIND_BN) | (nv.DTYPE_BF16 if x.dtype == torch.bfloat16 else 0)
+        with torch.cuda.device(dev):
+            rc = lib.dwt_site_pool_fwd(nv_kind, nv.ptr(x), nv.ptr(y), nv.ptr(idx), n, c, h, w, gs, n_domains, eps, momentum,
+                                       int(update_running), rm, rv, nv.ptr(gamma_c), nv.ptr(beta_c), nv.ptr(save_mean),
+                                       nv.ptr(save_w), nv.ptr(ws), ws.numel(), nv.stream_ptr(dev))
+        nv.check(rc)
+        nv.poll_status(dev)
+        if update_running:
+            seen = set()
+            for buf in (t for pair in running for t in pair):
+                if id(buf) not in seen:
+                    seen.add(id(buf))
+                    torch.autograd.graph.increment_version(buf)
+        ctx.save_for_backward(x, save_mean, save_w, gamma_c, beta_c, idx)
+        ctx.cfg = (nv_kind, gs, n_domains, n, c, h, w, eps, gamma.shape)
+        ctx.mark_non_differentiable(idx)
+        return y, idx
+
+    @staticmethod
+    def backward(ctx, dy, _didx):
+        lib = nv.lib()
+        x, save_mean, save_w, gamma_c, beta_c, idx = ctx.saved_tensors
+        nv_kind, gs, n_domains, n, c, h, w, eps, gshape = ctx.cfg
+        dy = dy.to(x.dtype).contiguous(memory_format=torch.channels_last)
+        if dy.data_ptr() % (8 if x.dtype == torch.bfloat16 else 16):
+            dy = dy.clone(memory_format=torch.channels_last)
+        dev = nv.require_cuda(dy, bf16=True)
+        dx = torch.empty_like(x)
+        want_affine = ctx.needs_input_grad[1] or ctx.needs_input_grad[2]
+        dgamma = torch.empty(c, dtype=torch.float32, device=dev) if want_affine else None
+        dbeta = torch.empty(c, dtype=torch.float32, device=dev) if want_affine else None
+        ws = nv.workspace(dev, n, c, h * w, gs, n_domains)
+        with torch.cuda.device(dev):
+            rc = lib.dwt_site_pool_bwd(nv_kind, nv.ptr(x), nv.ptr(dy), nv.ptr(idx), nv.ptr(dx), n, c, h, w, gs, n_domains, eps,
+                                       nv.ptr(save_mean), nv.ptr(save_w), nv.ptr(gamma_c), nv.ptr(beta_c), nv.ptr(dgamma),
+                                       nv.ptr(dbeta), nv.ptr(ws), ws.numel(), nv.stream_ptr(dev))
+        nv.check(rc)
+        if want_affine:
+            dgamma, dbeta = dgamma.view(gshape), dbeta.view(gshape)
+        return (dx, dgamma, dbeta) + (None,) * 7
+
+
+def site_pool_fits(x, gamma, kind, group_size, n_domains, training_stats, relu, residual, iterations, pool):
+    from .pooling import MaxPool2d
+    gs = group_size if kind == "whiten" else 1
+    return (training_stats and relu and residual is None and not iterations and gamma is not None
+            and isinstance(pool, MaxPool2d) and (pool.kernel_size, pool.stride, pool.padding) == (3, 2, 1)
+            and _channels_last(x) and x.dtype in _ACT_DTYPES and x.shape[0] % n_domains == 0
+            and x.data_ptr() % (8 if x.dtype == torch.bfloat16 else 16) == 0
+            and nv.stem_pool_supported(x.shape[1], x.shape[2], x.shape[3], gs))
+
+
 class _ForkForSum(torch.autograd.Function):
 
     @staticmethod
@@ -341,7 +417,14 @@
 
 
 def norm(x, gamma, beta, *, kind, group_size, n_domains, training_stats, eps, momentum, update_running,
-         running, relu=False, residual=None, iterations=0):
+         running, relu=False, residual=None, iterations=0, pool=None):
+    if pool is not None:
+        if site_pool_fits(x, gamma, kind, group_size, n_domains, training_stats, relu, residual, iterations, pool):
+            return _SitePoolFunction.apply(x, gamma, beta, kind, group_size, n_domains, float(eps), float(momentum),
+                                           bool(update_running), running)
+        return pool(norm(x, gamma, beta, kind=kind, group_size=group_size, n_domains=n_domains, training_stats=training_stats,
+                         eps=eps, momentum=momentum, update_running=update_running, running=running, relu=relu,
+                         residual=residual, iterations=iterations)), None
     if iterations != nv.EIGH and iterations and not 1 <= iterations <= nv.ZCA_MAX_ITERATIONS:
         raise ValueError(f"iterations must be in [1, {nv.ZCA_MAX_ITERATIONS}] (got {iterations})")
     mode = nv.MODE_TRAIN if training_stats else nv.MODE_EVAL
diff --git a/dwt-domain-adaptation_b200/dwt_b200/fused.py b/dwt-domain-adaptation_b200/dwt_b200/fused.py
--- a/dwt-domain-adaptation_b200/dwt_b200/fused.py
+++ b/dwt-domain-adaptation_b200/dwt_b200/fused.py
@@ -115,6 +115,18 @@
         return F.tail_pair(x, xd, gamma, beta, down_gamma, down_beta, kind=self.kind, group_size=self.group_size,
                            n_domains=self.n_domains, sites=(site_args, down_args))
 
+    def forward_with_pool(self, x, domain_modules, gamma, beta, pool, replicated=False, count_batches=True):
+        mods = list(domain_modules)
+        fuse = (not replicated and self.kernel_epilogue and len(mods) == self.n_domains and x.dim() == 4 and mods[0].training
+                and gamma is not None and not (gamma.dim() == 3 and tuple(gamma.shape[1:]) != (1, 1)))
+        if not fuse:
+            return pool(self(x, mods, gamma, beta, True, replicated=replicated, count_batches=count_batches))
+        self._iterations(mods)
+        running, eps, momentum, update = self._running_args(mods, count_batches)
+        y, _ = F.norm(x, gamma, beta, kind=self.kind, group_size=self.group_size, n_domains=self.n_domains, training_stats=True,
+                      eps=eps, momentum=momentum, update_running=update, running=running, relu=True, pool=pool)
+        return y
+
     @staticmethod
     def _tensor_epilogue(y, gamma, beta, relu, residual):
         if residual is not None and not relu:
diff --git a/harness/resnet50_dwt.py b/harness/resnet50_dwt.py
--- a/harness/resnet50_dwt.py
+++ b/harness/resnet50_dwt.py
@@ -197,13 +197,22 @@
         if cs:
             torch._foreach_add_(cs, 1)
 
+    def _stem_site_pool(self, x):
+        fused = getattr(self, "_fused_1", None) if self.training else None
+        if fused is None or not hasattr(fused, "forward_with_pool"):
+            return self.maxpool(self._site("1", x, relu=True))
+        names, gname, bname, whiten = self._sites["1"]
+        mods = [getattr(self, n) for n in names]
+        return fused.forward_with_pool(x, [m.wh if whiten else m for m in mods], getattr(self, gname), getattr(self, bname),
+                                       self.maxpool, replicated=_REPLICATED[0], count_batches=not _BATCHED_COUNTERS[0])
+
     def forward(self, x):
         batched = self.training and self.site_mode == "fused"
         if batched:
             self._bump_counters()
         _BATCHED_COUNTERS[0] = batched
         try:
-            x = self.maxpool(self._site("1", self._stem(x), relu=True))
+            x = self._stem_site_pool(self._stem(x))
             x = self.layer4(self.layer3(self.layer2(self.layer1(x))))
         finally:
             _BATCHED_COUNTERS[0] = False
diff --git a/include/dwt_b200.h b/include/dwt_b200.h
--- a/include/dwt_b200.h
+++ b/include/dwt_b200.h
@@ -133,6 +133,15 @@
                   const uint8_t *relu_mask, float *dz, int64_t N, int64_t C, int64_t HW, int group_size,
                   int n_domains, void *workspace, size_t workspace_bytes, dwt_stream_t stream);
 
+DWT_API int dwt_site_pool_fwd(int kind, const float *x, float *y, uint8_t *argmax, int64_t N, int64_t C, int64_t H, int64_t W,
+                      int group_size, int n_domains, float eps, float momentum, int update_running,
+                      float *const *running_mean, float *const *running_cov, const float *gamma, const float *beta,
+                      float *save_mean, float *save_w, void *workspace, size_t workspace_bytes, dwt_stream_t stream);
+DWT_API int dwt_site_pool_bwd(int kind, const float *x, const float *dy, const uint8_t *argmax, float *dx, int64_t N, int64_t C,
+                      int64_t H, int64_t W, int group_size, int n_domains, float eps, const float *save_mean,
+                      const float *save_w, const float *gamma, const float *beta, float *dgamma, float *dbeta,
+                      void *workspace, size_t workspace_bytes, dwt_stream_t stream);
+
 DWT_API int dwt_mec_fwd_bwd(const float *x, const float *y, int64_t N, int64_t K, float *loss, float *gx,
                     float *gy, dwt_stream_t stream);
 
```

Measured after the change: 3426, median of 6. 1.4% higher.
